# feiyeha/EGM-Unet

Measured on AMD Instinct MI355X. Metric: train images/sec at 3x512x512 bs=8/GPU, higher is better.
Workload: dtype bf16; 1 GPU; EGM-UNet GRFBUNet(3,2,base_c=32) fwd+5-term-loss+bwd+SGD, 8x3x512x512 per GPU (BASELINE.json configs[1]); global_batch=8, parallelism=dp1, launch=hipGraph replay, world_size=1

## Files before the change

egm_unet_amd/csrc/bn.hip:

```cpp
#include "common.h"
#include "bn_elem.h"
#include <stdlib.h>

namespace {


template <typename T, int MODE>
__device__ __forceinline__ void channel_partials_body(const T* __restrict__ a, int lda, const T* __restrict__ y, int ldy,
                                                      const float* __restrict__ scale, const float* __restrict__ shift,
                                                      const float* __restrict__ mean, const float* __restrict__ rstd,
                                                      int act, long long npix, int C, float* __restrict__ out, int bid, int nb) {
    __shared__ float red[2 * 256 * 8];
    const int ncv = C >> 3, rows = 256 / ncv;
    const int tid = threadIdx.x, cv = tid % ncv, row = tid / ncv;
    float s[8], q[8];
    zero8(s); zero8(q);
    if (MODE == 1) {
        for (int c = tid; c < C; c += 256) { red[c] = scale[c]; red[C + c] = shift[c]; red[2 * C + c] = mean[c]; red[3 * C + c] = rstd[c]; }
        __syncthreads();
    }
    float sc[8], sh[8], mu[8], rs[8];
    if (MODE == 1) {
#pragma unroll
        for (int j = 0; j < 8; ++j) { sc[j] = red[cv * 8 + j]; sh[j] = red[C + cv * 8 + j]; mu[j] = red[2 * C + cv * 8 + j]; rs[j] = red[3 * C + cv * 8 + j]; }
        __syncthreads();
    }
    if (row < rows) {
        for (long long p = (long long)bid * rows + row; p < npix; p += (long long)nb * rows) {
            float v[8];
            load8(a + p * lda + cv * 8, v);
            if (MODE == 0) {
#pragma unroll
                for (int j = 0; j < 8; ++j) { s[j] += v[j]; q[j] += v[j] * v[j]; }
            } else {
                float yv[8];
                load8(y + p * ldy + cv * 8, yv);
#pragma unroll
                for (int j = 0; j < 8; ++j) {
                    const float g = v[j] * act_grad<sizeof(T) == 2>(fmaf(yv[j], sc[j], sh[j]), act);
                    s[j] += g; q[j] += g * (yv[j] - mu[j]) * rs[j];
                }
            }
        }
    }
#pragma unroll
    for (int j = 0; j < 8; ++j) { red[tid * 8 + j] = s[j]; red[(256 + tid) * 8 + j] = q[j]; }
    __syncthreads();
    for (int t = tid; t < 2 * C; t += 256) {
        const int which = t / C, c = t - which * C, ccv = c >> 3, j = c & 7;
        float v = 0.f;
        for (int r = 0; r < rows; ++r) v += red[(which * 256 + r * ncv + ccv) * 8 + j];
        out[((long long)bid * 2 + which) * C + c] = v;
    }
}
template <typename T, int MODE>
__global__ __launch_bounds__(256) void channel_partials_kernel(const T* __restrict__ a, int lda, const T* __restrict__ y, int ldy,
                                                               const float* __restrict__ scale, const float* __restrict__ shift,
                                                               const float* __restrict__ mean, const float* __restrict__ rstd,
                                                               int act, long long npix, int C, float* __restrict__ out) {
    channel_partials_body<T, MODE>(a, lda, y, ldy, scale, shift, mean, rstd, act, npix, C, out, blockIdx.x, gridDim.x);
}

__device__ __forceinline__ void tiles_reduce(const float* __restrict__ st, int ntiles, int C, int c0, double& s_out, double& q_out,
                                             double* red) {
    const int tid = threadIdx.x, j = tid & 7, tl = tid >> 3;
    const int c = c0 + j;
    double s = 0.0, q = 0.0;
    if (c < C) {
        for (int t = tl; t < ntiles; t += 128) {
            s += (double)st[((long long)t * 2 + 0) * C + c];
            q += (double)st[((long long)t * 2 + 1) * C + c];
        }
    }
    red[tid] = s; red[1024 + tid] = q;
    __syncthreads();
    for (int stride = 64; stride > 0; stride >>= 1) {
        if (tl < stride) { red[tid] += red[tid + stride * 8]; red[1024 + tid] += red[1024 + tid + stride * 8]; }
        __syncthreads();
    }
    s_out = red[j]; q_out = red[1024 + j];
}

__global__ __launch_bounds__(1024) void reduce_tiles_kernel(const float* __restrict__ st, int ntiles, int C, float* __restrict__ out) {
    __shared__ double red[2048];
    double s, q;
    st += (long long)blockIdx.y * ntiles * 2 * C;
    out += (long long)blockIdx.y * 2 * C;
    tiles_reduce(st, ntiles, C, blockIdx.x * 8, s, q, red);
    const int c = blockIdx.x * 8 + (threadIdx.x & 7);
    if (threadIdx.x < 8 && c < C) { out[c] = (float)s; out[C + c] = (float)q; }
}

__device__ __forceinline__ void bn_finalize_body(const float* __restrict__ st, int ntiles, double count,
                                                 const float* __restrict__ gamma, const float* __restrict__ beta, float eps,
                                                 float momentum, float* __restrict__ rmean, float* __restrict__ rvar,
                                                 float* __restrict__ scale, float* __restrict__ shift,
                                                 float* __restrict__ save_mean, float* __restrict__ save_rstd, int C,
                                                 int Creal, int bid) {
    __shared__ double red[2048];
    double s, q;
    tiles_reduce(st, ntiles, C, bid * 8, s, q, red);
    const int c = bid * 8 + (threadIdx.x & 7);
    if (threadIdx.x < 8 && c >= Creal && c < C) { scale[c] = 0.f; shift[c] = 0.f; save_mean[c] = 0.f; save_rstd[c] = 0.f; }
    if (threadIdx.x < 8 && c < Creal) {
        const double mean = s / count;
        double var = q / count - mean * mean;
        if (var < 0.0) var = 0.0;
// ... 437 lines not shown
```

egm_unet_amd/csrc/conv3x3_tile.hip:

```cpp
#include "common.h"
#include "group.h"
#include "bn_elem.h"
#include <stdlib.h>

typedef __attribute__((ext_vector_type(8))) __bf16 bf16x8_t;
typedef __attribute__((ext_vector_type(16))) float f32x16_t;

__device__ uint4 egm_zero_page[4];

#ifndef EGM_TILE_DMA_EVERY
#define EGM_TILE_DMA_EVERY 1
#endif

namespace {

constexpr int TW = 32, PW = TW + 2, KC = 16;

struct TileParams {
    const bf16_t* x; const bf16_t* w; const float* bias; bf16_t* y; float* stats;
    bf16_t* y2; int ldy2, csplit;
    int ldx, ldy, N, H, W, Cin, Cout, bias_n;
    int tiles_y, tiles_x, npt, nct, G;
    int dbg;
};

template <int R, int NT, int WR, int WC, int NBUF> struct TileGeom {
    static constexpr int TROWS = WR * R, PH = TROWS + 2, NC = WC * NT * 32;
    static constexpr int PSLOTS = PH * PW * 2, WSLOTS = 9 * NC * 2;
    static constexpr int NPI = (PSLOTS + 63) / 64, NWI = WSLOTS / 64;
    static constexpr int KT = (NPI + NWI + 7) / 8;
    static constexpr int STAGE_BYTES = KT * 8 * 1024;
    static constexpr int WOFF = NPI * 1024;
    static constexpr int OROW = NT * 64 + 16;
    static constexpr int OUT_BYTES = 8 * 32 * OROW;
    static constexpr int SMEM = NBUF * STAGE_BYTES + OUT_BYTES;
    static_assert(WSLOTS % 64 == 0, "weight image must be whole DMA instructions");
    static_assert(SMEM <= 160 * 1024, "LDS budget");
    static_assert(9 * NC * 32 + 64 * 32 < 65536, "ds_read immediate offsets");
};

typedef __attribute__((ext_vector_type(2))) float f32x2_t;
typedef __attribute__((ext_vector_type(2))) __bf16 bf16x2_t;
__device__ __forceinline__ uint32_t pack_bf16x2(float lo, float hi) {
    f32x2_t v; v.x = lo; v.y = hi;
    const bf16x2_t b = __builtin_convertvector(v, bf16x2_t);
    return *reinterpret_cast<const uint32_t*>(&b);
}

__device__ __forceinline__ void glds16(const void* gsrc, unsigned lds_byte_addr) {
    unsigned keep;
    asm volatile("s_mov_b32 %0, m0\n\ts_mov_b32 m0, %2\n\ts_nop 0\n\tglobal_load_lds_dwordx4 %1, off\n\ts_mov_b32 m0, %0"
                 : "=&s"(keep) : "v"(gsrc), "s"(lds_byte_addr));
}

template <int R, int NT, int WR, int WC, int NBUF>
__global__ __launch_bounds__(512, 2) void conv3x3_tile_kernel(TileParams p) {
    constexpr int ACT = EGM_ACT_NONE;
#include "conv3x3_tile_body.h"
}
template <int R, int NT, int WR, int WC, int NBUF, int ACT>
__global__ __launch_bounds__(512, 2) void conv3x3_tile_act_kernel(TileParams p) {
#include "conv3x3_tile_body.h"
}

template <int R, int NT, int WR, int WC, int NBUF, int ACT = EGM_ACT_NONE>
int launch_tile(const TileParams& p, hipStream_t st) {
    using Gm = TileGeom<R, NT, WR, WC, NBUF>;
    constexpr auto kern = [] {
        if constexpr (ACT == EGM_ACT_NONE) return &conv3x3_tile_kernel<R, NT, WR, WC, NBUF>;
        else return &conv3x3_tile_act_kernel<R, NT, WR, WC, NBUF, ACT>;
    }();
    static bool attr_done = false;
    if (!attr_done) {
        hipError_t e = hipFuncSetAttribute(reinterpret_cast<const void*>(kern),
                                           hipFuncAttributeMaxDynamicSharedMemorySize, 160 * 1024);
        if (e != hipSuccess) EGM_FAIL(EGM_ERR_LAUNCH, "conv3x3_tile: hipFuncSetAttribute: %s", hipGetErrorString(e));
        attr_done = true;
    }
    const int grid = ((p.G + 7) / 8) * 8 * p.nct;
    hipLaunchKernelGGL(kern, dim3(grid), dim3(512), Gm::SMEM, st, p);
    EGM_CHECK_LAUNCH("conv3x3_tile");
    return EGM_OK;
}

struct TileCfg { int id, rows, nc; };
constexpr TileCfg kCfgs[] = {
    {0, 16, 128},
    {1, 8, 128},
    {2, 32, 64},
    {3, 16, 64},
    {4, 32, 32},
    {5, 16, 32},
};
}

static int g_tile_mode = -1;
extern "C" int egm_conv_tile_mode(int mode) {
    if (g_tile_mode < 0) g_tile_mode = getenv("EGM_CONV_TILE") ? atoi(getenv("EGM_CONV_TILE")) : 5;
    const int old = g_tile_mode;
    if (mode >= 0) g_tile_mode = mode;
    return old;
}

static int g_tile_dbg = 0;
extern "C" int egm_conv_tile_debug(int dbg) { const int old = g_tile_dbg; if (dbg >= 0) g_tile_dbg = dbg; return old; }

int egm_conv_tile_plan(int dtype, int N, int H, int W, int Cin, int Cout, int KH, int KW, int dil, int* cfg_out, int* nct_out, int* G_out) {
    if (dtype != EGM_BF16 || KH != 3 || KW != 3 || dil != 1) return 0;
    if (!egm_w_chunk16(dtype, KH, KW, Cin, Cout)) return 0;
    if (Cout % 32 != 0) return 0;
    if (egm_group_recording()) return 0;
    if (!(egm_conv_tile_mode(-1) & 1)) return 0;
    static int min_cin = -1;
    if (min_cin < 0) min_cin = getenv("EGM_TILE_MIN_CIN") ? atoi(getenv("EGM_TILE_MIN_CIN")) : 16;
    if (Cin < min_cin) return 0;
    const int tx = egm_cdiv(W, TW);
    int best = -1, best_nct = 0, best_npt = 0;
    long long best_score = -1;
    for (const TileCfg& c : kCfgs) {
        if (Cout % c.nc != 0) continue;
        if (c.nc == 32 && !(egm_conv_tile_mode(-1) & 2)) continue;
        const int nct = Cout / c.nc;
        const int npt = N * egm_cdiv(H, c.rows) * tx;
        const long long wgs = (long long)npt * nct;
        if (wgs < 192) continue;
        const long long rounds = (wgs + 255) / 256;
        const long long eff = wgs * 1000 / (rounds * 256);
        const long long score = eff * 4 + (long long)c.rows * c.nc / 128;
        if (score > best_score) { best_score = score; best = c.id; best_nct = nct; best_npt = npt; }
    }
    if (best < 0) return 0;
    int g = (256 / best_nct) / 8 * 8;
    if (g < 8) g = 8;
    if (g > best_npt) g = best_npt;
    *cfg_out = best; *nct_out = best_nct; *G_out = g;
    return 1;
}

const char* egm_conv_tile_name(int cfg) {
    switch (cfg) {
        case 0: return "conv3x3_tile_kernel<4, 2, 4, 2, 2>";
        case 1: return "conv3x3_tile_kernel<2, 2, 4, 2, 2>";
        case 2: return "conv3x3_tile_kernel<4, 2, 8, 1, 2>";
        case 3: return "conv3x3_tile_kernel<2, 2, 8, 1, 2>";
        case 4: return "conv3x3_tile_kernel<4, 1, 8, 1, 2>";
        default: return "conv3x3_tile_kernel<2, 1, 8, 1, 2>";
    }
}

int egm_conv_tile_launch(const void* x, int ldx, const void* wf, const float* bias, int bias_n, void* y, int ldy, float* stats, int N, int H,
                         int W, int Cin, int Cout, int cfg, int nct, int G, egm_stream_t s, void* y2, int ldy2, int csplit, int act) {
    TileParams p;
    p.x = (const bf16_t*)x; p.w = (const bf16_t*)wf; p.bias = bias; p.y = (bf16_t*)y; p.stats = stats;
    p.y2 = (bf16_t*)y2; p.ldy2 = ldy2; p.csplit = y2 ? csplit : 0;
    p.ldx = ldx; p.ldy = ldy; p.N = N; p.H = H; p.W = W; p.Cin = Cin; p.Cout = Cout; p.bias_n = bias ? bias_n : 0;
    p.dbg = g_tile_dbg;
    const int rows = kCfgs[cfg].rows;
    p.tiles_y = egm_cdiv(H, rows); p.tiles_x = egm_cdiv(W, TW); p.npt = N * p.tiles_y * p.tiles_x; p.nct = nct; p.G = G;
    EGM_REQUIRE((long long)(rows + 2) * W * ldx < (1LL << 31), "conv3x3_tile: halo window offsets exceed 32 bits");
    hipStream_t st = (hipStream_t)s;
    if (act != EGM_ACT_NONE) {
        EGM_REQUIRE(cfg <= 3 && y2 == nullptr, "conv3x3_tile: no activation instantiation for tile configuration %d", cfg);
        switch (cfg * 4 + act) {
#define EGM_TILE_ACT(c, R_, NT_, WR_, WC_) \
            case c * 4 + EGM_ACT_RELU: return launch_tile<R_, NT_, WR_, WC_, 2, EGM_ACT_RELU>(p, st); \
            case c * 4 + EGM_ACT_SIGMOID: return launch_tile<R_, NT_, WR_, WC_, 2, EGM_ACT_SIGMOID>(p, st); \
            case c * 4 + EGM_ACT_SILU: return launch_tile<R_, NT_, WR_, WC_, 2, EGM_ACT_SILU>(p, st);
            EGM_TILE_ACT(0, 4, 2, 4, 2)
            EGM_TILE_ACT(1, 2, 2, 4, 2)
            EGM_TILE_ACT(2, 4, 2, 8, 1)
            EGM_TILE_ACT(3, 2, 2, 8, 1)
#undef EGM_TILE_ACT
            default: EGM_FAIL(EGM_ERR_ARG, "conv3x3_tile: unknown activation %d", act);
        }
    }
    switch (cfg) {
        case 0: return launch_tile<4, 2, 4, 2, 2>(p, st);
        case 1: return launch_tile<2, 2, 4, 2, 2>(p, st);
        case 2: return launch_tile<4, 2, 8, 1, 2>(p, st);
        case 3: return launch_tile<2, 2, 8, 1, 2>(p, st);
        case 4: return launch_tile<4, 1, 8, 1, 2>(p, st);
        default: return launch_tile<2, 1, 8, 1, 2>(p, st);
    }
}
```

egm_unet_amd/csrc/conv3x3_tile_body.h:

```cpp
    extern __shared__ __attribute__((aligned(16))) unsigned char smem[];
    using Gm = TileGeom<R, NT, WR, WC, NBUF>;
    constexpr int PH = Gm::PH, NC = Gm::NC, NPI = Gm::NPI, NWI = Gm::NWI, KT = Gm::KT, STAGE = Gm::STAGE_BYTES, WOFF = Gm::WOFF;
    constexpr int OROW = Gm::OROW, NV = NT * 4;
    typedef __attribute__((address_space(3))) unsigned char* lds_p;

    const int b = blockIdx.x, q = b >> 3;
    const int ct = q % p.nct;
    const int grp = (q / p.nct) * 8 + (b & 7);
    if (grp >= p.G) return;
    const int co0 = ct * NC;
    const int tid = threadIdx.x, lane = tid & 63, r31 = lane & 31, h = lane >> 5;
    const int wv = __builtin_amdgcn_readfirstlane(tid >> 6);
    const int wr = wv / WC, wc = wv % WC;
    const int nch = p.Cin / KC;
    const int tpi = p.tiles_y * p.tiles_x;
    const unsigned smem_lds = (unsigned)(unsigned long long)(lds_p)smem;

    int rel[KT];
    int pk[KT];
#pragma unroll
    for (int k = 0; k < KT; ++k) {
        const int j = wv + 8 * k;
        if (j < NPI) {
            const int slot = j * 64 + lane, pix = slot >> 1, prow = pix / PW, col = pix - prow * PW;
// ... 75 lines not shown
    f32x16_t acc[R][NT];
#define EGM_ACC(m, nt, i) acc[m][nt][i]
    float ssum[8], ssq[8];
    zero8(ssum); zero8(ssq);

    auto compute = [&](int bufi, bool with_dma, const Src& q) __attribute__((always_inline)) {
        const unsigned char* sb = smem + bufi * STAGE;
#pragma unroll
        for (int s = 0; s < 3; ++s) {
            bf16x8_t fa[3][NT];
#pragma unroll
            for (int r = 0; r < 3; ++r)
#pragma unroll
                for (int nt = 0; nt < NT; ++nt)
                    fa[r][nt] = *reinterpret_cast<const bf16x8_t*>(sb + wbo + ((r * 3 + s) * NC + nt * 32) * 32);
#pragma unroll
            for (int rho = 0; rho < R + 2; ++rho) {
                const bf16x8_t fb = *reinterpret_cast<const bf16x8_t*>(sb + pb[s] + rho * (PW * 32));
#pragma unroll
                for (int m = 0; m < R; ++m) {
                    const int r = rho - m;
                    if (r >= 0 && r < 3) {
#pragma unroll
                        for (int nt = 0; nt < NT; ++nt) {
#ifdef EGM_TILE_MFMA16_PROXY
                            f32x16_t& a = acc[m][nt];
                            if (((r * 3 + s) & 1) == 0) {
                                f32x4_t t0 = __builtin_shufflevector(a, a, 0, 1, 2, 3), t1 = __builtin_shufflevector(a, a, 4, 5, 6, 7);
                                t0 = __builtin_amdgcn_mfma_f32_16x16x32_bf16(fa[r][nt], fb, t0, 0, 0, 0);
                                t1 = __builtin_amdgcn_mfma_f32_16x16x32_bf16(fa[r][nt], fb, t1, 0, 0, 0);
                                a[0] = t0[0]; a[1] = t0[1]; a[2] = t0[2]; a[3] = t0[3]; a[4] = t1[0]; a[5] = t1[1]; a[6] = t1[2]; a[7] = t1[3];
                            } else {
                                f32x4_t t0 = __builtin_shufflevector(a, a, 8, 9, 10, 11), t1 = __builtin_shufflevector(a, a, 12, 13, 14, 15);
                                t0 = __builtin_amdgcn_mfma_f32_16x16x32_bf16(fa[r][nt], fb, t0, 0, 0, 0);
                                t1 = __builtin_amdgcn_mfma_f32_16x16x32_bf16(fa[r][nt], fb, t1, 0, 0, 0);
                                a[8] = t0[0]; a[9] = t0[1]; a[10] = t0[2]; a[11] = t0[3]; a[12] = t1[0]; a[13] = t1[1]; a[14] = t1[2]; a[15] = t1[3];
                            }
#else
                            acc[m][nt] = __builtin_amdgcn_mfma_f32_32x32x16_bf16(fa[r][nt], fb, acc[m][nt], 0, 0, 0);
#endif
                        }
                    }
                }
                const int gi = s * (R + 2) + rho;
                if (gi % EGM_TILE_DMA_EVERY == 0 && gi / EGM_TILE_DMA_EVERY < KT) {
                    if (with_dma) dma(q, gi / EGM_TILE_DMA_EVERY);
                }
            }
        }
    };
    static_assert(9 >= KT && (3 * (R + 2) + EGM_TILE_DMA_EVERY - 1) / EGM_TILE_DMA_EVERY >= KT, "not enough fragment groups to carry the stage's DMA instructions");

    unsigned char* ot = smem + NBUF * STAGE + wv * 32 * OROW;
    auto epilogue = [&](const Tile& t) __attribute__((always_inline)) {
        const int cv = lane % NV, slot = lane / NV;
#pragma unroll
        for (int m = 0; m < R; ++m) {
#pragma unroll
            for (int nt = 0; nt < NT; ++nt)
#pragma unroll
                for (int gq = 0; gq < 4; ++gq) {
                    if (p.bias != nullptr) {
#pragma unroll
                        for (int j = 0; j < 4; ++j) {
                            const int co = co0 + wc * NT * 32 + nt * 32 + gq * 8 + h * 4 + j;
                            EGM_ACC(m, nt, gq * 4 + j) += co < p.bias_n ? p.bias[co] : 0.f;
                        }
                    }
                    if constexpr (ACT != EGM_ACT_NONE) {
#pragma unroll
                        for (int j = 0; j < 4; ++j) EGM_ACC(m, nt, gq * 4 + j) = conv_epi_act<ACT, true>(EGM_ACC(m, nt, gq * 4 + j));
                    }
                    uint2 v;
                    v.x = pack_bf16x2(EGM_ACC(m, nt, gq * 4 + 0), EGM_ACC(m, nt, gq * 4 + 1));
                    v.y = pack_bf16x2(EGM_ACC(m, nt, gq * 4 + 2), EGM_ACC(m, nt, gq * 4 + 3));
                    *reinterpret_cast<uint2*>(ot + r31 * OROW + (nt * 32 + gq * 8 + h * 4) * 2) = v;
                }
            const int oy = t.oy0 + R * wr + m;
            uint4 raw[NV / 2];
#pragma unroll
            for (int it2 = 0; it2 < NV / 2; ++it2)
                raw[it2] = *reinterpret_cast<const uint4*>(ot + (it2 * (64 / NV) + slot) * OROW + cv * 16);
            if (oy < p.H) {
                const int cvec = co0 + wc * NT * 32 + cv * 8;
                const bool second = p.csplit > 0 && cvec >= p.csplit;
                const int ldo = second ? p.ldy2 : p.ldy;
                bf16_t* yrow = (second ? p.y2 + (cvec - p.csplit) : p.y + cvec) + ((long long)(t.n * p.H + oy) * p.W + t.ox0) * ldo;
#pragma unroll
                for (int it2 = 0; it2 < NV / 2; ++it2) {
                    const int pl = it2 * (64 / NV) + slot;
                    const bool ok = t.ox0 + pl < p.W;
                    uint4 rw = raw[it2];
                    if (!ok) rw = make_uint4(0, 0, 0, 0);
                    if (ok) egm_store16_conv(yrow + (long long)pl * ldo, rw);
                    float v[8];
                    v[0] = __uint_as_float(rw.x << 16); v[1] = __uint_as_float(rw.x & 0xffff0000u);
                    v[2] = __uint_as_float(rw.y << 16); v[3] = __uint_as_float(rw.y & 0xffff0000u);
                    v[4] = __uint_as_float(rw.z << 16); v[5] = __uint_as_float(rw.z & 0xffff0000u);
                    v[6] = __uint_as_float(rw.w << 16); v[7] = __uint_as_float(rw.w & 0xffff0000u);
#pragma unroll
                    for (int j = 0; j < 8; ++j) { ssum[j] += v[j]; ssq[j] = fmaf(v[j], v[j], ssq[j]); }
                }
            }
        }
    };

#ifdef EGM_TILE_TIMING
    long long tph[6] = {0, 0, 0, 0, 0, 0};
    __builtin_amdgcn_sched_barrier(0);
    long long tmark = __builtin_amdgcn_s_memtime();
    const long long treal0 = __builtin_amdgcn_s_memrealtime();
    __builtin_amdgcn_sched_barrier(0);
#define EGM_TICK(i) do { __builtin_amdgcn_sched_barrier(0); const long long t_ = __builtin_amdgcn_s_memtime(); \
                         __builtin_amdgcn_s_waitcnt(0xC07F); __builtin_amdgcn_sched_barrier(0); tph[i] += t_ - tmark; tmark = t_; } while (0)
#else
#define EGM_TICK(i) do { } while (0)
#endif
    int cu_ch = 0;
    bool pending = false;
    if (NBUF == 3 && S > 1) asm volatile("s_waitcnt vmcnt(%0)" :: "n"(KT) : "memory");
    else asm volatile("s_waitcnt vmcnt(0)" ::: "memory");
    __builtin_amdgcn_s_barrier();
    EGM_TICK(5);

    int bc = 0, bi = NBUF - 1;
    for (int t = 0; t < S; ++t) {
        const bool more = t + NBUF - 1 < S;
        Src q = make_src(it, it_ch, bi);
        const bool with_dma = more && !(p.dbg & 1);
        if (more) advance_issue();
        if (with_dma && (p.dbg & 2)) {
#pragma unroll
            for (int k = 0; k < KT; ++k) dma(q, k);
        }
        EGM_TICK(0);
        if (pending) { if (!(p.dbg & 4)) epilogue(done); pending = false; }
        EGM_TICK(1);
        if (cu_ch == 0) {
#pragma unroll
            for (int m = 0; m < R; ++m)
#pragma unroll
                for (int nt = 0; nt < NT; ++nt)
#pragma unroll
                    for (int i = 0; i < 16; ++i) EGM_ACC(m, nt, i) = 0.f;
        }
        if (!(p.dbg & 2)) compute(bc, with_dma, q);
        EGM_TICK(2);
        if (++cu_ch == nch) {
            cu_ch = 0; pending = true; done = cu;
            cu.pt += p.G; if (cu.pt < p.npt) decode(cu);
        }
        if (NBUF == 3 && more) asm volatile("s_waitcnt vmcnt(%0)" :: "n"(KT) : "memory");
        else asm volatile("s_waitcnt vmcnt(0)" ::: "memory");
        EGM_TICK(3);
// ... 39 lines not shown
```

egm_unet_amd/csrc/conv3x3_wreg.hip:

```cpp
#include "common.h"
#include "group.h"
#include "bn_elem.h"
#include <stdlib.h>

typedef __attribute__((ext_vector_type(8))) __bf16 bf16x8_t;
typedef __attribute__((ext_vector_type(16))) float f32x16_t;
typedef __attribute__((ext_vector_type(2))) float f32x2_t;
typedef __attribute__((ext_vector_type(2))) __bf16 bf16x2_t;

__device__ uint4 egm_dump_wreg[64];
__device__ uint4 egm_zero_page_wreg[4];

namespace {

constexpr int TW = 32, PW = TW + 2, R = 2, TROWS = 16, PH = TROWS + 2, NBUF = 3;
constexpr int PSLOTS = PH * PW * 4;
constexpr int NPI = (PSLOTS + 63) / 64;
constexpr int KT = (NPI + 7) / 8;
constexpr int STAGE = KT * 8 * 1024;
constexpr int OROW = 64 + 16;
constexpr int SMEM = NBUF * STAGE + 8 * R * 32 * OROW;
static_assert(SMEM <= 160 * 1024, "LDS budget");
static_assert(KT <= 6, "DMA slots of a stage");

struct WregParams {
    const bf16_t* x; const bf16_t* w; const float* bias; bf16_t* y; float* stats;
    int ldx, ldy, N, H, W, Cin, Cout, bias_n;
    int tiles_y, tiles_x, npt, G;
};

__device__ __forceinline__ uint32_t pack2(float lo, float hi) {
    f32x2_t v; v.x = lo; v.y = hi;
    const bf16x2_t b = __builtin_convertvector(v, bf16x2_t);
    return *reinterpret_cast<const uint32_t*>(&b);
}
__device__ __forceinline__ void glds16(const void* gsrc, unsigned lds_byte_addr) {
    unsigned keep;
    asm volatile("s_mov_b32 %0, m0\n\ts_mov_b32 m0, %2\n\ts_nop 0\n\tglobal_load_lds_dwordx4 %1, off\n\ts_mov_b32 m0, %0"
                 : "=&s"(keep) : "v"(gsrc), "s"(lds_byte_addr));
}

template <int CH>
__global__ __launch_bounds__(512, 2) void conv3x3_wreg_kernel(WregParams p) {
    constexpr int ACT = EGM_ACT_NONE;
#include "conv3x3_wreg_body.h"
}
template <int CH, int ACT>
__global__ __launch_bounds__(512, 2) void conv3x3_wreg_act_kernel(WregParams p) {
#include "conv3x3_wreg_body.h"
}

template <int CH, int ACT = EGM_ACT_NONE>
int launch_wreg(const WregParams& p, hipStream_t st) {
    constexpr auto kern = [] { if constexpr (ACT == EGM_ACT_NONE) return &conv3x3_wreg_kernel<CH>; else return &conv3x3_wreg_act_kernel<CH, ACT>; }();
    static bool attr_done = false;
    if (!attr_done) {
        hipError_t e = hipFuncSetAttribute(reinterpret_cast<const void*>(kern), hipFuncAttributeMaxDynamicSharedMemorySize, 160 * 1024);
        if (e != hipSuccess) EGM_FAIL(EGM_ERR_LAUNCH, "conv3x3_wreg: hipFuncSetAttribute: %s", hipGetErrorString(e));
        attr_done = true;
    }
    hipLaunchKernelGGL(kern, dim3(p.G), dim3(512), SMEM, st, p);
    EGM_CHECK_LAUNCH("conv3x3_wreg");
    return EGM_OK;
}
}

int egm_conv_tile_mode(int mode);

int egm_conv_wreg_plan(int dtype, int N, int H, int W, int Cin, int Cout, int KH, int KW, int dil, int* G_out) {
    if (dtype != EGM_BF16 || KH != 3 || KW != 3 || dil != 1 || Cout != 32 || Cin != 32) return 0;
    if (egm_group_recording()) return 0;
    if (!(egm_conv_tile_mode(-1) & 4)) return 0;
    const long long npt = (long long)N * egm_cdiv(H, TROWS) * egm_cdiv(W, TW);
    if (npt < 512) return 0;
    *G_out = 256;
    return 1;
}
const char* egm_conv_wreg_name(int Cin) { (void)Cin; return "conv3x3_wreg_kernel<1>"; }

int egm_conv_wreg_launch(const void* x, int ldx, const void* wf, const float* bias, int bias_n, void* y, int ldy, float* stats, int N, int H,
                         int W, int Cin, int Cout, int G, egm_stream_t s, int act) {
    WregParams p;
    p.x = (const bf16_t*)x; p.w = (const bf16_t*)wf; p.bias = bias; p.y = (bf16_t*)y; p.stats = stats;
    p.ldx = ldx; p.ldy = ldy; p.N = N; p.H = H; p.W = W; p.Cin = Cin; p.Cout = Cout; p.bias_n = bias ? bias_n : 0;
    p.tiles_y = egm_cdiv(H, TROWS); p.tiles_x = egm_cdiv(W, TW); p.npt = N * p.tiles_y * p.tiles_x; p.G = G;
    EGM_REQUIRE((long long)(PH + 1) * W * ldx < (1LL << 31), "conv3x3_wreg: halo window offsets exceed 32 bits");
    switch (act) {
        case EGM_ACT_RELU: return launch_wreg<1, EGM_ACT_RELU>(p, (hipStream_t)s);
        case EGM_ACT_SIGMOID: return launch_wreg<1, EGM_ACT_SIGMOID>(p, (hipStream_t)s);
        case EGM_ACT_SILU: return launch_wreg<1, EGM_ACT_SILU>(p, (hipStream_t)s);
        default: return launch_wreg<1>(p, (hipStream_t)s);
    }
}
```

egm_unet_amd/csrc/conv3x3_wreg_body.h:

```cpp
    static_assert(CH == 1, "one 32-channel stage per tile");
    extern __shared__ __attribute__((aligned(16))) unsigned char smem[];
    typedef __attribute__((address_space(3))) unsigned char* lds_p;
    const int grp = blockIdx.x;
    if (grp >= p.G) return;
    const int tid = threadIdx.x, lane = tid & 63, r31 = lane & 31, h = lane >> 5;
    const int wv = __builtin_amdgcn_readfirstlane(tid >> 6);
    const int tpi = p.tiles_y * p.tiles_x;
    const unsigned smem_lds = (unsigned)(unsigned long long)(lds_p)smem;
    const void* const zp = reinterpret_cast<const void*>(egm_zero_page_wreg);
    const bool late = wv >= 4;

    int rel[KT];
#pragma unroll
    for (int k = 0; k < KT; ++k) {
        const int j = wv + 8 * k;
        const int slot = j * 64 + lane, pix = slot >> 2, prow = pix / PW, col = pix - prow * PW;
        const int cg = (slot & 3) ^ ((col >> 2) & 3);
        rel[k] = (j < NPI && pix < PH * PW) ? (prow * p.W + col) * p.ldx + cg * 8 : -1;
    }
    struct Tile { int pt, n, ty, tx; };
    const int d_n = p.G / tpi, d_rem = p.G - d_n * tpi, d_y = d_rem / p.tiles_x, d_x = d_rem - d_y * p.tiles_x;
    auto first_tile = [&](Tile& t) {
        t.pt = grp; t.n = grp / tpi; const int trem = grp - t.n * tpi;
        t.ty = trem / p.tiles_x; t.tx = trem - t.ty * p.tiles_x;
// ... 51 lines not shown
        }

    float ssum[8], ssq[8];
    zero8(ssum); zero8(ssq);
    unsigned char* ot = smem + NBUF * STAGE + wv * (R * 32 * OROW);
    unsigned char* dump = reinterpret_cast<unsigned char*>(egm_dump_wreg) + lane * 16;
    f32x16_t acc[R];

    auto compute = [&](int bufi, bool with_dma, const Src& q) __attribute__((always_inline)) {
        const unsigned char* sb = smem + bufi * STAGE;
#pragma unroll
        for (int ks = 0; ks < 2; ++ks)
#pragma unroll
            for (int s = 0; s < 3; ++s) {
                bf16x8_t fb[R + 2];
#pragma unroll
                for (int rho = 0; rho < R + 2; ++rho) fb[rho] = *reinterpret_cast<const bf16x8_t*>(sb + pb[s][ks] + rho * (PW * 64));
#pragma unroll
                for (int rho = 0; rho < R + 2; ++rho) {
#pragma unroll
                    for (int m = 0; m < R; ++m) {
                        const int r = rho - m;
                        if (r >= 0 && r < 3) acc[m] = __builtin_amdgcn_mfma_f32_32x32x16_bf16(wr[r * 3 + s][ks], fb[rho], acc[m], 0, 0, 0);
                    }
                }
                const int gi = ks * 3 + s;
                if (gi < KT) {
                    if (with_dma) dma(q, gi);
                }
            }
    };
    auto park = [&]() __attribute__((always_inline)) {
#pragma unroll
        for (int m = 0; m < R; ++m)
#pragma unroll
            for (int gq = 0; gq < 4; ++gq) {
                if (p.bias != nullptr) {
#pragma unroll
                    for (int j = 0; j < 4; ++j) {
                        const int co = gq * 8 + h * 4 + j;
                        acc[m][gq * 4 + j] += co < p.bias_n ? p.bias[co] : 0.f;
                    }
                }
                if constexpr (ACT != EGM_ACT_NONE) {
#pragma unroll
                    for (int j = 0; j < 4; ++j) acc[m][gq * 4 + j] = conv_epi_act<ACT, true>(acc[m][gq * 4 + j]);
                }
                uint2 v;
                v.x = pack2(acc[m][gq * 4 + 0], acc[m][gq * 4 + 1]);
                v.y = pack2(acc[m][gq * 4 + 2], acc[m][gq * 4 + 3]);
                *reinterpret_cast<uint2*>(ot + (m * 32 + r31) * OROW + (gq * 8 + h * 4) * 2) = v;
            }
    };
    auto store_tile = [&](const Tile& t) __attribute__((always_inline)) {
        const int cv = lane & 3, slot = lane >> 2;
        const int oy0 = t.ty * TROWS, ox0 = t.tx * TW;
        uint4 raw[R][2];
#pragma unroll
        for (int m = 0; m < R; ++m)
#pragma unroll
            for (int i2 = 0; i2 < 2; ++i2) raw[m][i2] = *reinterpret_cast<const uint4*>(ot + (m * 32 + i2 * 16 + slot) * OROW + cv * 16);
#pragma unroll
        for (int m = 0; m < R; ++m) {
            const int oy = oy0 + R * wv + m;
            bf16_t* yrow = p.y + ((long long)(t.n * p.H + oy) * p.W + ox0) * p.ldy + cv * 8;
#pragma unroll
            for (int i2 = 0; i2 < 2; ++i2) {
                const int pl = i2 * 16 + slot;
                const bool ok = oy < p.H && ox0 + pl < p.W;
                uint4 rw = raw[m][i2];
                if (!ok) rw = make_uint4(0, 0, 0, 0);
                unsigned char* dst = ok ? reinterpret_cast<unsigned char*>(yrow + (long long)pl * p.ldy) : dump;
                egm_store16_conv(dst, rw);
                float v[8];
                v[0] = __uint_as_float(rw.x << 16); v[1] = __uint_as_float(rw.x & 0xffff0000u);
                v[2] = __uint_as_float(rw.y << 16); v[3] = __uint_as_float(rw.y & 0xffff0000u);
                v[4] = __uint_as_float(rw.z << 16); v[5] = __uint_as_float(rw.z & 0xffff0000u);
                v[6] = __uint_as_float(rw.w << 16); v[7] = __uint_as_float(rw.w & 0xffff0000u);
#pragma unroll
                for (int j = 0; j < 8; ++j) { ssum[j] += v[j]; ssq[j] = fmaf(v[j], v[j], ssq[j]); }
            }
        }
    };

#ifdef EGM_TILE_TIMING
    long long tph[6] = {0, 0, 0, 0, 0, 0};
    __builtin_amdgcn_sched_barrier(0);
    long long tmark = __builtin_amdgcn_s_memtime();
    const long long treal0 = __builtin_amdgcn_s_memrealtime();
    __builtin_amdgcn_sched_barrier(0);
#define EGM_TICK(i) do { __builtin_amdgcn_sched_barrier(0); const long long t_ = __builtin_amdgcn_s_memtime(); \
                         __builtin_amdgcn_s_waitcnt(0xC07F); __builtin_amdgcn_sched_barrier(0); tph[i] += t_ - tmark; tmark = t_; } while (0)
#else
#define EGM_TICK(i) do { } while (0)
#endif
    if (ntl > 1) asm volatile("s_waitcnt vmcnt(%0)" :: "n"(KT) : "memory");
    else asm volatile("s_waitcnt vmcnt(0)" ::: "memory");
    __builtin_amdgcn_s_barrier();
    EGM_TICK(5);
    int bc = 0, bi = NBUF - 1;
    Tile cu; first_tile(cu);
    Tile prev = cu;
    for (int t = 0; t < ntl; ++t) {
        const bool more = t + NBUF - 1 < ntl;
        const Src q = make_src(it, bi);
        if (more) next_tile(it);
        EGM_TICK(0);
        if (t > 0 && !late) store_tile(prev);
        EGM_TICK(1);
#pragma unroll
        for (int m = 0; m < R; ++m)
#pragma unroll
            for (int i = 0; i < 16; ++i) acc[m][i] = 0.f;
        compute(bc, more, q);
        EGM_TICK(2);
        if (t > 0 && late) store_tile(prev);
        park();
        EGM_TICK(1);
        if (!more) asm volatile("s_waitcnt vmcnt(0)" ::: "memory");
        else if (late && t > 0) asm volatile("s_waitcnt vmcnt(%0)" :: "n"(KT + R * 2) : "memory");
        else asm volatile("s_waitcnt vmcnt(%0)" :: "n"(KT) : "memory");
        EGM_TICK(3);
        __builtin_amdgcn_s_barrier();
        EGM_TICK(4);
        prev = cu; next_tile(cu);
        bc = (bc + 1 == NBUF) ? 0 : bc + 1;
        bi = (bi + 1 == NBUF) ? 0 : bi + 1;
    }
    store_tile(prev);
    EGM_TICK(1);
#ifdef EGM_TILE_TIMING
    if (p.stats != nullptr) {
        const long long treal = __builtin_amdgcn_s_memrealtime() - treal0;
// ... 28 lines not shown
```

egm_unet_amd/csrc/conv_igemm.hip:

```cpp
#include "common.h"
#include "group.h"
#include "bn_elem.h"
#include <string.h>
#include <stdio.h>

typedef __attribute__((ext_vector_type(8))) __bf16 bf16x8_t;
typedef __attribute__((ext_vector_type(16))) float f32x16_t;
typedef __attribute__((ext_vector_type(2))) unsigned short u16x2_t;

int egm_conv_direct_plan(int dtype, int N, int H, int W, int Cin, int Cout, int KH, int KW, int dil, int* NT_out, int* nct_out, int* G_out,
                         size_t* smem_out);
int egm_conv_direct_launch(const void* x, int ldx, const void* wf, const float* bias, int bias_n, void* y, int ldy,
                           float* stats, int N, int H, int W, int Cin, int Cout, int KH, int KW, int dil, int NT, int nct, int G, size_t smem,
                           egm_stream_t s, int act = EGM_ACT_NONE);

int egm_conv_tile_plan(int dtype, int N, int H, int W, int Cin, int Cout, int KH, int KW, int dil, int* cfg_out, int* nct_out, int* G_out);
const char* egm_conv_tile_name(int cfg);
int egm_conv_wreg_plan(int dtype, int N, int H, int W, int Cin, int Cout, int KH, int KW, int dil, int* G_out);
const char* egm_conv_wreg_name(int Cin);
int egm_conv_wreg_launch(const void* x, int ldx, const void* wf, const float* bias, int bias_n, void* y, int ldy, float* stats, int N, int H,
                         int W, int Cin, int Cout, int G, egm_stream_t s, int act = EGM_ACT_NONE);
int egm_conv_tile_launch(const void* x, int ldx, const void* wf, const float* bias, int bias_n, void* y, int ldy, float* stats, int N, int H,
                         int W, int Cin, int Cout, int cfg, int nct, int G, egm_stream_t s, void* y2 = nullptr, int ldy2 = 0, int csplit = 0,
                         int act = EGM_ACT_NONE);
int egm_conv_c7_plan(int dtype, int N, int H, int W, int Cin, int Cout, int KH, int KW, int dil);
int egm_conv_c7_launch(const void* x, int ldx, const void* wf, const float* bias, int bias_n, void* y, int ldy, int N, int H, int W,
                       egm_stream_t s, int act = EGM_ACT_NONE);
int egm_conv_c16d_plan(int dtype, int N, int H, int W, int Cin, int Cout, int KH, int KW, int dil);
int egm_conv_c16d_launch(const void* x, int ldx, const void* wf, const float* bias, int bias_n, void* y, int ldy, float* stats, int N, int H,
                         int W, int dil, egm_stream_t s, int act = EGM_ACT_NONE);

namespace {

constexpr int TH = 8, TW = 32, KC = 32;

template <typename T> struct Mma;
template <> struct Mma<bf16_t> {
    static constexpr int kStep = 16;
    static constexpr int kPixStride = KC * 2 + 16;
    using Frag = bf16x8_t;
    static __device__ __forceinline__ Frag load(const unsigned char* row, int ks, int h) {
        return *reinterpret_cast<const Frag*>(row + ks * 32 + h * 16);
    }
    static __device__ __forceinline__ f32x16_t mma(Frag a, Frag b, f32x16_t c) {
        return __builtin_amdgcn_mfma_f32_32x32x16_bf16(a, b, c, 0, 0, 0);
    }
    static __device__ __forceinline__ void stage16(unsigned char* dst, const bf16_t* src, bool ok) {
        uint4 v = make_uint4(0, 0, 0, 0);
        if (ok) v = *reinterpret_cast<const uint4*>(src);
        *reinterpret_cast<uint4*>(dst) = v;
    }
    static __device__ __forceinline__ void stage_val(unsigned char* dst, uint4 v) { *reinterpret_cast<uint4*>(dst) = v; }
};
template <> struct Mma<float> {
    static constexpr int kStep = 2;
    static constexpr int kPixStride = KC * 4 + 4;
    using Frag = float;
    static __device__ __forceinline__ Frag load(const unsigned char* row, int ks, int h) {
        return *reinterpret_cast<const float*>(row + (ks * 2 + h) * 4);
    }
    static __device__ __forceinline__ f32x16_t mma(Frag a, Frag b, f32x16_t c) {
        return __builtin_amdgcn_mfma_f32_32x32x2f32(a, b, c, 0, 0, 0);
    }
    static __device__ __forceinline__ void stage16(unsigned char* dst, const float* src, bool ok) {
        float4 v = make_float4(0.f, 0.f, 0.f, 0.f);
        if (ok) v = *reinterpret_cast<const float4*>(src);
        float* d = reinterpret_cast<float*>(dst);
        d[0] = v.x; d[1] = v.y; d[2] = v.z; d[3] = v.w;
    }
    static __device__ __forceinline__ void stage_val(unsigned char* dst, uint4 v) {
        uint32_t* d = reinterpret_cast<uint32_t*>(dst);
        d[0] = v.x; d[1] = v.y; d[2] = v.z; d[3] = v.w;
    }
};

struct ConvParams {
    const void* x; const void* w; const float* bias; void* y; float* stats;
// ... 565 lines not shown
    const ConvPlan c = conv_plan(dtype, N, H, W, Cin, Cout, KH, KW, dil);
    char tmp[96];
    if (c.c16d) snprintf(tmp, sizeof(tmp), "conv3x3d_c16_kernel");
    else if (c.c7) snprintf(tmp, sizeof(tmp), "conv7x7_c16_kernel");
    else if (c.wreg) snprintf(tmp, sizeof(tmp), "%s", egm_conv_wreg_name(Cin));
    else if (c.tile) snprintf(tmp, sizeof(tmp), "%s", egm_conv_tile_name(c.tile_cfg));
    else if (c.direct) snprintf(tmp, sizeof(tmp), "conv_direct_kernel<%d, %s>", c.NT, KH == 1 ? "true" : "false");
    else if (c.pipe) snprintf(tmp, sizeof(tmp), "conv_igemm_pipe_kernel<%d, %d, %d, %d>", c.NT, (KH == 3 && dil == 1) ? 3 : 1,
                              (KH == 3 && dil == 1) ? 3 : (KH == 7 ? 7 : 1), c.R);
    else snprintf(tmp, sizeof(tmp), "conv_igemm_kernel<%s, %d>", dtype == EGM_BF16 ? "bf16_t" : "float", c.NT);
    const int n = (int)strlen(tmp);
    if (buf != nullptr && buflen > 0) { strncpy(buf, tmp, (size_t)buflen - 1); buf[buflen - 1] = 0; }
    return n;
}
extern "C" int egm_conv_stats_tiles(int dtype, int N, int H, int W, int Cin, int Cout, int KH, int KW, int dil) {
    return conv_plan(dtype, N, H, W, Cin, Cout, KH, KW, dil).G;
}

extern "C" int egm_conv_pack(int dtype, const void* w, void* wf, void* wd, int Cout, int Cin, int KH, int KW, int groups,
                             egm_stream_t s) {
    EGM_REQUIRE(w != nullptr && (wf != nullptr || wd != nullptr), "conv_pack: null pointer");
    EGM_REQUIRE(Cout > 0 && Cin > 0 && groups > 0 && Cout % groups == 0 && Cin % groups == 0, "conv_pack: bad channels/groups");
    EGM_REQUIRE(KH > 0 && KW > 0 && (KH & 1) && (KW & 1), "conv_pack: kernel must be odd");
    const int CoutP = (Cout + 7) / 8 * 8, CinP = (Cin + 7) / 8 * 8;
    const long long total = (long long)KH * KW * CoutP * CinP;
    const int grid = (int)((total + 255) / 256 > 4096 ? 4096 : (total + 255) / 256);
    EGM_DISPATCH_DTYPE(dtype, hipLaunchKernelGGL((conv_pack_kernel<T>), dim3(grid), dim3(256), 0, (hipStream_t)s,
                                                 (const float*)w, (T*)wf, (T*)wd, Cout, Cin, CoutP, CinP, KH, KW, groups));
    EGM_CHECK_LAUNCH("conv_pack");
    return EGM_OK;
}

extern "C" int egm_conv_pack_chunk(void) { return kPackChunk; }
extern "C" int egm_conv_pack_multi(int dtype, const void* table_dev, int n, long long total_chunks, egm_stream_t s) {
    EGM_REQUIRE(table_dev && n > 0 && total_chunks > 0 && total_chunks < (1LL << 30), "conv_pack_multi: bad args");
    EGM_DISPATCH_DTYPE(dtype, hipLaunchKernelGGL((conv_pack_multi_kernel<T>), dim3((unsigned)total_chunks), dim3(256), 0, (hipStream_t)s,
                                                 (const PackEntry*)table_dev, n));
    EGM_CHECK_LAUNCH("conv_pack_multi");
    return EGM_OK;
}

extern "C" int egm_conv_split_ok(int dtype, int N, int H, int W, int Cin, int Cout, int KH, int KW, int dil, int csplit) {
    if (csplit <= 0 || csplit >= Cout || csplit % 8 || N <= 0 || H <= 0 || W <= 0 || Cin <= 0 || Cin % 8 || Cout % 8) return 0;
    const ConvPlan c = conv_plan(dtype, N, H, W, Cin, Cout, KH, KW, dil);
    return (!c.c7 && !c.wreg && c.tile) ? 1 : 0;
}
extern "C" int egm_conv_fwd_split(int dtype, const void* x, int ldx, const void* wf, void* y, int ldy, void* y2, int ldy2, int csplit, int N,
                                  int H, int W, int Cin, int Cout, int KH, int KW, int dil, egm_stream_t s) {
    EGM_REQUIRE(x && wf && y && y2 && egm_aligned16(x) && egm_aligned16(wf) && egm_aligned16(y) && egm_aligned16(y2), "conv_fwd_split: bad pointers");
    EGM_REQUIRE(egm_conv_split_ok(dtype, N, H, W, Cin, Cout, KH, KW, dil, csplit), "conv_fwd_split: shape not supported (egm_conv_split_ok)");
    EGM_REQUIRE(ldx >= Cin && ldx % 8 == 0 && ldy >= csplit && ldy % 8 == 0 && ldy2 >= Cout - csplit && ldy2 % 8 == 0, "conv_fwd_split: bad ld");
    const ConvPlan c = conv_plan(dtype, N, H, W, Cin, Cout, KH, KW, dil);
    return egm_conv_tile_launch(x, ldx, wf, nullptr, 0, y, ldy, nullptr, N, H, W, Cin, Cout, c.tile_cfg, c.nct, c.G, s, y2, ldy2, csplit);
}

static int conv_fwd_impl(int dtype, const void* x, int ldx, const void* wf, const void* bias, int bias_n, void* y, int ldy, float* stats,
                         int N, int H, int W, int Cin, int Cout, int KH, int KW, int dil, int act, egm_stream_t s) {
    EGM_REQUIRE(x && wf && y, "conv_fwd: null pointer");
    EGM_REQUIRE(!bias || (bias_n > 0 && bias_n <= Cout), "conv_fwd: bad bias_n %d", bias_n);
    EGM_REQUIRE(N > 0 && H > 0 && W > 0, "conv_fwd: bad shape N=%d H=%d W=%d", N, H, W);
    EGM_REQUIRE(Cin > 0 && Cout > 0 && Cin % 8 == 0 && Cout % 8 == 0, "conv_fwd: Cin=%d/Cout=%d must be multiples of 8", Cin, Cout);
    EGM_REQUIRE(ldx >= Cin && ldy >= Cout && ldx % 8 == 0 && ldy % 8 == 0, "conv_fwd: bad ld (ldx=%d ldy=%d)", ldx, ldy);
    EGM_REQUIRE((KH & 1) && (KW & 1) && KH <= 7 && KW <= 7 && dil >= 1, "conv_fwd: unsupported kernel %dx%d dil %d", KH, KW, dil);
    EGM_REQUIRE(egm_aligned16(x) && egm_aligned16(wf) && egm_aligned16(y), "conv_fwd: pointers must be 16-byte aligned");
    EGM_REQUIRE((long long)N * H * W * (long long)(ldx > ldy ? ldx : ldy) < (1LL << 40), "conv_fwd: tensor too large");
    if (KH == 1 && KW == 1) dil = 1;

    ConvParams p;
    p.x = x; p.w = wf; p.bias = (const float*)bias; p.y = y; p.stats = stats;
    p.ldx = ldx; p.ldy = ldy; p.N = N; p.H = H; p.W = W; p.Cin = Cin; p.Cout = Cout; p.KH = KH; p.KW = KW; p.dil = dil; p.bias_n = bias ? bias_n : 0;
    p.wl = egm_w_layout(dtype, KH, KW, Cin, Cout);
    const ConvPlan c = conv_plan(dtype, N, H, W, Cin, Cout, KH, KW, dil);
    if (c.c16d) return egm_conv_c16d_launch(x, ldx, wf, (const float*)bias, bias_n, y, ldy, stats, N, H, W, dil, s, act);
    if (c.c7 && stats == nullptr) return egm_conv_c7_launch(x, ldx, wf, (const float*)bias, bias_n, y, ldy, N, H, W, s, act);
    if (c.wreg) return egm_conv_wreg_launch(x, ldx, wf, (const float*)bias, bias_n, y, ldy, stats, N, H, W, Cin, Cout, c.G, s, act);
    if (c.tile)
        return egm_conv_tile_launch(x, ldx, wf, (const float*)bias, bias_n, y, ldy, stats, N, H, W, Cin, Cout, c.tile_cfg, c.nct, c.G, s,
                                    nullptr, 0, 0, act);
    if (c.direct)
        return egm_conv_direct_launch(x, ldx, wf, (const float*)bias, bias_n, y, ldy, stats, N, H, W, Cin, Cout, KH, KW, dil, c.NT,
                                      c.nct, c.G, c.smem, s, act);
    p.tiles_y = c.tiles_y; p.tiles_x = c.tiles_x; p.npt = c.npt; p.nct = c.nct;
    const int NT = c.NT;
    if (c.pipe) {
        hipStream_t st = (hipStream_t)s;
        if (KH == 3 && dil == 1) {
            if (c.R == 4) return launch_pipe_act<1, 3, 3, 4>(p, c.G, st, act);
            if (c.R == 1) return launch_pipe_act<1, 3, 3, 1>(p, c.G, st, act);
            return NT == 2 ? launch_pipe_act<2, 3, 3, 2>(p, c.G, st, act) : launch_pipe_act<1, 3, 3, 2>(p, c.G, st, act);
        }
        if (KH == 7) return NT == 2 ? launch_pipe_act<2, 1, 7, 2>(p, c.G, st, act) : launch_pipe_act<1, 1, 7, 2>(p, c.G, st, act);
        return NT == 2 ? launch_pipe_act<2, 1, 1, 2>(p, c.G, st, act) : launch_pipe_act<1, 1, 1, 2>(p, c.G, st, act);
    }
    const int ps = (dtype == EGM_BF16) ? Mma<bf16_t>::kPixStride : Mma<float>::kPixStride;
    const bool halo = (dil == 1);
    const int wh = halo ? KH : 1, ww = halo ? KW : 1;
    int patch = (TH + wh - 1) * (TW + ww - 1) * ps;
    patch = (patch + 15) / 16 * 16;
    p.patch_bytes = patch;
    const int row_bytes = ww * NT * 32 * ps;
    p.wrows_per_stage = (wh * row_bytes <= 48 * 1024) ? wh : 1;
    size_t smem = (size_t)patch + (size_t)p.wrows_per_stage * row_bytes;
    const size_t red_bytes = 4 * 2 * NT * 32 * sizeof(float);
    if (smem < red_bytes) smem = red_bytes;
    EGM_REQUIRE(smem <= 160 * 1024, "conv_fwd: LDS budget exceeded (%zu)", smem);
    hipStream_t st = (hipStream_t)s;
// ... 16 lines not shown
```

egm_unet_amd/csrc/pool_up.hip:

```cpp
#include "common.h"

namespace {

inline int stream_grid(long long total_threads) {
    long long b = (total_threads + 255) / 256;
    if (b > 256 * 16) b = 256 * 16;
    if (b < 1) b = 1;
    return (int)b;
}

template <typename T>
__global__ void nchw_to_nhwc_kernel(const float* __restrict__ src, T* __restrict__ dst, int ld, int N, int C, long long HW) {
    const long long total = (long long)N * HW;
    for (long long i = blockIdx.x * 256LL + threadIdx.x; i < total; i += (long long)gridDim.x * 256) {
        const long long n = i / HW, p = i - n * HW;
        for (int c0 = 0; c0 < ld; c0 += 8) {
            float v[8];
#pragma unroll
            for (int j = 0; j < 8; ++j) v[j] = (c0 + j < C) ? src[(n * C + c0 + j) * HW + p] : 0.f;
            store8(dst + i * ld + c0, v);
        }
    }
}
template <typename T>
__global__ void nhwc_to_nchw_kernel(const T* __restrict__ src, int ld, float* __restrict__ dst, int N, int C, long long HW) {
    const long long total = (long long)N * HW;
    for (long long i = blockIdx.x * 256LL + threadIdx.x; i < total; i += (long long)gridDim.x * 256) {
        const long long n = i / HW, p = i - n * HW;
        for (int c0 = 0; c0 < C; c0 += 8) {
            float v[8];
            load8(src + i * ld + c0, v);
#pragma unroll
            for (int j = 0; j < 8; ++j) if (c0 + j < C) dst[(n * C + c0 + j) * HW + p] = v[j];
        }
    }
}

template <typename T>
__global__ void maxpool2_fwd_kernel(const T* __restrict__ x, int ldx, T* __restrict__ y, int ldy, int N, int H, int W, int C) {
    const int ncv = C >> 3, Ho = H >> 1, Wo = W >> 1;
    const long long total = (long long)N * Ho * Wo * ncv;
    for (long long i = blockIdx.x * 256LL + threadIdx.x; i < total; i += (long long)gridDim.x * 256) {
        long long p; int cv; egm_divmod(i, ncv, p, cv);
        int n, oy, ox; egm_pix_nyx(p, Ho, Wo, n, oy, ox);
        const T* b = x + (((long long)n * H + 2 * oy) * W + 2 * ox) * ldx + cv * 8;
        float a[8], v[8];
        load8(b, a);
        load8(b + ldx, v);
#pragma unroll
        for (int j = 0; j < 8; ++j) a[j] = fmaxf(a[j], v[j]);
        load8(b + (long long)W * ldx, v);
#pragma unroll
        for (int j = 0; j < 8; ++j) a[j] = fmaxf(a[j], v[j]);
// ... 387 lines not shown
        load8(a + p * lda + cv * 8, v);
        load8(b + p * ldb + cv * 8, u);
#pragma unroll
        for (int j = 0; j < 8; ++j) v[j] += u[j];
        load8(c + p * ldc + cv * 8, u);
#pragma unroll
        for (int j = 0; j < 8; ++j) v[j] += u[j];
        if (d != nullptr) {
            load8(d + p * ldd + cv * 8, u);
#pragma unroll
            for (int j = 0; j < 8; ++j) v[j] += u[j];
        }
        store8(out + p * ldo + cv * 8, v);
    }
}
template <typename T>
__global__ void sum4_hp_kernel(const T* __restrict__ a, int lda, const T* __restrict__ b, int ldb, const T* __restrict__ c, int ldc,
                               const T* __restrict__ d, int ldd, T* __restrict__ out, int ldo, int N, int H, int W, int C) {
    const int ncv = C >> 3;
    const long long total = (long long)N * H * W * ncv;
    for (long long i = xcd_contiguous_item(blockIdx.x, gridDim.x) * 256LL + threadIdx.x; i < total; i += (long long)gridDim.x * 256) {
        long long p; int cv; egm_divmod(i, ncv, p, cv);
        int xx, yy; egm_pix_yx(p, H, W, yy, xx);
        float v[8], u[8], s8[8];
        zero8(s8);
        load8(a + p * lda + cv * 8, v);
#pragma unroll
        for (int r = -1; r <= 1; ++r)
#pragma unroll
            for (int q = -1; q <= 1; ++q) {
                if (yy + r < 0 || yy + r >= H || xx + q < 0 || xx + q >= W) continue;
                load8(a + (p + (long long)r * W + q) * lda + cv * 8, u);
#pragma unroll
                for (int j = 0; j < 8; ++j) s8[j] += u[j];
            }
#pragma unroll
        for (int j = 0; j < 8; ++j) v[j] = to_f32(from_f32<T>(v[j] - s8[j] * (1.f / 9.f)));
        load8(b + p * ldb + cv * 8, u);
#pragma unroll
        for (int j = 0; j < 8; ++j) v[j] += u[j];
        if (c != nullptr) {
            load8(c + p * ldc + cv * 8, u);
#pragma unroll
            for (int j = 0; j < 8; ++j) v[j] += u[j];
        }
        if (d != nullptr) {
            load8(d + p * ldd + cv * 8, u);
#pragma unroll
            for (int j = 0; j < 8; ++j) v[j] += u[j];
        }
        store8(out + p * ldo + cv * 8, v);
    }
}
__global__ void vec_add_f32_kernel(float* __restrict__ y, const float* __restrict__ x, long long n) {
    for (long long i = blockIdx.x * 256LL + threadIdx.x; i < n; i += (long long)gridDim.x * 256) y[i] += x[i];
}
__global__ void fill_f32_kernel(float* __restrict__ y, float v, long long n) {
    for (long long i = blockIdx.x * 256LL + threadIdx.x; i < n; i += (long long)gridDim.x * 256) y[i] = v;
}

}

#define EGM_REQ_VEC(name, ptr, ld, C)                                                                      \
    EGM_REQUIRE((ptr) != nullptr && egm_aligned16(ptr) && (C) > 0 && (C) % 8 == 0 && (ld) >= (C) && (ld) % 8 == 0, \
                name ": bad tensor (ptr/alignment/C=%d/ld=%d)", (int)(C), (int)(ld))

extern "C" int egm_nchw_to_nhwc(int dtype, const void* src, void* dst, int ld, int N, int C, int H, int W, egm_stream_t s) {
    EGM_REQUIRE(src && dst && egm_aligned16(dst) && N > 0 && C > 0 && H > 0 && W > 0 && ld >= C && ld % 8 == 0, "nchw_to_nhwc: bad args");
    const long long HW = (long long)H * W;
    EGM_DISPATCH_DTYPE(dtype, hipLaunchKernelGGL((nchw_to_nhwc_kernel<T>), dim3(stream_grid(N * HW)), dim3(256), 0, (hipStream_t)s,
                                                 (const float*)src, (T*)dst, ld, N, C, HW));
    EGM_CHECK_LAUNCH("nchw_to_nhwc");
    return EGM_OK;
}
extern "C" int egm_nhwc_to_nchw(int dtype, const void* src, int ld, void* dst, int N, int C, int H, int W, egm_stream_t s) {
    EGM_REQUIRE(src && dst && egm_aligned16(src) && N > 0 && C > 0 && H > 0 && W > 0 && ld >= C && ld % 8 == 0, "nhwc_to_nchw: bad args");
    const long long HW = (long long)H * W;
    EGM_DISPATCH_DTYPE(dtype, hipLaunchKernelGGL((nhwc_to_nchw_kernel<T>), dim3(stream_grid(N * HW)), dim3(256), 0, (hipStream_t)s,
                                                 (const T*)src, ld, (float*)dst, N, C, HW));
    EGM_CHECK_LAUNCH("nhwc_to_nchw");
    return EGM_OK;
}

extern "C" int egm_maxpool2_fwd(int dtype, const void* x, int ldx, void* y, int ldy, int N, int H, int W, int C, egm_stream_t s) {
    EGM_REQ_VEC("maxpool2_fwd", x, ldx, C);
    EGM_REQ_VEC("maxpool2_fwd", y, ldy, C);
    EGM_REQUIRE(N > 0 && H >= 2 && W >= 2, "maxpool2_fwd: bad shape");
    const long long total = (long long)N * (H / 2) * (W / 2) * (C / 8);
    EGM_DISPATCH_DTYPE(dtype, hipLaunchKernelGGL((maxpool2_fwd_kernel<T>), dim3(stream_grid(total)), dim3(256), 0, (hipStream_t)s,
                                                 (const T*)x, ldx, (T*)y, ldy, N, H, W, C));
    EGM_CHECK_LAUNCH("maxpool2_fwd");
    return EGM_OK;
}
extern "C" int egm_maxpool2_bwd(int dtype, const void* x, int ldx, const void* dy, int lddy, void* dx, int lddx, int N, int H, int W,
                                int C, egm_stream_t s) {
    EGM_REQ_VEC("maxpool2_bwd", x, ldx, C);
    EGM_REQ_VEC("maxpool2_bwd", dy, lddy, C);
    EGM_REQ_VEC("maxpool2_bwd", dx, lddx, C);
    EGM_REQUIRE(N > 0 && H >= 2 && W >= 2, "maxpool2_bwd: bad shape");
    const long long total = (long long)N * (H / 2) * (W / 2) * (C / 8);
    EGM_DISPATCH_DTYPE(dtype, {
        hipLaunchKernelGGL((maxpool2_bwd_kernel<T>), dim3(stream_grid(total)), dim3(256), 0, (hipStream_t)s, (const T*)x, ldx,
                           (const T*)dy, lddy, (const T*)nullptr, 0, (T*)dx, lddx, N, H, W, C);
        if ((H & 1) || (W & 1))
            hipLaunchKernelGGL((zero_tail_kernel<T>), dim3(stream_grid((long long)N * H * W * (C / 8))), dim3(256), 0, (hipStream_t)s,
                               (T*)dx, lddx, N, H, W, C);
    });
    EGM_CHECK_LAUNCH("maxpool2_bwd");
    return EGM_OK;
}

extern "C" int egm_maxpool2_bwd_add(int dtype, const void* x, int ldx, const void* dy, int lddy, const void* add, int ldadd, void* dx, int lddx,
                                    int N, int H, int W, int C, egm_stream_t s) {
    EGM_REQ_VEC("maxpool2_bwd_add", x, ldx, C); EGM_REQ_VEC("maxpool2_bwd_add", dy, lddy, C); EGM_REQ_VEC("maxpool2_bwd_add", add, ldadd, C);
    EGM_REQ_VEC("maxpool2_bwd_add", dx, lddx, C);
    EGM_REQUIRE(N > 0 && H >= 2 && W >= 2 && !(H & 1) && !(W & 1), "maxpool2_bwd_add: H and W must be even (got %d x %d)", H, W);
    const long long total = (long long)N * (H / 2) * (W / 2) * (C / 8);
    EGM_DISPATCH_DTYPE(dtype, hipLaunchKernelGGL((maxpool2_bwd_kernel<T>), dim3(stream_grid(total)), dim3(256), 0, (hipStream_t)s, (const T*)x, ldx,
                                                 (const T*)dy, lddy, (const T*)add, ldadd, (T*)dx, lddx, N, H, W, C));
    EGM_CHECK_LAUNCH("maxpool2_bwd_add");
    return EGM_OK;
}

extern "C" int egm_sum4_hp(int dtype, const void* a, int lda, const void* b, int ldb, const void* c, int ldc, const void* d, int ldd, void* out,
                           int ldo, int N, int H, int W, int C, egm_stream_t s) {
    EGM_REQ_VEC("sum4_hp", a, lda, C); EGM_REQ_VEC("sum4_hp", b, ldb, C); EGM_REQ_VEC("sum4_hp", out, ldo, C);
    if (c != nullptr) EGM_REQ_VEC("sum4_hp", c, ldc, C);
    if (d != nullptr) EGM_REQ_VEC("sum4_hp", d, ldd, C);
    EGM_REQUIRE(N > 0 && H > 0 && W > 0, "sum4_hp: bad shape");
    EGM_DISPATCH_DTYPE(dtype, hipLaunchKernelGGL((sum4_hp_kernel<T>), dim3(stream_grid((long long)N * H * W * (C / 8))), dim3(256), 0, (hipStream_t)s,
                                                 (const T*)a, lda, (const T*)b, ldb, (const T*)c, ldc, (const T*)d, ldd, (T*)out, ldo, N, H, W, C));
    EGM_CHECK_LAUNCH("sum4_hp");
    return EGM_OK;
}
extern "C" int egm_upcat_fwd(int dtype, const void* skip, int lds, const void* low, int ldl, void* out, int ldo, int N, int Hs, int Ws,
                             int Cs, int Hl, int Wl, int Cl, egm_stream_t s) {
    if (skip != nullptr) EGM_REQ_VEC("upcat_fwd", skip, lds, Cs);
    EGM_REQUIRE(Cs > 0 && Cs % 8 == 0, "upcat_fwd: bad Cs %d", Cs);
    EGM_REQ_VEC("upcat_fwd", low, ldl, Cl);
    EGM_REQ_VEC("upcat_fwd", out, ldo, Cs + Cl);
    EGM_REQUIRE(N > 0 && Hl > 0 && Wl > 0 && Hs >= 2 * Hl && Ws >= 2 * Wl, "upcat_fwd: skip must be at least 2x the low-res size");
    const long long total = (long long)N * Hs * Ws * ((skip ? Cs + Cl : Cl) / 8);
    EGM_DISPATCH_DTYPE(dtype, hipLaunchKernelGGL((upcat_fwd_kernel<T>), dim3(stream_grid(total)), dim3(256), 0, (hipStream_t)s,
                                                 (const T*)skip, lds, (const T*)low, ldl, (T*)out, ldo, N, Hs, Ws, Cs, Hl, Wl, Cl));
    EGM_CHECK_LAUNCH("upcat_fwd");
    return EGM_OK;
}
extern "C" int egm_upcat_bwd_low(int dtype, const void* dout, int ldo, void* dlow, int ldl, int N, int Hs, int Ws, int Cs, int Hl,
                                 int Wl, int Cl, egm_stream_t s) {
    EGM_REQ_VEC("upcat_bwd_low", dout, ldo, Cs + Cl);
    EGM_REQ_VEC("upcat_bwd_low", dlow, ldl, Cl);
    EGM_REQUIRE(N > 0 && Hl > 0 && Wl > 0 && Hs >= 2 * Hl && Ws >= 2 * Wl && Cs % 8 == 0, "upcat_bwd_low: bad shape");
    const long long total = (long long)N * Hl * Wl * (Cl / 8);
    if (dtype == EGM_BF16 && Hl >= UB_TY && Wl >= UB_TX) {
        const int tiles_y = egm_cdiv(Hl, UB_TY), tiles_x = egm_cdiv(Wl, UB_TX), nchunk = egm_cdiv(Cl, UB_CB);
        hipLaunchKernelGGL((upcat_bwd_low_tiled_kernel<bf16_t>), dim3((unsigned)((long long)N * tiles_y * tiles_x * nchunk)), dim3(256), 0, (hipStream_t)s,
                           (const bf16_t*)dout, ldo, (bf16_t*)dlow, ldl, N, Hs, Ws, Cs, Hl, Wl, Cl, tiles_x, tiles_y, nchunk);
        EGM_CHECK_LAUNCH("upcat_bwd_low");
        return EGM_OK;
    }
    EGM_DISPATCH_DTYPE(dtype, hipLaunchKernelGGL((upcat_bwd_low_kernel<T>), dim3(stream_grid(total)), dim3(256), 0, (hipStream_t)s,
                                                 (const T*)dout, ldo, (T*)dlow, ldl, N, Hs, Ws, Cs, Hl, Wl, Cl));
    EGM_CHECK_LAUNCH("upcat_bwd_low");
    return EGM_OK;
}

extern "C" int egm_dwconv3_fwd(int dtype, const void* x, int ldx, const float* w, const float* b, const float* scale, void* y, int ldy,
                               int N, int H, int W, int C, egm_stream_t s) {
    EGM_REQ_VEC("dwconv3_fwd", x, ldx, C);
    EGM_REQ_VEC("dwconv3_fwd", y, ldy, C);
    EGM_REQUIRE(w && N > 0 && H > 0 && W > 0, "dwconv3_fwd: bad args");
    const long long total = (long long)N * H * W * (C / 8);
    EGM_DISPATCH_DTYPE(dtype, hipLaunchKernelGGL((dwconv3_fwd_kernel<T>), dim3(stream_grid(total)), dim3(256), (size_t)C * 10 * sizeof(float), (hipStream_t)s,
                                                 (const T*)x, ldx, w, b, scale, (T*)y, ldy, N, H, W, C));
    EGM_CHECK_LAUNCH("dwconv3_fwd");
    return EGM_OK;
}
static int dw_blocks(long long npix, int C) {
    const int rows = 256 / (C >> 3);
    long long b = (npix + rows - 1) / rows;
    if (b > 256) b = 256;
    return (int)(b < 1 ? 1 : b);
}
extern "C" long long egm_dwconv3_bwd_workspace(int N, int H, int W, int C) {
    if (C <= 0 || C % 8 || C > 2048) return -1;
// ... 150 lines not shown
```

egm_unet_amd/egm_unet.py:

```python
import math
from typing import Dict

import torch
import torch.nn as nn

from . import ops
from ._lib import ACT_NONE, ACT_RELU, ACT_SIGMOID
from .unet import DoubleConv, OutConv, Up, _SegNetBase


class StdPool(nn.Module):
    """Holder only (src/EGM-UNet.py:827-834); the statistics come from egm_mca_reduce."""


class MCAGate(nn.Module):
    def __init__(self, k_size, pool_types=("avg", "std")):
        super().__init__()
        self.pools = nn.ModuleList([nn.AdaptiveAvgPool2d(1) if p == "avg" else StdPool() for p in pool_types])
        self.conv = nn.Conv2d(1, 1, kernel_size=(1, k_size), stride=1, padding=(0, (k_size - 1) // 2), bias=False)
        self.sigmoid = nn.Sigmoid()
        self.weight = nn.Parameter(torch.rand(2))
        self.conv._egm_no_prepack = True


# ... 334 lines not shown
        self.proj_out = nn.Conv2d(self.split_sizes[-1], dim, 1)
        self.scale = nn.Parameter(torch.tensor(1.0))
        self.dwconv._egm_no_prepack = True
        print(f"[RGA] order={order}, split_sizes={self.split_sizes}")

    def _gate(self, i, g):
        seq = self.gate_convs[i]
        h = ops.gelu(ops.conv2d(g, seq[0].weight, seq[0].bias))
        return ops.conv2d(h, seq[2].weight, seq[2].bias)

    def forward(self, x):
        s0 = self.split_sizes[0]
        fused = ops.conv2d(x, self.proj_in.weight, self.proj_in.bias)
        base, gates = ops.split_channels(fused, s0)
        gates = ops.dwconv3(gates, self.dwconv.weight, self.dwconv.bias, self.scale)
        pieces, rest = [], gates
        for i in range(self.order - 1):
            piece, rest = ops.split_channels(rest, self.split_sizes[i])
            pieces.append(piece)
        pieces.append(rest)
        out = base
        for i in range(self.order):
            out = ops.bcast_gate(out, self._gate(i, pieces[i]))
            if i < self.order - 1:
                out = ops.conv2d(out, self.transform_convs[i].weight, self.transform_convs[i].bias)
        return ops.conv2d(out, self.proj_out.weight, self.proj_out.bias)


class DoubleConv1(nn.Sequential):

    def __init__(self, in_channels, out_channels, mid_channels=None, use_mca=True):
        if mid_channels is None:
            mid_channels = out_channels
        layers = [nn.Conv2d(in_channels, mid_channels, kernel_size=3, padding=1, bias=False), nn.BatchNorm2d(mid_channels), nn.ReLU(inplace=True)]
        if use_mca:
            layers.append(MCALayer(mid_channels))
        layers += [nn.Conv2d(mid_channels, out_channels, kernel_size=3, padding=1, bias=False), nn.BatchNorm2d(out_channels),
                   nn.ReLU(inplace=True), EdgeEnhancedGRFB(mid_channels, out_channels, stride=1, scale=0.1, visual=12)]
        super().__init__(*layers)
        self._mca = use_mca

    def forward(self, x, out=None, pool=False):
        o = 1 if self._mca else 0
        if self._mca:
            if ops.fuse_mca_bn():
                x = self[3](ops.conv_bn_lazy(x, self[0], self[1], ACT_RELU), exclusive=True)
            else:
                x = self[3](ops.conv_bn_act(x, self[0], self[1], ACT_RELU))
        else:
            x = ops.conv_bn_act(x, self[0], self[1], ACT_RELU)
        grfb = self[6 + o]
        N, H, W = x.shape[0], x.shape[1], x.shape[2]
        cat = grfb.cat_buffer(N, H, W, x.dtype, x.device) if self[3 + o].out_channels == grfb.shortcut.conv.in_channels else None
        x = ops.conv_bn_act(x, self[3 + o], self[4 + o], ACT_RELU, out=None if cat is None else cat[1][0])
        return grfb(x, out, cat, pool=pool)


class Down(nn.Sequential):
    def __init__(self, in_channels, out_channels, use_mca=True):
        super().__init__(nn.MaxPool2d(2, stride=2), DoubleConv1(in_channels, out_channels, use_mca=use_mca))

    def forward(self, x, out=None, pooled=None, pool=False):
        return self[1](ops.maxpool2(x) if pooled is None else pooled, out, pool=pool)


class GRFBUNet(_SegNetBase):
    def __init__(self, in_channels: int = 1, num_classes: int = 2, bilinear: bool = True, base_c: int = 64,
                 use_attention: bool = False, use_mca: bool = True):
        super().__init__()
        self.in_channels = in_channels
        self.num_classes = num_classes
        self.bilinear = bilinear
        self.in_conv = DoubleConv(in_channels, base_c)
        self.down1 = Down(base_c, base_c * 2, use_mca)
        self.down2 = Down(base_c * 2, base_c * 4, use_mca)
        self.down3 = Down(base_c * 4, base_c * 8, use_mca)
        factor = 2 if bilinear else 1
        self.down4 = Down(base_c * 8, base_c * 16 // factor, use_mca)
        self.attn1 = RecursiveGatedAttention(base_c * 16 // factor)
        self.up1 = Up(base_c * 16, base_c * 8 // factor, bilinear)
        self.up2 = Up(base_c * 8, base_c * 4 // factor, bilinear)
        self.up3 = Up(base_c * 4, base_c * 2 // factor, bilinear)
        self.up4 = Up(base_c * 2, base_c, bilinear)
        self.out_conv = OutConv(base_c, num_classes)

    def forward(self, x: torch.Tensor) -> Dict[str, torch.Tensor]:
        x = self._enter(x)
        bufs, slots = [None] * 4, [None] * 4
        if self.bilinear:
            N, H, W, _ = x.shape
            for k, up in enumerate((self.up4, self.up3, self.up2, self.up1)):
                cin = up.conv[0].in_channels
                cs = cin // 2
                h, w = H >> k, W >> k
                if cs % 8 == 0 and cin % 8 == 0 and (h << k) == H and (w << k) == W:
                    bufs[k], (slots[k], _) = ops.cat_slots(N, h, w, [cs, cin - cs], x.dtype, x.device)
        x1s, p1 = self.in_conv(x, slots[0], pool=True)
        x2s, p2 = self.down1(None, slots[1], pooled=p1, pool=True)
        x3s, p3 = self.down2(None, slots[2], pooled=p2, pool=True)
        x4s, p4 = self.down3(None, slots[3], pooled=p3, pool=True)
        d4 = self.down4(None, pooled=p4)
        if self.ddp_boundary is not None:
            self.ddp_boundary.extend([x1s, x2s, x3s, x4s, d4])
        x5 = self.attn1(d4)
        y = self.up1(x5, x4s, bufs[3])
        y = self.up2(y, x3s, bufs[2])
        y = self.up3(y, x2s, bufs[1])
# ... 3 lines not shown
```

egm_unet_amd/ops.py:

```python
import ctypes
import os
import struct
import threading
import weakref
from collections import namedtuple

import torch
from torch.autograd import Function, Variable

from ._lib import ACT_NONE, ACT_RELU, ACT_SIGMOID, dtype_code, lib, ptr, stream


def pad8(c: int) -> int:
    return (c + 7) // 8 * 8


def _nhwc(t: torch.Tensor):
    assert t.dim() == 4, t.shape
    N, H, W, C = t.shape
    s = t.stride()
    ok = (s[3] == 1 and s[2] % 8 == 0 and s[2] >= C and s[1] == W * s[2] and s[0] == H * W * s[2]
          and t.data_ptr() % 16 == 0 and C % 8 == 0)
    if not ok:
        if C % 8:
# ... 232 lines not shown
    blob, chunks = bytearray(), 0
    for m, (wf, wd) in zip(convs, bufs):
        Cout, Cin_g, KH, KW = m.weight.shape
        Cin = Cin_g * m.groups
        blob += struct.pack("<QQQiiiiiiii", m.weight.data_ptr(), wf.data_ptr(), wd.data_ptr(), Cout, Cin, pad8(Cout), pad8(Cin), KH, KW,
                            m.groups, chunks)
        chunks += (KH * KW * pad8(Cout) * pad8(Cin) + chunk - 1) // chunk
    dev = convs[0].weight.device
    table = st["table"].get(bytes(blob), dev)
    L.call("egm_conv_pack_multi", dtype_code(dtype), ptr(table), len(convs), chunks, stream())
    for m, (wf, wd) in zip(convs, bufs):
        w = m.weight
        key = (w.data_ptr(), w._version, _weight_generation[0], dtype, m.groups, tuple(w.shape))
        _pack_cache[id(w)] = (key, wf, wd, weakref.ref(w))
    st["stamp"] = stamp


_conv_uses = {}


def _note_conv_use(weight):
    ent = _conv_uses.get(id(weight))
    if ent is None or ent[0]() is not weight or ent[1] != _weight_generation[0]:
        ent = _conv_uses[id(weight)] = [weakref.ref(weight), _weight_generation[0], 0, 0]
        if len(_conv_uses) > 4096:
            for k in [k for k, v in _conv_uses.items() if v[0]() is None]:
                del _conv_uses[k]
    ent[2] += 1
    ent[3] = max(ent[3], ent[2])


def _sole_conv_use(weight):
    ent = _conv_uses.get(id(weight))
    if ent is None or ent[0]() is not weight:
        return False
    sole = ent[3] == 1
    ent[2] -= 1
    if ent[2] <= 0:
        del _conv_uses[id(weight)]
    return sole


_DEFER_WGRAD = os.environ.get("EGM_DEFER_WGRAD", "1") != "0"
merge_wgrads = _Switch("EGM_MERGE_WGRAD", "1",
                       """Get / set whether the slab kernels of deferred weight gradients are launched together when backward ends (merged
                       launches).""")
defer_bgrads = _Switch("EGM_DEFER_BGRAD", "1",
                       """Get / set whether conv bias gradients are left to the one multi-tensor pass at the end of backward.""")
fuse_dz = _Switch("EGM_FUSE_DZ", "1",
                  """Get / set whether BatchNorm backward computes dz on the fly from the classifier / MCALayer behind it (tests compare both
                  ways).""")


def _wgrad_deferrable(weight):
    return (_DEFER_WGRAD and _sole_conv_use(weight) and weight.is_leaf and weight.grad is None
            and not weight._backward_hooks and not torch.is_grad_enabled())


_wgrad_table, _wgrad_table_partial, _bgrad_table, _bgrad_table_partial = DeviceTable(), DeviceTable(), DeviceTable(), DeviceTable()
_BSUM_ENTRY = struct.Struct("<3Qq6i")
_WGRAD_DESC = struct.Struct("<3Q14i")
_wgrad_names = {}


def _wgrad_kernel_of(dt, N, H, W, CinP, CoutP, KH, KW, dil):
    key = (dt, N, H, W, CinP, CoutP, KH, KW, dil)
    name = _wgrad_names.get(key)
    if name is None:
        buf = ctypes.create_string_buffer(96)
        lib().cdll.egm_conv_wgrad_kernel_name(dt, N, H, W, CinP, CoutP, KH, KW, dil, ctypes.cast(buf, ctypes.c_void_p), 96)
        name = _wgrad_names[key] = buf.value
    return name


_Slab = namedtuple("_Slab", "dt x ldx gy ldg ws N H W CinP CoutP Cin Cout KH KW dil groups")
_Wgrad = namedtuple("_Wgrad", "ws param nslab taps CoutP CinP Cout Cin groups gref gptr")
_Bgrad = namedtuple("_Bgrad", "gy ldg npix C Cout param gref gptr")


def _handed_over(queue, ready_only, name):
    todo, later = [], []
    for ent in queue:
        grad = ent.param.grad
        if ent.gref() is not None or (grad is not None and grad.data_ptr() == ent.gptr):
            todo.append(ent)
        elif ready_only:
            later.append(ent)
        elif grad is not None:
            raise RuntimeError(f"deferred conv {name} gradient lost its destination: {name}.grad exists but is not the buffer backward() "
                               f"returned (tensor hook / gradient copy); set EGM_DEFER_{name[0].upper()}GRAD=0 for this model")
    queue[:] = later
    return todo


_runs = {}


class _BackwardRun:
    __slots__ = ("id", "slabs", "wgrads", "bgrads", "dz", "__weakref__")

    def __init__(self, run_id):
        self.id, self.slabs, self.wgrads, self.bgrads, self.dz = run_id, [], [], [], {}

    def finish(self):
        _runs.pop(self.id, None)
        if self.dz:
            kinds = [v[1][0] for v in self.dz.values()]
            self.dz.clear()
            raise RuntimeError(f"egm_unet_amd: deferred BatchNorm gradients {kinds} were never consumed (the tensor between the producer and "
                               "its BatchNorm had another consumer); call ops.fuse_dz(False)")
        self.flush()

    def flush(self, ready_only=False):
        self.flush_bgrads(ready_only)
        self.launch_slabs()
        self.reduce_wgrads(ready_only)

    def flush_bgrads(self, ready_only=False):
        todo = _handed_over(self.bgrads, ready_only, "bias") if self.bgrads else None
        if not todo:
            return
        L = lib()
        by_dtype = {}
        for e in todo:
            by_dtype.setdefault(e.gy.dtype, []).append(e)
        for dtype, ents in by_dtype.items():
            dev = ents[0].gy.device
            nblks = [L.query("egm_channel_partials_blocks", e.npix, e.C) for e in ents]
            ws = torch.empty(sum(nb * 2 * e.C for nb, e in zip(nblks, ents)), dtype=torch.float32, device=dev)
            blob1, blob2, b1, b2, off = bytearray(), bytearray(), 0, 0, 0
            for nb, e in zip(nblks, ents):
                part = ws.data_ptr() + 4 * off
                blob1 += _BSUM_ENTRY.pack(e.gy.data_ptr(), part, e.gptr, e.npix, e.ldg, e.C, e.Cout, nb, b1, 0)
                blob2 += _BSUM_ENTRY.pack(e.gy.data_ptr(), part, e.gptr, e.npix, e.ldg, e.C, e.Cout, nb, b2, 0)
                b1 += nb; b2 += e.C // 8; off += nb * 2 * e.C
            _bgrad_table.reserve(dev); _bgrad_table_partial.reserve(dev)
            table = (_bgrad_table_partial if ready_only else _bgrad_table).get(bytes(blob1 + blob2), dev)
            L.call("egm_bias_grad_multi", dtype_code(dtype), ptr(table), len(ents), b1, b2, stream())

    def launch_slabs(self):
        if not self.slabs:
            return
        L, st = lib(), stream()
        todo, self.slabs = self.slabs, []
        buckets = {}
        for e in todo:
            buckets.setdefault((e.dt, _wgrad_kernel_of(e.dt, e.N, e.H, e.W, e.CinP, e.CoutP, e.KH, e.KW, e.dil)), []).append(e)
        per = 4
        for (dt, _name), ents in buckets.items():
            for i in range(0, len(ents), per):
                blob = b"".join(_WGRAD_DESC.pack(e.x.data_ptr(), e.gy.data_ptr(), e.ws.data_ptr(), e.ldx, e.ldg, e.N, e.H, e.W, e.CinP, e.CoutP,
                                                 e.Cin, e.Cout, e.KH, e.KW, e.dil, e.groups, 0) for e in ents[i:i + per])
                L.call("egm_conv_wgrad_multi", dt, blob, len(ents[i:i + per]), st)

    def reduce_wgrads(self, ready_only=False):
        todo = _handed_over(self.wgrads, ready_only, "weight") if self.wgrads else None
        if not todo:
            return
# ... 19 lines not shown
    return run


def flush_ready_wgrads():
    run = _run(create=False)
    if run is not None:
        run.flush(ready_only=True)


def _queue_wgrad(ws, weight, nslab, taps, CoutP, CinP, Cout, Cin, groups, gw):
    _run().wgrads.append(_Wgrad(ws, weight, nslab, taps, CoutP, CinP, Cout, Cin, groups, weakref.ref(gw), gw.data_ptr()))


def _defer_dz(standin, payload):
    _run().dz[standin.data_ptr()] = (standin, payload)


def _take_dz(g):
    run = _run(create=False)
    return run.dz.pop(g.data_ptr(), None) if run is not None and run.dz else None


def _bias_grad(gy, Cout, bias=None, defer=False):
    if (defer and defer_bgrads.on and bias is not None and bias.is_leaf and bias.grad is None and not bias._backward_hooks
            and not torch.is_grad_enabled()):
        gy, ldg = _nhwc(gy)
        gb = torch.empty(Cout, dtype=torch.float32, device=gy.device)
        _run().bgrads.append(_Bgrad(gy, ldg, _npix(gy), gy.shape[3], Cout, bias, weakref.ref(gb), gb.data_ptr()))
        return gb
    return _channel_sum(gy)[0, :Cout]


def _channel_sum(t):
    t, ld = _nhwc(t)
    C, npix = t.shape[3], _npix(t)
    nb = lib().query("egm_channel_partials_blocks", npix, C)
    part = _f32(nb * 2 * C, t.device)
    out = _f32((2, C), t.device)
    lib().call("egm_channel_sums", dtype_code(t.dtype), ptr(t), ld, npix, C, ptr(part), stream())
    lib().call("egm_reduce_tiles", ptr(part), nb, C, ptr(out), stream())
    return out


class Lazy:
    __slots__ = ("y", "coef", "act")

    def __init__(self, y, coef, act):
        self.y, self.coef, self.act = y, coef, act

    shape = property(lambda self: self.y.shape)
    dtype = property(lambda self: self.y.dtype)
    device = property(lambda self: self.y.device)

    def materialize(self, out=None):
        return _Materialize.apply(self.y, self.coef, self.act, None if out is None else [out])


def materialize(x, out=None):
    if isinstance(x, Lazy):
        return x.materialize(out)
    if out is not None and not (x.data_ptr() == out.data_ptr() and x.stride() == out.stride()):
        return _axpby(x, 1.0, None, 0.0, out)
    return x


class _Materialize(Function):

    @staticmethod
    def forward(ctx, y, coef, act, out_slot):
        y, ldy = _nhwc(y)
        N, H, W, CP = y.shape
        z, ldz = _slot_or_new(out_slot, (N, H, W, CP), y.dtype, y.device)
        lib().call("egm_bn_act_fwd", dtype_code(y.dtype), ptr(y), ldy, ptr(coef[0]), ptr(coef[1]), act, ptr(z), ldz, _npix(y), CP, stream())
        return z

    @staticmethod
    def backward(ctx, g):
        return g, None, None, None


def _unlazy(x):
    if isinstance(x, Lazy):
        return x.y, x.coef, x.act
    return x, None, ACT_NONE


group_convs = _Switch("EGM_GROUP_CONVS", "1",
                      """Get / set whether conv_group() merges launches (tests compare both ways).""")


class conv_group:

    depth = 0
    serial = 0

    def __enter__(self):
        self.on = group_convs.on
        conv_group.depth += 1
        if conv_group.depth == 1:
            conv_group.serial += 1
        if self.on:
            lib().call("egm_group_begin")
        return self

    def __exit__(self, et, ev, tb):
        conv_group.depth -= 1
        if self.on:
            if et is None:
# ... 11 lines not shown
        raise RuntimeError(f"conv2d: input has {CinP} channels, weight expects {Cin} (padded {pad8(Cin)})")
    CoutP = pad8(Cout)
    L, dt = lib(), dtype_code(x.dtype)
    wf, wd = _packed_weights(weight, groups, x.dtype)
    y = torch.empty((N, H, W, CoutP), dtype=x.dtype, device=x.device)
    stats = None
    if want_stats:
        ntiles = L.query("egm_conv_stats_tiles", dt, N, H, W, CinP, CoutP, KH, KW, dil)
        stats = _f32((ntiles, 2, CoutP), x.device)
    b = bias.detach() if bias is not None else None
    L.call("egm_conv_fwd", dt, ptr(x), ldx, ptr(wf), ptr(b), Cout if b is not None else 0, ptr(y), CoutP, ptr(stats), N, H, W, CinP, CoutP,
           KH, KW, dil, stream())
    return y, stats, wd


_C1_DESC = struct.Struct("<5Qq6i")
_C1_MAXC = int(os.environ.get("EGM_CONV1X1_BWD_MAXC", "64"))


fuse_c1 = _Switch("EGM_CONV1X1_BWD", "1",
                  """Get / set whether the backward of a 1x1 conv runs as one fused launch (dx + weight-gradient slabs) where that applies.""")


def _c1_shape_ok(x, gy, weight, dil, groups):
    return (fuse_c1.on and weight.shape[2] == 1 and weight.shape[3] == 1 and groups == 1 and x.shape[3] <= _C1_MAXC and gy.shape[3] <= _C1_MAXC
            and bool(lib().cdll.egm_conv1x1_bwd_supported(dtype_code(x.dtype), x.shape[3], gy.shape[3])))


def _conv1x1_bwd(items):
    L, st = lib(), stream()
    descs, res, now = [], [], []
    dt = dtype_code(items[0][0].dtype)
    for x, ldx, dy, lddy, weight, wd, need_gx, defer in items:
        N, H, W, CinP = x.shape
        CoutP, npix = dy.shape[3], _npix(x)
        Cout, Cin = weight.shape[0], weight.shape[1]
        nslab = L.query("egm_conv1x1_bwd_slabs", npix)
        ws = torch.empty(nslab * CoutP * CinP + 4, dtype=torch.float32, device=x.device)
        gx = torch.empty((N, H, W, CinP), dtype=x.dtype, device=x.device) if need_gx else None
        gw = torch.empty_like(weight)
        descs.append(_C1_DESC.pack(x.data_ptr(), dy.data_ptr(), wd.data_ptr(), 0 if gx is None else gx.data_ptr(), ws.data_ptr(), npix, ldx, lddy,
                                   CinP, CinP, CoutP, 0))
        if defer:
            _queue_wgrad(ws, weight, nslab, 1, CoutP, CinP, Cout, Cin, 1, gw)
        else:
            now.append((ws, gw, nslab, CoutP, CinP, Cout, Cin))
        res.append((gx, gw))
    L.call("egm_conv1x1_bwd", dt, b"".join(descs), len(descs), st)
    for ws, gw, nslab, CoutP, CinP, Cout, Cin in now:
        L.call("egm_wgrad_reduce", ptr(ws), ptr(gw), nslab, 1, CoutP, CinP, Cout, Cin, 1, 0, st)
    return res


def _conv_grads(x, ldx, dy, weight, wd, dil, groups, Cin, Cout, need_gx, need_gw, x_split=0, c1=True):
    N, H, W, CinP = x.shape
    CoutP = dy.shape[3]
    if c1 and need_gw and not x_split and _c1_shape_ok(x, dy, weight, dil, groups):
        return _conv1x1_bwd([(x, ldx, dy, CoutP, weight, wd, need_gx, _wgrad_deferrable(weight))])[0]
    gx = gw = None
    if need_gw:
        gw = _conv_wgrad(x, ldx, dy, CoutP, weight, dil, groups, Cin, Cout)
    if need_gx:
        gx = _conv_dgrad(dy, wd, N, H, W, CoutP, CinP, weight.shape[2], weight.shape[3], dil, x_split)
    return gx, gw


def _conv_wgrad(x, ldx, gy, ldg, weight, dil, groups, Cin, Cout, defer=None):
    N, H, W, CinP = x.shape
    CoutP = gy.shape[3]
    KH, KW = weight.shape[2], weight.shape[3]
    L, dt, st = lib(), dtype_code(x.dtype), stream()
    gw = torch.empty_like(weight)
    nbytes = L.query("egm_conv_wgrad_workspace", N, H, W, CinP, CoutP, KH, KW)
    ws = torch.empty(nbytes // 4 + 4, dtype=torch.float32, device=x.device)
    if defer is None:
        defer = _wgrad_deferrable(weight)
    if defer and merge_wgrads.on:
        _run().slabs.append(_Slab(dt, x, ldx, gy, ldg, ws, N, H, W, CinP, CoutP, Cin, Cout, KH, KW, dil, groups))
    else:
        L.call("egm_conv_wgrad", dt, ptr(x), ldx, ptr(gy), ldg, None if defer else ptr(gw), ptr(ws), N, H, W, CinP, CoutP, Cin, Cout, KH, KW,
               dil, groups, 0, st)
    if defer:
        nslab = L.query("egm_conv_wgrad_slabs", dt, N, H, W, CinP, CoutP, KH, KW, dil)
        _queue_wgrad(ws, weight, nslab, KH * KW, CoutP, CinP, Cout, Cin, groups, gw)
    return gw


def _dz_fusable(C):
    return fuse_dz.on and C % 8 == 0 and C <= 1024 and 256 % (C // 8) == 0


class _Conv2d(Function):

    @staticmethod
    def forward(ctx, x, weight, bias, dil, groups, want_stats, bias_grad_zero=False, defer_dgrad=False):
        x, ldx = _nhwc(x)
        Cout, Cin_g = weight.shape[0], weight.shape[1]
        y, stats, wd = _conv_forward(x, ldx, weight, bias, dil, groups, want_stats)
        if ctx.needs_input_grad[1]:
            _note_conv_use(weight)
        ctx.save_for_backward(x, weight, wd)
        ctx.meta = (dil, groups, bias is not None, Cin_g * groups, Cout)
        ctx.bias_grad_zero = bias_grad_zero
        ctx.bias = bias
        ctx.defer_dgrad = bool(defer_dgrad and weight.shape[2] == 1 and weight.shape[3] == 1 and groups == 1
                               and Cout <= 8 and weight.is_contiguous() and _dz_fusable(x.shape[3]))
        ctx.set_materialize_grads(False)
        if want_stats:
            ctx.mark_non_differentiable(stats)
            return y, stats
        return y

    @staticmethod
    def backward(ctx, gy, *_):
        if gy is None:
            return (None,) * 8
        x, weight, wd = ctx.saved_tensors
        dil, groups, has_bias, Cin, Cout = ctx.meta
        gy, ldg = _nhwc(gy)
        x, ldx = _nhwc(x)
        N, H, W, CinP = x.shape
        CoutP = gy.shape[3]
        KH, KW = weight.shape[2], weight.shape[3]
        L, dt, st = lib(), dtype_code(x.dtype), stream()
        gx = gw = gb = None
        need_gx, need_gw = ctx.needs_input_grad[0], ctx.needs_input_grad[1]
        defer = _wgrad_deferrable(weight) if need_gw else False
        if has_bias and ctx.needs_input_grad[2]:
            gb = _zero_grad_vec(Cout, x.device) if ctx.bias_grad_zero else _bias_grad(gy, Cout, ctx.bias, defer)
        if need_gw and not (need_gx and ctx.defer_dgrad and fuse_dz.on) and _c1_shape_ok(x, gy, weight, dil, groups):
            gx, gw = _conv1x1_bwd([(x, ldx, gy, ldg, weight, wd, need_gx, defer)])[0]
            return gx, gw, gb, None, None, None, None, None
        if need_gx:
            gx = torch.empty((N, H, W, CinP), dtype=x.dtype, device=x.device)
            if ctx.defer_dgrad and fuse_dz.on:
                _defer_dz(gx, ("cls", gy, ldg, weight.detach(), Cout, Cin))
            else:
                L.call("egm_conv_fwd", dt, ptr(gy), ldg, ptr(wd), None, 0, ptr(gx), CinP, None, N, H, W, CoutP, CinP, KH, KW, dil, st)
        if need_gw and gw is None:
            gw = _conv_wgrad(x, ldx, gy, ldg, weight, dil, groups, Cin, Cout, defer=defer)
        return gx, gw, gb, None, None, None, None, None


def conv2d(x, weight, bias=None, dil=1, groups=1, want_stats=False, bias_grad_zero=False, defer_dgrad=False):
    return _Conv2d.apply(materialize(x), weight, bias, dil, groups, want_stats, bias_grad_zero, defer_dgrad)


def _conv_dgrad(dy, wd, N, H, W, CoutP, CinP, KH, KW, dil, x_split):
    L, dt, st = lib(), dtype_code(dy.dtype), stream()
    gx = torch.empty((N, H, W, CinP), dtype=dy.dtype, device=dy.device)
    if x_split and fuse_dz.on and L.cdll.egm_conv_split_ok(dt, N, H, W, CoutP, CinP, KH, KW, dil, x_split):
        ga = torch.empty((N, H, W, x_split), dtype=dy.dtype, device=dy.device)
        gb = torch.empty((N, H, W, CinP - x_split), dtype=dy.dtype, device=dy.device)
        L.call("egm_conv_fwd_split", dt, ptr(dy), CoutP, ptr(wd), ptr(ga), x_split, ptr(gb), CinP - x_split, x_split, N, H, W, CoutP, CinP,
               KH, KW, dil, st)
        _defer_dz(gx, ("split", ga, gb))
    else:
        L.call("egm_conv_fwd", dt, ptr(dy), CoutP, ptr(wd), None, 0, ptr(gx), CinP, None, N, H, W, CoutP, CinP, KH, KW, dil, st)
    return gx


fuse_cls = _Switch("EGM_FUSE_CLS", "1",
                   """Get / set whether the 1x1 classifier runs inside the BatchNorm apply pass of the layer in front (tests compare both ways).""")


class _BnActCls(Function):

    @staticmethod
    def forward(ctx, y, coef, act, weight, bias):
        y, ldy = _nhwc(y)
        N, H, W, C = y.shape
        nc, Cin = weight.shape[0], weight.shape[1]
        L, dt, st, dev = lib(), dtype_code(y.dtype), stream(), y.device
        z = torch.empty((N, H, W, C), dtype=y.dtype, device=dev)
        logits = torch.empty((N, nc, H, W), dtype=torch.float32, device=dev)
        L.call("egm_bn_act_cls_fwd", dt, ptr(y), ldy, ptr(coef[0]), ptr(coef[1]), act, ptr(z), C, ptr(weight.detach()), nc, Cin,
               ptr(bias.detach()) if bias is not None else None, ptr(logits), N, H, W, C, st)
        if ctx.needs_input_grad[3]:
            _note_conv_use(weight)
        ctx.save_for_backward(z, weight)
        ctx.meta = (nc, Cin, bias is not None)
        ctx.bias = bias
        return logits

    @staticmethod
    def backward(ctx, g):
        z, weight = ctx.saved_tensors
        nc, Cin, has_bias = ctx.meta
        N, H, W, C = z.shape
        L, dt, st, dev = lib(), dtype_code(z.dtype), stream(), z.device
        g = g.contiguous().float()
        dl = torch.empty((N, H, W, 8), dtype=z.dtype, device=dev)
        L.call("egm_nchw_to_nhwc", dt, ptr(g), ptr(dl), 8, N, nc, H, W, st)
        gy = gw = gb = None
        defer = _wgrad_deferrable(weight) if ctx.needs_input_grad[3] else False
        if ctx.needs_input_grad[3]:
            gw = _conv_wgrad(z, C, dl, 8, weight, 1, 1, Cin, nc, defer=defer)
        if has_bias and ctx.needs_input_grad[4]:
            gb = _bias_grad(dl, nc, ctx.bias, defer)
        if ctx.needs_input_grad[0]:
            gy = torch.empty((N, H, W, C), dtype=z.dtype, device=dev)
            if fuse_dz.on and _dz_fusable(C):
                _defer_dz(gy, ("cls", dl, 8, weight.detach(), nc, Cin))
            else:
                _, wd = _packed_weights(weight, 1, z.dtype)
                L.call("egm_conv_fwd", dt, ptr(dl), 8, ptr(wd), None, 0, ptr(gy), C, None, N, H, W, 8, C, 1, 1, 1, st)
        return gy, None, None, gw, gb


def bn_act_cls_ok(x, weight):
    C = x.shape[3] if isinstance(x, Lazy) else 0
    return (fuse_cls.on and isinstance(x, Lazy) and weight.dim() == 4 and weight.shape[2] == 1 and weight.shape[3] == 1 and weight.shape[0] <= 8
            and pad8(weight.shape[1]) == C and C % 8 == 0 and C // 8 <= 64 and (C // 8) & (C // 8 - 1) == 0 and weight.is_contiguous())


def bn_act_cls(x, weight, bias):
    return _BnActCls.apply(x.y, x.coef, x.act, weight, bias)


def _bn_step(bn):
    if bn.training and bn.num_batches_tracked is not None and not getattr(bn, "_egm_counter_managed", False):
        bn.num_batches_tracked.add_(1)
    return bn.training or bn.running_mean is None, 0.1 if bn.momentum is None else bn.momentum


def _rows(coef):
    return ptr(coef[0]), ptr(coef[1]), ptr(coef[2]), ptr(coef[3])


def _bn_coef(stats, npix, gamma, beta, running_mean, running_var, eps, momentum, training, CP, C, dev):
    L, coef = lib(), _f32((4, CP), dev)
    if training:
        L.call("egm_bn_finalize", ptr(stats), stats.shape[0], npix, ptr(gamma.detach()), ptr(beta.detach()), eps, momentum,
               ptr(running_mean), ptr(running_var), *_rows(coef), CP, C, stream())
    else:
        L.call("egm_bn_eval_coeffs", ptr(gamma.detach()), ptr(beta.detach()), ptr(running_mean), ptr(running_var), eps, *_rows(coef), CP, C,
               stream())
    return coef


def _bn_bwd_buffers(y, nb=None):
    CP, dev = y.shape[3], y.device
    if nb is None:
        nb = lib().query("egm_channel_partials_blocks", _npix(y), CP)
    return nb, _f32(nb * 2 * CP, dev), _f32((2, CP), dev), _f32((4, CP), dev), torch.empty(tuple(y.shape), dtype=y.dtype, device=dev)


def _bn_backward(family, lead, geo, y, coef, act, training, nb=None):
    L, st = lib(), stream()
    y, ldy = _nhwc(y)
    CP, npix = y.shape[3], _npix(y)
    nb, part, sums, cf4, dy = _bn_bwd_buffers(y, nb)
    rows, train = _rows(coef), 1 if training else 0
    L.call(family + "_bwd_reduce", *lead, ptr(y), ldy, *rows, act, ptr(part), *geo, st)
    L.call("egm_bn_bwd_coefs", ptr(part), nb, npix, *rows, train, ptr(sums), ptr(cf4), CP, st)
    L.call(family + "_bwd_apply", *lead, ptr(y), ldy, *rows, act, train, ptr(sums), ptr(dy), CP, *geo, st)
    return dy, sums


def _conv_bn_grads(need, x, ldx, dy, weight, wd, sums, dil, groups, has_bias, Cin, Cout, training, x_split=0, c1=True, conv_grads=None):
    if conv_grads is None:
        conv_grads = _conv_grads(x, ldx, dy, weight, wd, dil, groups, Cin, Cout, need[0], need[1], x_split, c1)
    gx, gw = conv_grads
    gb = _bn_conv_bias_grad(Cout, dy, training, dy.device) if (has_bias and need[2]) else None
    return gx, gw, gb, sums[1, :Cout] if need[3] else None, sums[0, :Cout] if need[4] else None


class _ConvBN(Function):

    @staticmethod
    def forward(ctx, x, weight, bias, gamma, beta, running_mean, running_var, eps, momentum, act, training, dil, groups, x_split=0):
        x, ldx = _nhwc(x)
        ctx.x_split = int(x_split) if (x_split and 0 < x_split < x.shape[3] and x_split % 8 == 0) else 0
        Cout, Cin_g = weight.shape[0], weight.shape[1]
        y, stats, wd = _conv_forward(x, ldx, weight, bias, dil, groups, training)
        coef = _bn_coef(stats, _npix(y), gamma, beta, running_mean, running_var, eps, momentum, training, y.shape[3], Cout, y.device)
        if ctx.needs_input_grad[1]:
            _note_conv_use(weight)
        ctx.save_for_backward(x, weight, wd, y, coef)
        ctx.meta = (dil, groups, bias is not None, Cin_g * groups, Cout, act, training)
        ctx.mark_non_differentiable(coef)
        ctx.set_materialize_grads(False)
        return y, coef

    @staticmethod
    def backward(ctx, gz, _):
        if gz is None:
            return (None,) * 14
        x, weight, wd, y, coef = ctx.saved_tensors
        dil, groups, has_bias, Cin, Cout, act, training = ctx.meta
        pend = _take_dz(gz)
        gz, ldg = _nhwc(gz)
        x, ldx = _nhwc(x)
        CoutP, npix, dt = y.shape[3], _npix(y), dtype_code(x.dtype)
        if pend is None:
            family = ("egm_bn_act", (dt, ptr(gz), ldg), (npix, CoutP))
        elif pend[1][0] == "cls":
            _, dl, lddl, wcls, nc, ldw = pend[1]
            family = ("egm_bn_cls", (dt, ptr(dl), lddl, ptr(wcls), nc, ldw), (npix, CoutP))
        else:
            _, dxo, ldd, gates, mcoef, ns, geo = pend[1]
            family = ("egm_bn_mca", (dt, ptr(dxo), ldd, ptr(gates), ptr(mcoef), ns), geo + (CoutP,))
        dy, sums = _bn_backward(*family, y, coef, act, training)
        return _conv_bn_grads(ctx.needs_input_grad, x, ldx, dy, weight, wd, sums, dil, groups, has_bias, Cin, Cout, training,
                              ctx.x_split) + (None,) * 9


fuse_mca_bwd = _Switch("EGM_FUSE_MCA_BWD", "1",
                       """Get / set whether the MCALayer backward computes du and dxo in one tiled launch (bf16; egm_mca_bwd_dudxo).""")


fuse_mca_bn = _Switch("EGM_FUSE_MCA_BN", "1",
                      """Get / set whether the BatchNorm+ReLU in front of an MCALayer is applied by the layer's statistics pass
                      (egm_mca_reduce_bn).""")


fuse_pool = _Switch("EGM_FUSE_POOL", "1",
                    """Get / set whether the skip-connection max pool is fused into the kernels on either side of it (tests compare both
                    ways).""")


class _ConvBNPool(Function):

    @staticmethod
    def forward(ctx, x, weight, bias, gamma, beta, running_mean, running_var, eps, momentum, act, training, dil, groups, out_slot):
        x, ldx = _nhwc(x)
        Cout, Cin_g = weight.shape[0], weight.shape[1]
        y, stats, wd = _conv_forward(x, ldx, weight, bias, dil, groups, training)
        N, H, W, CoutP = y.shape
        L, dt, st, dev = lib(), dtype_code(y.dtype), stream(), y.device
        coef = _bn_coef(stats, _npix(y), gamma, beta, running_mean, running_var, eps, momentum, training, CoutP, Cout, dev)
        z, ldz = _slot_or_new(out_slot, (N, H, W, CoutP), y.dtype, dev)
        pooled = torch.empty((N, H // 2, W // 2, CoutP), dtype=y.dtype, device=dev)
        L.call("egm_bn_act_fwd_pool", dt, ptr(y), CoutP, ptr(coef[0]), ptr(coef[1]), act, ptr(z), ldz, ptr(pooled), CoutP, N, H, W, CoutP, st)
        if ctx.needs_input_grad[1]:
            _note_conv_use(weight)
        ctx.save_for_backward(x, weight, wd, y, coef, z)
        ctx.meta = (dil, groups, bias is not None, Cin_g * groups, Cout, act, training)
        ctx.set_materialize_grads(False)
        return z, pooled

    @staticmethod
    def backward(ctx, gz, gpool):
        if gz is None and gpool is None:
            return (None,) * 14
        x, weight, wd, y, coef, z = ctx.saved_tensors
        dil, groups, has_bias, Cin, Cout, act, training = ctx.meta
        x, ldx = _nhwc(x)
        N, H, W, CoutP = y.shape
        L, dt = lib(), dtype_code(x.dtype)
        if gz is not None and gpool is not None:
            gz, ldg = _nhwc(gz)
            gpool, ldp = _nhwc(gpool)
            family = ("egm_bn_pool", (dt, ptr(gz), ldg, ptr(gpool), ldp), (N, H, W, CoutP))
            nb = L.query("egm_bn_pool_bwd_blocks", N, H, W, CoutP)
        else:
            if gz is None:
                zk, ldzk = _nhwc(z)
                gpool, ldp = _nhwc(gpool)
                gz = torch.empty((N, H, W, CoutP), dtype=x.dtype, device=y.device)
                L.call("egm_maxpool2_bwd", dt, ptr(zk), ldzk, ptr(gpool), ldp, ptr(gz), CoutP, N, H, W, CoutP, stream())
            gz, ldg = _nhwc(gz)
            family, nb = ("egm_bn_act", (dt, ptr(gz), ldg), (_npix(y), CoutP)), None
        dy, sums = _bn_backward(*family, y, coef, act, training, nb)
        return _conv_bn_grads(ctx.needs_input_grad, x, ldx, dy, weight, wd, sums, dil, groups, has_bias, Cin, Cout, training,
                              c1=False) + (None,) * 9


def conv_bn_lazy(x, conv, bn, act, dil=1, groups=1):
    if _fold_packs() is not None:
        return _fold_conv(x, conv, act, dil)
    training, momentum = _bn_step(bn)
    y, coef = _ConvBN.apply(materialize(x), conv.weight, conv.bias, bn.weight, bn.bias, bn.running_mean, bn.running_var, bn.eps, momentum, act,
                            training, dil, groups)
    return Lazy(y, coef, act)


def conv_bn_act_pool(x, conv, bn, act, dil=1, groups=1, out=None):
    if _fold_packs() is not None:
        z = _fold_conv(x, conv, act, dil, out)
        return z, maxpool2(z)
    training, momentum = _bn_step(bn)
    x = materialize(x)
    return _ConvBNPool.apply(x, conv.weight, conv.bias, bn.weight, bn.bias, bn.running_mean, bn.running_var, bn.eps, momentum, act,
                             training, dil, groups, None if out is None else [out])


def pool_fusable(x):
    return fuse_pool.on and x.shape[1] % 2 == 0 and x.shape[2] % 2 == 0 and x.shape[1] >= 2 and x.shape[2] >= 2 and x.shape[3] <= 1024


class _BnAct(Function):
    @staticmethod
    def forward(ctx, y, stats, gamma, beta, running_mean, running_var, eps, momentum, act, training, out_slot=None):
        y, ldy = _nhwc(y)
        N, H, W, CP = y.shape
        C, npix, dev = gamma.shape[0], _npix(y), y.device
        L, dt, st = lib(), dtype_code(y.dtype), stream()
        if training and stats is None:
            nb = L.query("egm_channel_partials_blocks", npix, CP)
            stats = _f32((nb, 2, CP), dev)
            L.call("egm_channel_sums", dt, ptr(y), ldy, npix, CP, ptr(stats), st)
        coef = _bn_coef(stats, npix, gamma, beta, running_mean, running_var, eps, momentum, training, CP, C, dev)
        z, ldz = _slot_or_new(out_slot, (N, H, W, CP), y.dtype, dev)
        L.call("egm_bn_act_fwd", dt, ptr(y), ldy, ptr(coef[0]), ptr(coef[1]), act, ptr(z), ldz, npix, CP, st)
        ctx.save_for_backward(y, coef)
        ctx.meta = (act, training, C)
        return z

    @staticmethod
    def backward(ctx, gz):
        y, coef = ctx.saved_tensors
        act, training, C = ctx.meta
        gz, ldg = _nhwc(gz)
        y, ldy = _nhwc(y)
        N, H, W, CP = y.shape
        npix, dev = _npix(y), y.device
        L, dt, st = lib(), dtype_code(y.dtype), stream()
        rows = _rows(coef)
# ... 315 lines not shown
                    dbias = _zero_grad_vec(Cout, dev) if training else _f32(CoutP, dev)
                descs.append(_pw_head(x=x, w=wf, wd=wd, coef=coef, g=g, q=q, dp=dp, sums=sums, cf4=cf4, dw=dw, dbias=None if training else dbias,
                                      cov=cov, mu=mu, bwd=bwd, dx=dx, npix=npix, ldx=ldx, lddx=CinP, Cin=CinP, Cin_real=Cin, Cout=Cout, CoutP=CoutP,
                                      act=act, mode=mode, ldg=ldg, ldq=ldq, lddp=CoutP, train=1 if training else 0, alpha=alpha))
                keep += [g, q, sums, cf4, bwd]
                grads[wpos] = dw
                grads[wpos + 1] = dbias if (dbias is None or training) else dbias[:Cout]
                grads[wpos + 2] = sums[1, :Cout] if ctx.needs_input_grad[1 + wpos + 2] else None
                grads[wpos + 3] = sums[0, :Cout] if ctx.needs_input_grad[1 + wpos + 3] else None
                grads[wpos + 4] = dp
        blob = b"".join(descs)
        L.call("egm_pw_bwd_reduce", dt, blob, len(descs), st)
        L.call("egm_pw_bwd_coefs", dt, blob, len(descs), st)
        L.call("egm_pw_bwd_apply", dt, blob, len(descs), st)
        return (None,) + tuple(grads)


def pw_conv_bn(problems):
    meta, flat = [], []
    for x, heads in problems:
        flat.append(materialize(x))
        hm = []
        for conv, bn, act, mode, p, alpha, out in heads:
            training, momentum = _bn_step(bn)
            hm.append((bn.running_mean, bn.running_var, bn.eps, momentum, act, 0 if mode is None else mode + 1, alpha, training,
                       None if out is None else [out]))
            flat += [conv.weight, conv.bias, bn.weight, bn.bias, None if mode is None else materialize(p)]
        meta.append(hm)
    return list(_PwConvBN.apply(meta, *flat))


_pw_sites = _Switch("EGM_PW_SITES", "ew,heads,tails", parse=lambda v: set(t for t in v.split(",") if t))


def pw_sites(sites=None):
    return _pw_sites(sites)


def pw_applicable(x, convs, site="ew"):
    if not fuse_pw.on or site not in _pw_sites.on or _fold_packs() is not None:
        return False
    for c in convs:
        if tuple(c.weight.shape[2:]) != (1, 1) or c.groups != 1 or pad8(c.weight.shape[1]) != x.shape[3]:
            return False
    return _pw_ok(x.dtype, x.shape[3], [pad8(c.weight.shape[0]) for c in convs])


def bn_act(y, bn, act, stats=None, out=None):
    training, momentum = _bn_step(bn)
    return _BnAct.apply(y, stats, bn.weight, bn.bias, bn.running_mean, bn.running_var, bn.eps, momentum, act, training,
                        None if out is None else [out])


def conv_bn_act(x, conv, bn, act, dil=1, groups=1, out=None, lazy=False):
    if _fold_packs() is not None:
        z = _fold_conv(x, conv, act, dil, out)
        return Lazy(z, _fold_identity(z.shape[3]), ACT_NONE) if out is None and lazy == "force" else z
    training, momentum = _bn_step(bn)
    x = materialize(x)
    y, coef = _ConvBN.apply(x, conv.weight, conv.bias, bn.weight, bn.bias, bn.running_mean, bn.running_var, bn.eps, momentum, act,
                            training, dil, groups, getattr(x, "_egm_split", 0))
    z = Lazy(y, coef, act)
    if out is None and lazy == "force":
        return z
    return z.materialize(out)


_fold_state = threading.local()


class folded_inference:

    def __init__(self, packs):
        self.packs, self.prev = packs, None

    def __enter__(self):
        self.prev = getattr(_fold_state, "packs", None)
        _fold_state.packs = self.packs
        return self

    def __exit__(self, *a):
        _fold_state.packs = self.prev
        return False


def _fold_packs():
    return getattr(_fold_state, "packs", None)


def _fold_identity(C):
    ident = _fold_state.packs["identity"]
    if ident.shape[1] < C:
        raise RuntimeError(f"folded_inference: identity coefficients cover {ident.shape[1]} channels, {C} needed")
    return ident[:, :C]


def _fold_conv(x, conv, act, dil=1, out=None):
    hit = _fold_state.packs.get(conv)
    if hit is None:
        raise RuntimeError("folded_inference: no folded pack for this convolution (not followed by a BatchNorm in the model)")
    wf, bias = hit
    x, ldx = _nhwc(materialize(x))
    N, H, W, CinP = x.shape
    Cout, Cin_g, KH, KW = conv.weight.shape
    if pad8(Cin_g * conv.groups) != CinP:
        raise RuntimeError(f"conv_bn: input has {CinP} channels, weight expects {Cin_g * conv.groups}")
    CoutP = pad8(Cout)
    z, ldz = _slot_or_new(None if out is None else [out], (N, H, W, CoutP), x.dtype, x.device)
    lib().call("egm_conv_fwd_act", dtype_code(x.dtype), ptr(x), ldx, ptr(wf), ptr(bias), CoutP, ptr(z), ldz, N, H, W, CinP, CoutP, KH, KW,
               1 if KH == 1 and KW == 1 else dil, act, stream())
    return z


def _fold_conv_ew(x, conv, act, p, mode, alpha, out):
    y = _fold_conv(x, conv, ACT_NONE)
    p, ldp = _nhwc(materialize(p))
    if tuple(p.shape) != tuple(y.shape):
        raise RuntimeError(f"conv_bn_ew: element-wise operand {tuple(p.shape)} does not match the conv output {tuple(y.shape)}")
# ... 228 lines not shown
        cs = [x.shape[3] for x in xs]
        buf = buf_slot[0] if buf_slot is not None else None
        if buf is not None and not (buf.is_contiguous() and tuple(buf.shape) == (N, H, W, sum(cs)) and buf.dtype == xs[0].dtype):
            raise RuntimeError("cat_channels: destination buffer does not match the inputs")
        out = buf if buf is not None else torch.empty((N, H, W, sum(cs)), dtype=xs[0].dtype, device=xs[0].device)
        off = 0
        for x, c in zip(xs, cs):
            dst = out[..., off:off + c]
            if not (x.data_ptr() == dst.data_ptr() and x.stride() == dst.stride()):
                _axpby(x, 1.0, None, 0.0, dst)
            off += c
        ctx.cs = cs
        return out

    @staticmethod
    def backward(ctx, g):
        outs, off = [None], 0
        for c in ctx.cs:
            outs.append(g[..., off:off + c])
            off += c
        return tuple(outs)


def cat_channels(xs, buf=None):
    return _CatC.apply(None if buf is None else [buf], *xs)


def _hp(x):
    x, ldx = _nhwc(x)
    N, H, W, C = x.shape
    out = torch.empty((N, H, W, C), dtype=x.dtype, device=x.device)
    lib().call("egm_highpass3", dtype_code(x.dtype), ptr(x), ldx, ptr(out), C, N, H, W, C, stream())
    return out


class _Highpass3(Function):
    @staticmethod
    def forward(ctx, x):
        return _hp(x)

    @staticmethod
    def backward(ctx, g):
        return _hp(g)


def highpass3(x):
    return _Highpass3.apply(x)


class _ForkHighpass(Function):

    @staticmethod
    def forward(ctx, x, n):
        return (_hp(x),) + tuple(x.view_as(x) for _ in range(n))

    @staticmethod
    def backward(ctx, ghp, *gs):
        gs = [g for g in gs if g is not None]
        if ghp is None:
            return (_Fork.backward(ctx, *gs)[0] if gs else None), None
        if not gs:
            return _hp(ghp), None
        while len(gs) > 3:
            gs = gs[:2] + [_Fork.backward(ctx, *gs[2:])[0]]
        a, lda = _nhwc(ghp)
        N, H, W, C = a.shape
        ts = [_nhwc(t) for t in gs] + [(None, 0)] * (3 - len(gs))
        out = torch.empty(a.shape, dtype=a.dtype, device=a.device)
        lib().call("egm_sum4_hp", dtype_code(a.dtype), ptr(a), lda, ptr(ts[0][0]), ts[0][1], ptr(ts[1][0]), ts[1][1], ptr(ts[2][0]), ts[2][1],
                   ptr(out), C, N, H, W, C, stream())
        return out, None


def fork_highpass3(x, n):
    return _ForkHighpass.apply(x, n)


class _GateMul(Function):
    @staticmethod
    def forward(ctx, x, w):
        x, ldx = _nhwc(x)
        w, ldw = _nhwc(w)
        out = torch.empty(x.shape, dtype=x.dtype, device=x.device)
        lib().call("egm_gate_mul_fwd", dtype_code(x.dtype), ptr(x), ldx, ptr(w), ldw, ptr(out), x.shape[3], _npix(x), x.shape[3], stream())
        ctx.save_for_backward(x, w)
        return out

    @staticmethod
    def backward(ctx, g):
        x, w = ctx.saved_tensors
        x, ldx = _nhwc(x); w, ldw = _nhwc(w); g, ldg = _nhwc(g)
        C = x.shape[3]
        dx = torch.empty(x.shape, dtype=x.dtype, device=x.device)
        dw = torch.empty(x.shape, dtype=x.dtype, device=x.device)
        lib().call("egm_gate_mul_bwd", dtype_code(x.dtype), ptr(g), ldg, ptr(x), ldx, ptr(w), ldw, ptr(dx), C, ptr(dw), C, _npix(x), C, stream())
        return dx, dw


def gate_mul(x, w):
    return _GateMul.apply(x, w)


class _ScaleAddRelu(Function):
    @staticmethod
    def forward(ctx, a, alpha, b):
        a, lda = _nhwc(a); b, ldb = _nhwc(b)
        C = a.shape[3]
        out = torch.empty(a.shape, dtype=a.dtype, device=a.device)
        lib().call("egm_scale_add_relu_fwd", dtype_code(a.dtype), ptr(a), lda, float(alpha), ptr(b), ldb, ptr(out), C, _npix(a), C, stream())
        ctx.save_for_backward(out)
        ctx.alpha = float(alpha)
        return out

    @staticmethod
    def backward(ctx, g):
        (out,) = ctx.saved_tensors
        out, ldo = _nhwc(out); g, ldg = _nhwc(g)
        C = out.shape[3]
        da = torch.empty(out.shape, dtype=out.dtype, device=out.device)
        db = torch.empty(out.shape, dtype=out.dtype, device=out.device)
        lib().call("egm_scale_add_relu_bwd", dtype_code(out.dtype), ptr(g), ldg, ptr(out), ldo, ctx.alpha, ptr(da), C, ptr(db), C, _npix(out), C,
                   stream())
        return da, None, db
# ... 688 lines not shown
```

egm_unet_amd/unet.py:

```python
from typing import Dict

import torch
import torch.nn as nn

from . import ops
from ._lib import ACT_RELU, require_gpu


class DoubleConv(nn.Sequential):

    def __init__(self, in_channels, out_channels, mid_channels=None, use_attention=False):
        if mid_channels is None:
            mid_channels = out_channels
        super().__init__(
            nn.Conv2d(in_channels, mid_channels, kernel_size=3, padding=1, bias=False),
            nn.BatchNorm2d(mid_channels),
            nn.ReLU(inplace=True),
            nn.Conv2d(mid_channels, out_channels, kernel_size=3, padding=1, bias=False),
            nn.BatchNorm2d(out_channels),
            nn.ReLU(inplace=True),
        )

    def forward(self, x, out=None, lazy=False, pool=False):
        x = ops.conv_bn_act(x, self[0], self[1], ACT_RELU)
        if pool:
            if ops.pool_fusable(x):
                return ops.conv_bn_act_pool(x, self[3], self[4], ACT_RELU, out=out)
            return ops.fork_maxpool2(ops.conv_bn_act(x, self[3], self[4], ACT_RELU, out=out))
        return ops.conv_bn_act(x, self[3], self[4], ACT_RELU, out=out, lazy=lazy)


class Down(nn.Sequential):

    def __init__(self, in_channels, out_channels):
        super().__init__(nn.MaxPool2d(2, stride=2), DoubleConv(in_channels, out_channels))

    def forward(self, x, pooled=None, pool=False):
        return self[1](ops.maxpool2(x) if pooled is None else pooled, pool=pool)


class Up(nn.Module):

    def __init__(self, in_channels, out_channels, bilinear=True, use_attention=False):
        super().__init__()
        self.bilinear = bilinear
        if bilinear:
            self.up = nn.Upsample(scale_factor=2, mode="bilinear", align_corners=True)
            self.conv = DoubleConv(in_channels, out_channels, in_channels // 2)
        else:
            self.up = nn.ConvTranspose2d(in_channels, in_channels // 2, kernel_size=2, stride=2)
            self.conv = DoubleConv(in_channels, out_channels)

    def forward(self, x1, x2, catbuf=None, lazy=False):
        if self.bilinear:
            return self.conv(ops.upcat(x2, x1, catbuf), lazy=lazy)
        x1 = ops.conv_transpose2x2(x1, self.up, (x2.shape[1], x2.shape[2]))
        return self.conv(ops.cat_channels([x2, x1]), lazy=lazy)


class OutConv(nn.Sequential):

    def __init__(self, in_channels, num_classes):
        super().__init__(nn.Conv2d(in_channels, num_classes, kernel_size=1))

    def forward(self, x, sole_consumer=False):
        if sole_consumer and ops.bn_act_cls_ok(x, self[0].weight):
            out = ops.bn_act_cls(x, self[0].weight, self[0].bias)
            out._egm_nchw_logits = True
            return out
        was_lazy = isinstance(x, ops.Lazy)
        return ops.conv2d(ops.materialize(x), self[0].weight, self[0].bias, defer_dgrad=sole_consumer and not was_lazy)


class _SegNetBase(nn.Module):

    compute_dtype = torch.float32
    ddp_boundary = None
# ... 68 lines not shown
```

include/egm_hip.h:

```cpp
#ifndef EGM_HIP_H
#define EGM_HIP_H

#ifdef __cplusplus
extern "C" {
#endif

typedef void* egm_stream_t;

enum egm_status { EGM_OK = 0, EGM_ERR_ARG = -1, EGM_ERR_LAUNCH = -2, EGM_ERR_UNSUPPORTED = -3 };
enum egm_dtype { EGM_F32 = 0, EGM_BF16 = 1 };
enum egm_act { EGM_ACT_NONE = 0, EGM_ACT_RELU = 1, EGM_ACT_SIGMOID = 2, EGM_ACT_SILU = 3  };

int egm_version(void);
const char* egm_last_error(void);
int egm_device_ok(void);

int egm_nchw_to_nhwc(int dtype, const void* src_f32, void* dst, int ld, int N, int C, int H, int W, egm_stream_t s);
int egm_nhwc_to_nchw(int dtype, const void* src, int ld, void* dst_f32, int N, int C, int H, int W, egm_stream_t s);

int egm_conv_pack(int dtype, const void* w_oihw_f32, void* wf, void* wd, int Cout, int Cin, int KH, int KW, int groups,
                  egm_stream_t s);
int egm_conv_pack_chunk(void);
int egm_conv_pack_multi(int dtype, const void* table_dev, int n, long long total_chunks, egm_stream_t s);
int egm_group_begin(void);
int egm_group_end(egm_stream_t s);
int egm_group_abort(void);
int egm_conv_tile_mode(int mode);
int egm_conv_tile_debug(int dbg);
int egm_conv_c7_mode(int mode);
int egm_conv_split_ok(int dtype, int N, int H, int W, int Cin, int Cout, int KH, int KW, int dil, int csplit);
int egm_conv_fwd_split(int dtype, const void* x, int ldx, const void* wf, void* y, int ldy, void* y2, int ldy2, int csplit, int N,
                       int H, int W, int Cin, int Cout, int KH, int KW, int dil, egm_stream_t s);
int egm_conv_kernel_name(int dtype, int N, int H, int W, int Cin, int Cout, int KH, int KW, int dil, char* buf, int buflen);
int egm_conv_fwd(int dtype, const void* x, int ldx, const void* wf, const void* bias_f32, int bias_n, void* y, int ldy,
                 float* stats, int N, int H, int W, int Cin, int Cout, int KH, int KW, int dil, egm_stream_t s);
int egm_conv_stats_tiles(int dtype, int N, int H, int W, int Cin, int Cout, int KH, int KW, int dil);
int egm_conv_fwd_act(int dtype, const void* x, int ldx, const void* wf, const void* bias_f32, int bias_n, void* y, int ldy, int N, int H,
                     int W, int Cin, int Cout, int KH, int KW, int dil, int act, egm_stream_t s);
int egm_conv_fold_chunk(void);
int egm_conv_fold_pack_multi(int dtype, const void* table_dev, int n, long long total_chunks, egm_stream_t s);
int egm_argmax_u8(const float* logits, const unsigned char* lut, unsigned char* out, int N, int C, int H, int W, egm_stream_t s);
long long egm_conv_wgrad_workspace(int N, int H, int W, int Cin, int Cout, int KH, int KW);
int egm_conv_wgrad(int dtype, const void* x, int ldx, const void* dy, int lddy, float* dw_oihw_f32, void* workspace,
                   int N, int H, int W, int Cin, int Cout, int CinR, int CoutR, int KH, int KW, int dil, int groups,
                   int accumulate, egm_stream_t s);
int egm_conv_wgrad_kernel_name(int dtype, int N, int H, int W, int Cin, int Cout, int KH, int KW, int dil, char* buf, int buflen);
#define EGM_WGRAD_MULTI_MAX 4
typedef struct egm_conv_wgrad_desc {
    const void* x; const void* dy; void* slabs;
    int ldx, lddy, N, H, W, Cin, Cout, Cin_real, Cout_real, KH, KW, dil, groups, pad_;
} egm_conv_wgrad_desc;
int egm_conv_wgrad_multi(int dtype, const egm_conv_wgrad_desc* descs, int n, egm_stream_t stream);
int egm_conv_wgrad_slabs(int dtype, int N, int H, int W, int Cin, int Cout, int KH, int KW, int dil);
int egm_wgrad_reduce(const float* slabs, float* dw_oihw_f32, int nslab, int taps, int CoutP, int CinP, int CoutR, int CinR, int groups,
                     int accumulate, egm_stream_t s);
int egm_wgrad_reduce_chunk(void);
int egm_wgrad_reduce_multi(const void* table_dev, int n, long long total_chunks, egm_stream_t s);
int egm_dwconv3_fwd(int dtype, const void* x, int ldx, const float* w, const float* b, const float* scale, void* y, int ldy,
                    int N, int H, int W, int C, egm_stream_t s);
long long egm_dwconv3_bwd_workspace(int N, int H, int W, int C);
int egm_dwconv3_bwd(int dtype, const void* x, int ldx, const void* dy, int lddy, const float* w, const float* b,
                    const float* scale, void* dx, int lddx, float* dw, float* db, float* dscale, void* workspace,
                    int N, int H, int W, int C, egm_stream_t s);

int egm_channel_partials_blocks(long long npix, int C);
int egm_channel_sums(int dtype, const void* x, int ld, long long npix, int C, float* partials, egm_stream_t s);
int egm_reduce_tiles(const float* tiles, int ntiles, int C, float* out_2xC, egm_stream_t s);
int egm_reduce_tiles_batched(const float* tiles, int batch, int ntiles, int C, float* out, egm_stream_t s);
typedef struct { const void* x; float* part; float* out; long long npix; int ld, C, Cout, nblk, chunk0, pad; } egm_bsum_entry;
int egm_bias_grad_multi(int dtype, const void* table_dev, int n, long long blocks1, long long blocks2, egm_stream_t s);

int egm_bn_finalize(const float* stats, int ntiles, long long count, const float* gamma, const float* beta, float eps,
                    float momentum, float* running_mean, float* running_var, float* scale, float* shift,
                    float* save_mean, float* save_rstd, int C, int C_real, egm_stream_t s);
int egm_bn_eval_coeffs(const float* gamma, const float* beta, const float* running_mean, const float* running_var,
                       float eps, float* scale, float* shift, float* save_mean, float* save_rstd, int C, int C_real,
                       egm_stream_t s);
int egm_bn_act_fwd(int dtype, const void* y, int ldy, const float* scale, const float* shift, int act, void* z, int ldz,
                   long long npix, int C, egm_stream_t s);
int egm_bn_act_bwd_reduce(int dtype, const void* dz, int lddz, const void* y, int ldy, const float* scale,
                          const float* shift, const float* save_mean, const float* save_rstd, int act, float* partials,
                          long long npix, int C, egm_stream_t s);
int egm_bn_act_bwd_apply(int dtype, const void* dz, int lddz, const void* y, int ldy, const float* scale,
                         const float* shift, const float* save_mean, const float* save_rstd, int act, int train,
                         const float* sums, void* dy, int lddy, long long npix, int C, egm_stream_t s);
// ... 54 lines not shown
    int ldx, lddx, Cin, Cin_real, Cout, CoutP, act, mode, ldp, ldo, ldg, ldq, lddp, train;
    float alpha, eps, momentum;
} egm_pw_head;
int egm_pw_supported(int dtype, int Cin, int CoutTot, int heads_on_input);
int egm_pw_moments_parts(long long npix);
long long egm_pw_moments_floats(long long npix, int Cin);
int egm_pw_bwd_parts(int dtype, long long npix, int Cin, int CoutTot);
long long egm_pw_bwd_floats(int dtype, long long npix, int Cin, int CoutTot);
int egm_pw_moments(int dtype, const egm_pw_head* heads, int n, egm_stream_t s);
int egm_pw_fwd_coefs(int dtype, const egm_pw_head* heads, int n, egm_stream_t s);
int egm_pw_fwd(int dtype, const egm_pw_head* heads, int n, egm_stream_t s);
int egm_pw_bwd_reduce(int dtype, const egm_pw_head* heads, int n, egm_stream_t s);
int egm_pw_bwd_coefs(int dtype, const egm_pw_head* heads, int n, egm_stream_t s);
int egm_pw_bwd_apply(int dtype, const egm_pw_head* heads, int n, egm_stream_t s);

typedef struct egm_conv1x1_bwd_desc {
    const void* x;  const void* dy;  const void* wd;  void* dx;  float* slabs;
    long long npix;
    int ldx, lddy, lddx, Cin, Cout, pad_;
} egm_conv1x1_bwd_desc;
int egm_conv1x1_bwd_supported(int dtype, int Cin, int Cout);
int egm_conv1x1_bwd_slabs(long long npix);
int egm_conv1x1_bwd(int dtype, const egm_conv1x1_bwd_desc* descs, int n, egm_stream_t s);

int egm_maxpool2_fwd(int dtype, const void* x, int ldx, void* y, int ldy, int N, int H, int W, int C, egm_stream_t s);
int egm_maxpool2_bwd(int dtype, const void* x, int ldx, const void* dy, int lddy, void* dx, int lddx, int N, int H, int W,
                     int C, egm_stream_t s);
int egm_maxpool2_bwd_add(int dtype, const void* x, int ldx, const void* dy, int lddy, const void* add, int ldadd, void* dx, int lddx,
                         int N, int H, int W, int C, egm_stream_t s);
int egm_bn_act_fwd_pool(int dtype, const void* y, int ldy, const float* scale, const float* shift, int act, void* z, int ldz,
                        void* pooled, int ldp, int N, int H, int W, int C, egm_stream_t s);
int egm_bn_pool_bwd_blocks(int N, int H, int W, int C);
int egm_bn_pool_bwd_reduce(int dtype, const void* gskip, int ldgs, const void* gpool, int ldgp, const void* y, int ldy,
                           const float* scale, const float* shift, const float* save_mean, const float* save_rstd, int act,
                           float* partials, int N, int H, int W, int C, egm_stream_t s);
int egm_bn_pool_bwd_apply(int dtype, const void* gskip, int ldgs, const void* gpool, int ldgp, const void* y, int ldy,
                          const float* scale, const float* shift, const float* save_mean, const float* save_rstd, int act, int train,
                          const float* sums, void* dy, int lddy, int N, int H, int W, int C, egm_stream_t s);
int egm_gate3_fwd_pool(int dtype, const void* x, int ldx, const void* t, int ldt, void* out, int ldo, void* pooled, int ldp, int N,
                       int H, int W, int C, egm_stream_t s);
int egm_gate3_pool_bwd(int dtype, const void* gskip, int ldgs, const void* gpool, int ldgp, const void* x, int ldx, const void* t,
                       int ldt, void* dx, int lddx, void* dt, int lddt, int N, int H, int W, int C, egm_stream_t s);
int egm_upcat_fwd(int dtype, const void* skip, int lds, const void* low, int ldl, void* out, int ldo, int N, int Hs, int Ws,
                  int Cs, int Hl, int Wl, int Cl, egm_stream_t s);
int egm_upcat_bwd_low(int dtype, const void* dout, int ldo, void* dlow, int ldl, int N, int Hs, int Ws, int Cs, int Hl,
                      int Wl, int Cl, egm_stream_t s);

int egm_axpby(int dtype, const void* a, int lda, float alpha, const void* b, int ldb, float beta, void* out, int ldo,
              long long npix, int C, egm_stream_t s);
int egm_sum4(int dtype, const void* a, int lda, const void* b, int ldb, const void* c, int ldc, const void* d, int ldd, void* out,
             int ldo, long long npix, int C, egm_stream_t s);
int egm_sum4_hp(int dtype, const void* a, int lda, const void* b, int ldb, const void* c, int ldc, const void* d, int ldd, void* out,
                int ldo, int N, int H, int W, int C, egm_stream_t s);
int egm_vec_add_f32(float* y, const float* x, long long n, egm_stream_t s);
int egm_fill_f32(float* y, float v, long long n, egm_stream_t s);
int egm_copy_cols_f32(const float* src, int ld_src, int col0_src, float* dst, int ld_dst, int col0_dst, int rows, int ncols,
                      egm_stream_t s);

int egm_highpass3(int dtype, const void* x, int ldx, void* out, int ldo, int N, int H, int W, int C, egm_stream_t s);
int egm_gate_mul_fwd(int dtype, const void* x, int ldx, const void* w, int ldw, void* out, int ldo, long long npix, int C,
                     egm_stream_t s);
int egm_gate_mul_bwd(int dtype, const void* g, int ldg, const void* x, int ldx, const void* w, int ldw, void* dx, int lddx,
                     void* dw, int lddw, long long npix, int C, egm_stream_t s);

int egm_scale_add_relu_fwd(int dtype, const void* a, int lda, float alpha, const void* b, int ldb, void* out, int ldo,
                           long long npix, int C, egm_stream_t s);
int egm_scale_add_relu_bwd(int dtype, const void* g, int ldg, const void* out, int ldo, float alpha, void* da, int ldda,
                           void* db, int lddb, long long npix, int C, egm_stream_t s);
int egm_gate3_fwd(int dtype, const void* x, int ldx, const void* t, int ldt, void* out, int ldo, long long npix, int C,
                  egm_stream_t s);
int egm_gate3_bwd(int dtype, const void* g, int ldg, const void* x, int ldx, const void* t, int ldt, void* dx, int lddx,
                  void* dt, int lddt, long long npix, int C, egm_stream_t s);

int egm_bcast_gate_fwd(int dtype, const void* a, int lda, const void* gl, int ldgl, void* out, int ldo, long long npix, int C,
                       egm_stream_t s);
int egm_bcast_gate_bwd(int dtype, const void* g, int ldg, const void* a, int lda, const void* gl, int ldgl, void* da, int ldda,
                       void* dgl, int lddgl, long long npix, int C, egm_stream_t s);
int egm_gelu_fwd(int dtype, const void* x, int ldx, void* out, int ldo, long long npix, int C, egm_stream_t s);
int egm_gelu_bwd(int dtype, const void* g, int ldg, const void* x, int ldx, void* dx, int lddx, long long npix, int C,
                 egm_stream_t s);

int egm_chan_meanmax_fwd(int dtype, const void* x, int ldx, void* out, int ldo, long long npix, int C, int C_real,
                         egm_stream_t s);
int egm_chan_meanmax_bwd(int dtype, const void* g, int ldg, const void* x, int ldx, void* dx, int lddx, long long npix, int C,
                         int C_real, egm_stream_t s);
int egm_sa_conv7_fwd(int dtype, const void* x, int ldx, const float* w, void* y, int ldy, int N, int H, int W, egm_stream_t s);
long long egm_sa_conv7_bwd_workspace(int N, int H, int W);
int egm_sa_conv7_bwd(int dtype, const void* x, int ldx, const void* dy, int lddy, const float* w, void* dx, int lddx, float* dw,
                     void* workspace, int N, int H, int W, egm_stream_t s);
long long egm_global_pool_workspace(int N, long long HW, int C);
int egm_global_avgmax_fwd(int dtype, const void* x, int ldx, void* out, int* argidx, void* workspace, int N, long long HW,
                          int C, egm_stream_t s);
int egm_global_avgmax_bwd(int dtype, const void* gout, const int* argidx, void* dx, int lddx, int N, long long HW, int C,
                          egm_stream_t s);
int egm_rows_dup(int dtype, const float* red, void* dst, int ldd, int N, int C, egm_stream_t s);
int egm_ca_mlp_fwd(int dtype, const void* pooled, int ldp, const float* w0, const float* w2, float* h, void* logits, int ldo, int R,
                   int C, int Cr, egm_stream_t s);
int egm_ca_mlp_bwd(int dtype, const void* dlogits, int ldd, const void* pooled, int ldp, const float* h, const float* w0,
                   const float* w2, float* dw0, float* dw2, void* dpooled, int lddp, int R, int C, int Cr, egm_stream_t s);
int egm_fusion_combine_fwd(int dtype, const void* f, int ldf, const void* sv, int lds, const void* sa, int ldsa, const void* ca,
                           void* out, int ldo, int N, long long HW, int C, egm_stream_t s);
int egm_fusion_combine_blocks(long long HW, int C);
int egm_fusion_combine_bwd(int dtype, const void* g, int ldg, const void* sv, int lds, const void* sa, int ldsa, const void* ca,
                           void* ds, int ldds, void* dsa, int lddsa, float* partials, int N, long long HW, int C, egm_stream_t s);
int egm_fold2_fwd(const float* w, float* out, int rows, int K, egm_stream_t s);
int egm_fold2_bwd(const float* g, float* dw, int rows, int K, egm_stream_t s);
// ... 214 lines not shown
```

Measured before the change: 677.0 images/s.

## Fuse downstream BN-backward channel reductions into dgrad conv and sum4_hp epilogues

Adds bwdstats variants of the 3x3 tile/wreg conv kernels and the sum4_hp kernel whose epilogues compute the per-channel partial sums that the next BN backward needs (activation gradient times the input, plus its correlation with normalized y). The Python autograd layer tracks the BN producer below each conv/stream op and passes these partials forward, so the standalone bwd_reduce pass is skipped. This removes a full extra read of the gradient and activation tensors per BN backward. In exchange the epilogue gains extra loads and LDS, and the new paths only apply to single-use producers and supported tile configurations.

```diff
diff --git a/egm_unet_amd/csrc/bn.hip b/egm_unet_amd/csrc/bn.hip
--- a/egm_unet_amd/csrc/bn.hip
+++ b/egm_unet_amd/csrc/bn.hip
@@ -1,58 +1,11 @@
 #include "common.h"
 #include "bn_elem.h"
+#include "bn_partials.h"
 #include <stdlib.h>
 
 namespace {
 
 
-template <typename T, int MODE>
-__device__ __forceinline__ void channel_partials_body(const T* __restrict__ a, int lda, const T* __restrict__ y, int ldy,
-                                                      const float* __restrict__ scale, const float* __restrict__ shift,
-                                                      const float* __restrict__ mean, const float* __restrict__ rstd,
-                                                      int act, long long npix, int C, float* __restrict__ out, int bid, int nb) {
-    __shared__ float red[2 * 256 * 8];
-    const int ncv = C >> 3, rows = 256 / ncv;
-    const int tid = threadIdx.x, cv = tid % ncv, row = tid / ncv;
-    float s[8], q[8];
-    zero8(s); zero8(q);
-    if (MODE == 1) {
-        for (int c = tid; c < C; c += 256) { red[c] = scale[c]; red[C + c] = shift[c]; red[2 * C + c] = mean[c]; red[3 * C + c] = rstd[c]; }
-        __syncthreads();
-    }
-    float sc[8], sh[8], mu[8], rs[8];
-    if (MODE == 1) {
-#pragma unroll
-        for (int j = 0; j < 8; ++j) { sc[j] = red[cv * 8 + j]; sh[j] = red[C + cv * 8 + j]; mu[j] = red[2 * C + cv * 8 + j]; rs[j] = red[3 * C + cv * 8 + j]; }
-        __syncthreads();
-    }
-    if (row < rows) {
-        for (long long p = (long long)bid * rows + row; p < npix; p += (long long)nb * rows) {
-            float v[8];
-            load8(a + p * lda + cv * 8, v);
-            if (MODE == 0) {
-#pragma unroll
-                for (int j = 0; j < 8; ++j) { s[j] += v[j]; q[j] += v[j] * v[j]; }
-            } else {
-                float yv[8];
-                load8(y + p * ldy + cv * 8, yv);
-#pragma unroll
-                for (int j = 0; j < 8; ++j) {
-                    const float g = v[j] * act_grad<sizeof(T) == 2>(fmaf(yv[j], sc[j], sh[j]), act);
-                    s[j] += g; q[j] += g * (yv[j] - mu[j]) * rs[j];
-                }
-            }
-        }
-    }
-#pragma unroll
-    for (int j = 0; j < 8; ++j) { red[tid * 8 + j] = s[j]; red[(256 + tid) * 8 + j] = q[j]; }
-    __syncthreads();
-    for (int t = tid; t < 2 * C; t += 256) {
-        const int which = t / C, c = t - which * C, ccv = c >> 3, j = c & 7;
-        float v = 0.f;
-        for (int r = 0; r < rows; ++r) v += red[(which * 256 + r * ncv + ccv) * 8 + j];
-        out[((long long)bid * 2 + which) * C + c] = v;
-    }
-}
 template <typename T, int MODE>
 __global__ __launch_bounds__(256) void channel_partials_kernel(const T* __restrict__ a, int lda, const T* __restrict__ y, int ldy,
                                                                const float* __restrict__ scale, const float* __restrict__ shift,
diff --git a/egm_unet_amd/csrc/bn_partials.h b/egm_unet_amd/csrc/bn_partials.h
--- /dev/null
+++ b/egm_unet_amd/csrc/bn_partials.h
@@ -0,0 +1,60 @@
+#pragma once
+#include "common.h"
+#include "bn_elem.h"
+
+template <typename T, int MODE, typename Src>
+__device__ __forceinline__ void channel_partials_from(Src src, const T* __restrict__ y, int ldy,
+                                                      const float* __restrict__ scale, const float* __restrict__ shift,
+                                                      const float* __restrict__ mean, const float* __restrict__ rstd,
+                                                      int act, long long npix, int C, float* __restrict__ out, int bid, int nb) {
+    __shared__ float red[2 * 256 * 8];
+    const int ncv = C >> 3, rows = 256 / ncv;
+    const int tid = threadIdx.x, cv = tid % ncv, row = tid / ncv;
+    float s[8], q[8];
+    zero8(s); zero8(q);
+    if (MODE == 1) {
+        for (int c = tid; c < C; c += 256) { red[c] = scale[c]; red[C + c] = shift[c]; red[2 * C + c] = mean[c]; red[3 * C + c] = rstd[c]; }
+        __syncthreads();
+    }
+    float sc[8], sh[8], mu[8], rs[8];
+    if (MODE == 1) {
+#pragma unroll
+        for (int j = 0; j < 8; ++j) { sc[j] = red[cv * 8 + j]; sh[j] = red[C + cv * 8 + j]; mu[j] = red[2 * C + cv * 8 + j]; rs[j] = red[3 * C + cv * 8 + j]; }
+        __syncthreads();
+    }
+    if (row < rows) {
+        for (long long p = (long long)bid * rows + row; p < npix; p += (long long)nb * rows) {
+            float v[8];
+            src(p, cv, v);
+            if (MODE == 0) {
+#pragma unroll
+                for (int j = 0; j < 8; ++j) { s[j] += v[j]; q[j] += v[j] * v[j]; }
+            } else {
+                float yv[8];
+                load8(y + p * ldy + cv * 8, yv);
+#pragma unroll
+                for (int j = 0; j < 8; ++j) {
+                    const float g = v[j] * act_grad<sizeof(T) == 2>(fmaf(yv[j], sc[j], sh[j]), act);
+                    s[j] += g; q[j] += g * (yv[j] - mu[j]) * rs[j];
+                }
+            }
+        }
+    }
+#pragma unroll
+    for (int j = 0; j < 8; ++j) { red[tid * 8 + j] = s[j]; red[(256 + tid) * 8 + j] = q[j]; }
+    __syncthreads();
+    for (int t = tid; t < 2 * C; t += 256) {
+        const int which = t / C, c = t - which * C, ccv = c >> 3, j = c & 7;
+        float v = 0.f;
+        for (int r = 0; r < rows; ++r) v += red[(which * 256 + r * ncv + ccv) * 8 + j];
+        out[((long long)bid * 2 + which) * C + c] = v;
+    }
+}
+template <typename T, int MODE>
+__device__ __forceinline__ void channel_partials_body(const T* __restrict__ a, int lda, const T* __restrict__ y, int ldy,
+                                                      const float* __restrict__ scale, const float* __restrict__ shift,
+                                                      const float* __restrict__ mean, const float* __restrict__ rstd,
+                                                      int act, long long npix, int C, float* __restrict__ out, int bid, int nb) {
+    channel_partials_from<T, MODE>([&](long long p, int cv, float (&v)[8]) __attribute__((always_inline)) { load8(a + p * lda + cv * 8, v); },
+                                   y, ldy, scale, shift, mean, rstd, act, npix, C, out, bid, nb);
+}
diff --git a/egm_unet_amd/csrc/conv3x3_tile.hip b/egm_unet_amd/csrc/conv3x3_tile.hip
--- a/egm_unet_amd/csrc/conv3x3_tile.hip
+++ b/egm_unet_amd/csrc/conv3x3_tile.hip
@@ -23,6 +23,7 @@
     int tiles_y, tiles_x, npt, nct, G;
     int dbg;
 };
+struct TileBwdStats { const bf16_t* yb; const float* scale; const float* shift; const float* mean; const float* rstd; int ldyb, act; };
 
 template <int R, int NT, int WR, int WC, int NBUF> struct TileGeom {
     static constexpr int TROWS = WR * R, PH = TROWS + 2, NC = WC * NT * 32;
@@ -56,10 +57,20 @@
 template <int R, int NT, int WR, int WC, int NBUF>
 __global__ __launch_bounds__(512, 2) void conv3x3_tile_kernel(TileParams p) {
     constexpr int ACT = EGM_ACT_NONE;
+    constexpr bool BWDSTATS = false;
+    const TileBwdStats bs = {};
+#include "conv3x3_tile_body.h"
+}
+template <int R, int NT, int WR, int WC, int NBUF>
+__global__ __launch_bounds__(512, 2) void conv3x3_tile_bwdstats_kernel(TileParams p, TileBwdStats bs) {
+    constexpr int ACT = EGM_ACT_NONE;
+    constexpr bool BWDSTATS = true;
 #include "conv3x3_tile_body.h"
 }
 template <int R, int NT, int WR, int WC, int NBUF, int ACT>
 __global__ __launch_bounds__(512, 2) void conv3x3_tile_act_kernel(TileParams p) {
+    constexpr bool BWDSTATS = false;
+    const TileBwdStats bs = {};
 #include "conv3x3_tile_body.h"
 }
 
@@ -80,6 +91,24 @@
     const int grid = ((p.G + 7) / 8) * 8 * p.nct;
     hipLaunchKernelGGL(kern, dim3(grid), dim3(512), Gm::SMEM, st, p);
     EGM_CHECK_LAUNCH("conv3x3_tile");
+    return EGM_OK;
+}
+
+template <int R, int NT, int WR, int WC, int NBUF>
+int launch_tile_bwdstats(const TileParams& p, const TileBwdStats& bs, hipStream_t st) {
+    using Gm = TileGeom<R, NT, WR, WC, NBUF>;
+    constexpr int SMEM_BS = Gm::SMEM + 4 * Gm::NC * (int)sizeof(float);
+    static_assert(SMEM_BS <= 160 * 1024, "LDS budget");
+    constexpr auto kern = &conv3x3_tile_bwdstats_kernel<R, NT, WR, WC, NBUF>;
+    static bool attr_done = false;
+    if (!attr_done) {
+        hipError_t e = hipFuncSetAttribute(reinterpret_cast<const void*>(kern), hipFuncAttributeMaxDynamicSharedMemorySize, 160 * 1024);
+        if (e != hipSuccess) EGM_FAIL(EGM_ERR_LAUNCH, "conv3x3_tile: hipFuncSetAttribute: %s", hipGetErrorString(e));
+        attr_done = true;
+    }
+    const int grid = ((p.G + 7) / 8) * 8 * p.nct;
+    hipLaunchKernelGGL(kern, dim3(grid), dim3(512), SMEM_BS, st, p, bs);
+    EGM_CHECK_LAUNCH("conv3x3_tile (bwdstats)");
     return EGM_OK;
 }
 
@@ -148,9 +177,8 @@
     }
 }
 
-int egm_conv_tile_launch(const void* x, int ldx, const void* wf, const float* bias, int bias_n, void* y, int ldy, float* stats, int N, int H,
-                         int W, int Cin, int Cout, int cfg, int nct, int G, egm_stream_t s, void* y2, int ldy2, int csplit, int act) {
-    TileParams p;
+static int tile_params(TileParams& p, const void* x, int ldx, const void* wf, const float* bias, int bias_n, void* y, int ldy, float* stats, int N,
+                       int H, int W, int Cin, int Cout, int cfg, int nct, int G, void* y2, int ldy2, int csplit) {
     p.x = (const bf16_t*)x; p.w = (const bf16_t*)wf; p.bias = bias; p.y = (bf16_t*)y; p.stats = stats;
     p.y2 = (bf16_t*)y2; p.ldy2 = ldy2; p.csplit = y2 ? csplit : 0;
     p.ldx = ldx; p.ldy = ldy; p.N = N; p.H = H; p.W = W; p.Cin = Cin; p.Cout = Cout; p.bias_n = bias ? bias_n : 0;
@@ -158,6 +186,33 @@
     const int rows = kCfgs[cfg].rows;
     p.tiles_y = egm_cdiv(H, rows); p.tiles_x = egm_cdiv(W, TW); p.npt = N * p.tiles_y * p.tiles_x; p.nct = nct; p.G = G;
     EGM_REQUIRE((long long)(rows + 2) * W * ldx < (1LL << 31), "conv3x3_tile: halo window offsets exceed 32 bits");
+    return EGM_OK;
+}
+
+int egm_conv_tile_launch_bwdstats(const void* x, int ldx, const void* wf, void* y, int ldy, float* part, const void* yb, int ldyb,
+                                  const float* scale, const float* shift, const float* mean, const float* rstd, int act, int N, int H, int W,
+                                  int Cin, int Cout, int cfg, int nct, int G, egm_stream_t s) {
+    EGM_REQUIRE(cfg >= 0 && cfg <= 3, "conv3x3_tile: no bwdstats instantiation for tile configuration %d", cfg);
+    TileParams p;
+    const int rc = tile_params(p, x, ldx, wf, nullptr, 0, y, ldy, part, N, H, W, Cin, Cout, cfg, nct, G, nullptr, 0, 0);
+    if (rc != EGM_OK) return rc;
+    EGM_REQUIRE((long long)N * H * W * ldyb < (1LL << 40), "conv3x3_tile: yb too large");
+    TileBwdStats bs;
+    bs.yb = (const bf16_t*)yb; bs.scale = scale; bs.shift = shift; bs.mean = mean; bs.rstd = rstd; bs.ldyb = ldyb; bs.act = act;
+    hipStream_t st = (hipStream_t)s;
+    switch (cfg) {
+        case 0: return launch_tile_bwdstats<4, 2, 4, 2, 2>(p, bs, st);
+        case 1: return launch_tile_bwdstats<2, 2, 4, 2, 2>(p, bs, st);
+        case 2: return launch_tile_bwdstats<4, 2, 8, 1, 2>(p, bs, st);
+        default: return launch_tile_bwdstats<2, 2, 8, 1, 2>(p, bs, st);
+    }
+}
+
+int egm_conv_tile_launch(const void* x, int ldx, const void* wf, const float* bias, int bias_n, void* y, int ldy, float* stats, int N, int H,
+                         int W, int Cin, int Cout, int cfg, int nct, int G, egm_stream_t s, void* y2, int ldy2, int csplit, int act) {
+    TileParams p;
+    const int rc = tile_params(p, x, ldx, wf, bias, bias_n, y, ldy, stats, N, H, W, Cin, Cout, cfg, nct, G, y2, ldy2, csplit);
+    if (rc != EGM_OK) return rc;
     hipStream_t st = (hipStream_t)s;
     if (act != EGM_ACT_NONE) {
         EGM_REQUIRE(cfg <= 3 && y2 == nullptr, "conv3x3_tile: no activation instantiation for tile configuration %d", cfg);
diff --git a/egm_unet_amd/csrc/conv3x3_tile_body.h b/egm_unet_amd/csrc/conv3x3_tile_body.h
--- a/egm_unet_amd/csrc/conv3x3_tile_body.h
+++ b/egm_unet_amd/csrc/conv3x3_tile_body.h
@@ -151,10 +151,33 @@
     static_assert(9 >= KT && (3 * (R + 2) + EGM_TILE_DMA_EVERY - 1) / EGM_TILE_DMA_EVERY >= KT, "not enough fragment groups to carry the stage's DMA instructions");
 
     unsigned char* ot = smem + NBUF * STAGE + wv * 32 * OROW;
+    if constexpr (BWDSTATS) {
+        float* cf = reinterpret_cast<float*>(smem + Gm::SMEM);
+        for (int i = tid; i < NC; i += 512) {
+            cf[i] = bs.scale[co0 + i]; cf[NC + i] = bs.shift[co0 + i]; cf[2 * NC + i] = bs.mean[co0 + i]; cf[3 * NC + i] = bs.rstd[co0 + i];
+        }
+        asm volatile("s_waitcnt lgkmcnt(0)" ::: "memory");
+    }
     auto epilogue = [&](const Tile& t) __attribute__((always_inline)) {
         const int cv = lane % NV, slot = lane / NV;
+        [[maybe_unused]] const bool relu = bs.act == EGM_ACT_RELU;
+        [[maybe_unused]] const float* cf = reinterpret_cast<const float*>(smem + Gm::SMEM) + wc * NT * 32 + cv * 8;
 #pragma unroll
         for (int m = 0; m < R; ++m) {
+            [[maybe_unused]] uint4 ybr[NV / 2];
+            auto load_yb = [&]() __attribute__((always_inline)) {
+                const int oyb = t.oy0 + R * wr + m;
+                if (oyb < p.H) {
+                    const bf16_t* ybrow = bs.yb + co0 + wc * NT * 32 + ((long long)(t.n * p.H + oyb) * p.W + t.ox0) * bs.ldyb;
+#pragma unroll
+                    for (int it2 = 0; it2 < NV / 2; ++it2) {
+                        const int pl = it2 * (64 / NV) + slot;
+                        const int plc = t.ox0 + pl < p.W ? pl : 0;
+                        ybr[it2] = *reinterpret_cast<const uint4*>(ybrow + (plc * bs.ldyb + cv * 8));
+                    }
+                }
+            };
+            if constexpr (BWDSTATS && R < 4) load_yb();
 #pragma unroll
             for (int nt = 0; nt < NT; ++nt)
 #pragma unroll
@@ -175,6 +198,7 @@
                     v.y = pack_bf16x2(EGM_ACC(m, nt, gq * 4 + 2), EGM_ACC(m, nt, gq * 4 + 3));
                     *reinterpret_cast<uint2*>(ot + r31 * OROW + (nt * 32 + gq * 8 + h * 4) * 2) = v;
                 }
+            if constexpr (BWDSTATS && R >= 4) load_yb();
             const int oy = t.oy0 + R * wr + m;
             uint4 raw[NV / 2];
 #pragma unroll
@@ -197,8 +221,37 @@
                     v[2] = __uint_as_float(rw.y << 16); v[3] = __uint_as_float(rw.y & 0xffff0000u);
                     v[4] = __uint_as_float(rw.z << 16); v[5] = __uint_as_float(rw.z & 0xffff0000u);
                     v[6] = __uint_as_float(rw.w << 16); v[7] = __uint_as_float(rw.w & 0xffff0000u);
-#pragma unroll
-                    for (int j = 0; j < 8; ++j) { ssum[j] += v[j]; ssq[j] = fmaf(v[j], v[j], ssq[j]); }
+                    if constexpr (!BWDSTATS) {
+#pragma unroll
+                        for (int j = 0; j < 8; ++j) { ssum[j] += v[j]; ssq[j] = fmaf(v[j], v[j], ssq[j]); }
+                    }
+                }
+                if constexpr (BWDSTATS) {
+                    constexpr int CW = 4;
+                    typedef __attribute__((ext_vector_type(CW))) float cfv_t;
+#pragma unroll
+                    for (int c0 = 0; c0 < 8; c0 += CW) {
+                        const cfv_t csc = *reinterpret_cast<const volatile cfv_t*>(cf + c0), csh = *reinterpret_cast<const volatile cfv_t*>(cf + NC + c0);
+                        const cfv_t cmu = *reinterpret_cast<const volatile cfv_t*>(cf + 2 * NC + c0), crs = *reinterpret_cast<const volatile cfv_t*>(cf + 3 * NC + c0);
+#pragma unroll
+                        for (int it2 = 0; it2 < NV / 2; ++it2) {
+                            const bool ok = t.ox0 + it2 * (64 / NV) + slot < p.W;
+                            const unsigned rd[4] = {raw[it2].x, raw[it2].y, raw[it2].z, raw[it2].w};
+                            const unsigned yd[4] = {ybr[it2].x, ybr[it2].y, ybr[it2].z, ybr[it2].w};
+#pragma unroll
+                            for (int i = 0; i < CW; i += 2) {
+                                unsigned d = rd[(c0 + i) >> 1], y2 = yd[(c0 + i) >> 1];
+                                if (!ok) { d = 0; y2 = 0; }
+                                const float v[2] = {__uint_as_float(d << 16), __uint_as_float(d & 0xffff0000u)};
+                                const float yv[2] = {__uint_as_float(y2 << 16), __uint_as_float(y2 & 0xffff0000u)};
+#pragma unroll
+                                for (int k = 0; k < 2; ++k) {
+                                    const float g = v[k] * (relu ? act_grad<true>(fmaf(yv[k], csc[i + k], csh[i + k]), EGM_ACT_RELU) : 1.f);
+                                    ssum[c0 + i + k] += g; ssq[c0 + i + k] += g * (yv[k] - cmu[i + k]) * crs[i + k];
+                                }
+                            }
+                        }
+                    }
                 }
             }
         }
diff --git a/egm_unet_amd/csrc/conv3x3_wreg.hip b/egm_unet_amd/csrc/conv3x3_wreg.hip
--- a/egm_unet_amd/csrc/conv3x3_wreg.hip
+++ b/egm_unet_amd/csrc/conv3x3_wreg.hip
@@ -28,6 +28,7 @@
     int ldx, ldy, N, H, W, Cin, Cout, bias_n;
     int tiles_y, tiles_x, npt, G;
 };
+struct WregBwdStats { const bf16_t* yb; const float* scale; const float* shift; const float* mean; const float* rstd; int ldyb, act; };
 
 __device__ __forceinline__ uint32_t pack2(float lo, float hi) {
     f32x2_t v; v.x = lo; v.y = hi;
@@ -43,10 +44,20 @@
 template <int CH>
 __global__ __launch_bounds__(512, 2) void conv3x3_wreg_kernel(WregParams p) {
     constexpr int ACT = EGM_ACT_NONE;
+    constexpr bool BWDSTATS = false;
+    const WregBwdStats bs = {};
+#include "conv3x3_wreg_body.h"
+}
+template <int CH>
+__global__ __launch_bounds__(512, 2) void conv3x3_wreg_bwdstats_kernel(WregParams p, WregBwdStats bs) {
+    constexpr int ACT = EGM_ACT_NONE;
+    constexpr bool BWDSTATS = true;
 #include "conv3x3_wreg_body.h"
 }
 template <int CH, int ACT>
 __global__ __launch_bounds__(512, 2) void conv3x3_wreg_act_kernel(WregParams p) {
+    constexpr bool BWDSTATS = false;
+    const WregBwdStats bs = {};
 #include "conv3x3_wreg_body.h"
 }
 
@@ -78,13 +89,41 @@
 }
 const char* egm_conv_wreg_name(int Cin) { (void)Cin; return "conv3x3_wreg_kernel<1>"; }
 
-int egm_conv_wreg_launch(const void* x, int ldx, const void* wf, const float* bias, int bias_n, void* y, int ldy, float* stats, int N, int H,
-                         int W, int Cin, int Cout, int G, egm_stream_t s, int act) {
-    WregParams p;
+static int wreg_params(WregParams& p, const void* x, int ldx, const void* wf, const float* bias, int bias_n, void* y, int ldy, float* stats, int N,
+                       int H, int W, int Cin, int Cout, int G) {
     p.x = (const bf16_t*)x; p.w = (const bf16_t*)wf; p.bias = bias; p.y = (bf16_t*)y; p.stats = stats;
     p.ldx = ldx; p.ldy = ldy; p.N = N; p.H = H; p.W = W; p.Cin = Cin; p.Cout = Cout; p.bias_n = bias ? bias_n : 0;
     p.tiles_y = egm_cdiv(H, TROWS); p.tiles_x = egm_cdiv(W, TW); p.npt = N * p.tiles_y * p.tiles_x; p.G = G;
     EGM_REQUIRE((long long)(PH + 1) * W * ldx < (1LL << 31), "conv3x3_wreg: halo window offsets exceed 32 bits");
+    return EGM_OK;
+}
+
+int egm_conv_wreg_launch_bwdstats(const void* x, int ldx, const void* wf, void* y, int ldy, float* part, const void* yb, int ldyb,
+                                  const float* scale, const float* shift, const float* mean, const float* rstd, int act, int N, int H, int W,
+                                  int Cin, int Cout, int G, egm_stream_t s) {
+    WregParams p;
+    const int rc = wreg_params(p, x, ldx, wf, nullptr, 0, y, ldy, part, N, H, W, Cin, Cout, G);
+    if (rc != EGM_OK) return rc;
+    EGM_REQUIRE(Cout == 32 && (long long)N * H * W * ldyb < (1LL << 40), "conv3x3_wreg: bad yb");
+    WregBwdStats bs;
+    bs.yb = (const bf16_t*)yb; bs.scale = scale; bs.shift = shift; bs.mean = mean; bs.rstd = rstd; bs.ldyb = ldyb; bs.act = act;
+    constexpr auto kern = &conv3x3_wreg_bwdstats_kernel<1>;
+    static bool attr_done = false;
+    if (!attr_done) {
+        hipError_t e = hipFuncSetAttribute(reinterpret_cast<const void*>(kern), hipFuncAttributeMaxDynamicSharedMemorySize, 160 * 1024);
+        if (e != hipSuccess) EGM_FAIL(EGM_ERR_LAUNCH, "conv3x3_wreg: hipFuncSetAttribute: %s", hipGetErrorString(e));
+        attr_done = true;
+    }
+    hipLaunchKernelGGL(kern, dim3(p.G), dim3(512), SMEM, (hipStream_t)s, p, bs);
+    EGM_CHECK_LAUNCH("conv3x3_wreg (bwdstats)");
+    return EGM_OK;
+}
+
+int egm_conv_wreg_launch(const void* x, int ldx, const void* wf, const float* bias, int bias_n, void* y, int ldy, float* stats, int N, int H,
+                         int W, int Cin, int Cout, int G, egm_stream_t s, int act) {
+    WregParams p;
+    const int rc = wreg_params(p, x, ldx, wf, bias, bias_n, y, ldy, stats, N, H, W, Cin, Cout, G);
+    if (rc != EGM_OK) return rc;
     switch (act) {
         case EGM_ACT_RELU: return launch_wreg<1, EGM_ACT_RELU>(p, (hipStream_t)s);
         case EGM_ACT_SIGMOID: return launch_wreg<1, EGM_ACT_SIGMOID>(p, (hipStream_t)s);
diff --git a/egm_unet_amd/csrc/conv3x3_wreg_body.h b/egm_unet_amd/csrc/conv3x3_wreg_body.h
--- a/egm_unet_amd/csrc/conv3x3_wreg_body.h
+++ b/egm_unet_amd/csrc/conv3x3_wreg_body.h
@@ -127,9 +127,32 @@
                 *reinterpret_cast<uint2*>(ot + (m * 32 + r31) * OROW + (gq * 8 + h * 4) * 2) = v;
             }
     };
+    [[maybe_unused]] float sc[8], sh[8], mu[8], rs[8];
+    if constexpr (BWDSTATS) {
+#pragma unroll
+        for (int j = 0; j < 8; ++j) {
+            const int c = (lane & 3) * 8 + j;
+            sc[j] = bs.scale[c]; sh[j] = bs.shift[c]; mu[j] = bs.mean[c]; rs[j] = bs.rstd[c];
+        }
+    }
     auto store_tile = [&](const Tile& t) __attribute__((always_inline)) {
         const int cv = lane & 3, slot = lane >> 2;
         const int oy0 = t.ty * TROWS, ox0 = t.tx * TW;
+        [[maybe_unused]] const bool relu = bs.act == EGM_ACT_RELU;
+        [[maybe_unused]] uint4 ybr[R][2];
+        if constexpr (BWDSTATS) {
+#pragma unroll
+            for (int m = 0; m < R; ++m) {
+                const int oy = oy0 + R * wv + m;
+                const bf16_t* ybrow = bs.yb + ((long long)(t.n * p.H + oy) * p.W + ox0) * bs.ldyb + cv * 8;
+#pragma unroll
+                for (int i2 = 0; i2 < 2; ++i2) {
+                    const int pl = i2 * 16 + slot;
+                    ybr[m][i2] = make_uint4(0, 0, 0, 0);
+                    if (oy < p.H && ox0 + pl < p.W) ybr[m][i2] = *reinterpret_cast<const uint4*>(ybrow + (long long)pl * bs.ldyb);
+                }
+            }
+        }
         uint4 raw[R][2];
 #pragma unroll
         for (int m = 0; m < R; ++m)
@@ -152,8 +175,22 @@
                 v[2] = __uint_as_float(rw.y << 16); v[3] = __uint_as_float(rw.y & 0xffff0000u);
                 v[4] = __uint_as_float(rw.z << 16); v[5] = __uint_as_float(rw.z & 0xffff0000u);
                 v[6] = __uint_as_float(rw.w << 16); v[7] = __uint_as_float(rw.w & 0xffff0000u);
-#pragma unroll
-                for (int j = 0; j < 8; ++j) { ssum[j] += v[j]; ssq[j] = fmaf(v[j], v[j], ssq[j]); }
+                if constexpr (BWDSTATS) {
+                    const uint4 yr = ybr[m][i2];
+                    float yv[8];
+                    yv[0] = __uint_as_float(yr.x << 16); yv[1] = __uint_as_float(yr.x & 0xffff0000u);
+                    yv[2] = __uint_as_float(yr.y << 16); yv[3] = __uint_as_float(yr.y & 0xffff0000u);
+                    yv[4] = __uint_as_float(yr.z << 16); yv[5] = __uint_as_float(yr.z & 0xffff0000u);
+                    yv[6] = __uint_as_float(yr.w << 16); yv[7] = __uint_as_float(yr.w & 0xffff0000u);
+#pragma unroll
+                    for (int j = 0; j < 8; ++j) {
+                        const float g = v[j] * (relu ? act_grad<true>(fmaf(yv[j], sc[j], sh[j]), EGM_ACT_RELU) : 1.f);
+                        ssum[j] += g; ssq[j] += g * (yv[j] - mu[j]) * rs[j];
+                    }
+                } else {
+#pragma unroll
+                    for (int j = 0; j < 8; ++j) { ssum[j] += v[j]; ssq[j] = fmaf(v[j], v[j], ssq[j]); }
+                }
             }
         }
     };
diff --git a/egm_unet_amd/csrc/conv_igemm.hip b/egm_unet_amd/csrc/conv_igemm.hip
--- a/egm_unet_amd/csrc/conv_igemm.hip
+++ b/egm_unet_amd/csrc/conv_igemm.hip
@@ -23,6 +23,12 @@
 int egm_conv_tile_launch(const void* x, int ldx, const void* wf, const float* bias, int bias_n, void* y, int ldy, float* stats, int N, int H,
                          int W, int Cin, int Cout, int cfg, int nct, int G, egm_stream_t s, void* y2 = nullptr, int ldy2 = 0, int csplit = 0,
                          int act = EGM_ACT_NONE);
+int egm_conv_wreg_launch_bwdstats(const void* x, int ldx, const void* wf, void* y, int ldy, float* part, const void* yb, int ldyb,
+                                  const float* scale, const float* shift, const float* mean, const float* rstd, int act, int N, int H, int W,
+                                  int Cin, int Cout, int G, egm_stream_t s);
+int egm_conv_tile_launch_bwdstats(const void* x, int ldx, const void* wf, void* y, int ldy, float* part, const void* yb, int ldyb,
+                                  const float* scale, const float* shift, const float* mean, const float* rstd, int act, int N, int H, int W,
+                                  int Cin, int Cout, int cfg, int nct, int G, egm_stream_t s);
 int egm_conv_c7_plan(int dtype, int N, int H, int W, int Cin, int Cout, int KH, int KW, int dil);
 int egm_conv_c7_launch(const void* x, int ldx, const void* wf, const float* bias, int bias_n, void* y, int ldy, int N, int H, int W,
                        egm_stream_t s, int act = EGM_ACT_NONE);
@@ -694,6 +700,38 @@
     EGM_REQUIRE(ldx >= Cin && ldx % 8 == 0 && ldy >= csplit && ldy % 8 == 0 && ldy2 >= Cout - csplit && ldy2 % 8 == 0, "conv_fwd_split: bad ld");
     const ConvPlan c = conv_plan(dtype, N, H, W, Cin, Cout, KH, KW, dil);
     return egm_conv_tile_launch(x, ldx, wf, nullptr, 0, y, ldy, nullptr, N, H, W, Cin, Cout, c.tile_cfg, c.nct, c.G, s, y2, ldy2, csplit);
+}
+
+#ifndef EGM_WREG_BWDSTATS
+#define EGM_WREG_BWDSTATS 1
+#endif
+static int conv_bwdstats_kind(int dtype, int N, int H, int W, int Cin, int Cout, int KH, int KW, int dil) {
+    if (dtype != EGM_BF16 || N <= 0 || H <= 0 || W <= 0 || Cin <= 0 || Cin % 8 || Cout <= 0 || Cout % 8) return 0;
+    if (KH == 1 && KW == 1) dil = 1;
+    const ConvPlan c = conv_plan(dtype, N, H, W, Cin, Cout, KH, KW, dil);
+    if (c.c16d || c.c7) return 0;
+    if (c.wreg) return EGM_WREG_BWDSTATS ? 1 : 2;
+    if (!c.tile || c.tile_cfg > 3) return 0;
+    return (c.tile_cfg == 1 || c.tile_cfg == 3) ? 1 : 2;
+}
+extern "C" int egm_conv_bwdstats_ok(int dtype, int N, int H, int W, int Cin, int Cout, int KH, int KW, int dil) {
+    return conv_bwdstats_kind(dtype, N, H, W, Cin, Cout, KH, KW, dil) == 1;
+}
+extern "C" int egm_conv_fwd_bwdstats(int dtype, const void* x, int ldx, const void* wf, void* y, int ldy, float* part, const void* yb, int ldyb,
+                                     const float* scale, const float* shift, const float* mean, const float* rstd, int act, int N, int H,
+                                     int W, int Cin, int Cout, int KH, int KW, int dil, egm_stream_t s) {
+    EGM_REQUIRE(x && wf && y && part && yb && scale && shift && mean && rstd, "conv_fwd_bwdstats: null pointer");
+    EGM_REQUIRE(egm_aligned16(x) && egm_aligned16(wf) && egm_aligned16(y) && egm_aligned16(yb), "conv_fwd_bwdstats: pointers must be 16-byte aligned");
+    EGM_REQUIRE(conv_bwdstats_kind(dtype, N, H, W, Cin, Cout, KH, KW, dil) != 0, "conv_fwd_bwdstats: no instantiation for this shape");
+    EGM_REQUIRE(act == EGM_ACT_NONE || act == EGM_ACT_RELU, "conv_fwd_bwdstats: activation %d (NONE or RELU)", act);
+    EGM_REQUIRE(ldx >= Cin && ldx % 8 == 0 && ldy >= Cout && ldy % 8 == 0 && ldyb >= Cout && ldyb % 8 == 0, "conv_fwd_bwdstats: bad ld");
+    EGM_REQUIRE(act >= EGM_ACT_NONE && act <= EGM_ACT_SILU, "conv_fwd_bwdstats: unknown activation %d", act);
+    EGM_REQUIRE((long long)N * H * W * (long long)(ldx > ldy ? ldx : ldy) < (1LL << 40), "conv_fwd_bwdstats: tensor too large");
+    const ConvPlan c = conv_plan(dtype, N, H, W, Cin, Cout, KH, KW, dil);
+    if (c.wreg)
+        return egm_conv_wreg_launch_bwdstats(x, ldx, wf, y, ldy, part, yb, ldyb, scale, shift, mean, rstd, act, N, H, W, Cin, Cout, c.G, s);
+    return egm_conv_tile_launch_bwdstats(x, ldx, wf, y, ldy, part, yb, ldyb, scale, shift, mean, rstd, act, N, H, W, Cin, Cout, c.tile_cfg,
+                                         c.nct, c.G, s);
 }
 
 static int conv_fwd_impl(int dtype, const void* x, int ldx, const void* wf, const void* bias, int bias_n, void* y, int ldy, float* stats,
diff --git a/egm_unet_amd/csrc/pool_up.hip b/egm_unet_amd/csrc/pool_up.hip
--- a/egm_unet_amd/csrc/pool_up.hip
+++ b/egm_unet_amd/csrc/pool_up.hip
@@ -1,4 +1,5 @@
 #include "common.h"
+#include "bn_partials.h"
 
 namespace {
 
@@ -492,6 +493,48 @@
         store8(out + p * ldo + cv * 8, v);
     }
 }
+template <typename T>
+__global__ __launch_bounds__(256) void sum4_hp_part_kernel(const T* __restrict__ a, int lda, const T* __restrict__ b, int ldb, const T* __restrict__ c,
+                                                           int ldc, const T* __restrict__ d, int ldd, T* __restrict__ out, int ldo, int N, int H, int W,
+                                                           int C, const T* __restrict__ yb, int ldyb, const float* __restrict__ scale,
+                                                           const float* __restrict__ shift, const float* __restrict__ mean,
+                                                           const float* __restrict__ rstd, int act, float* __restrict__ part) {
+    auto produce = [&](long long p, int cv, float (&v)[8]) __attribute__((always_inline)) {
+        int xx, yy; egm_pix_yx(p, H, W, yy, xx);
+        float u[8], s8[8];
+        zero8(s8);
+        load8(a + p * lda + cv * 8, v);
+#pragma unroll
+        for (int r = -1; r <= 1; ++r)
+#pragma unroll
+            for (int q = -1; q <= 1; ++q) {
+                if (yy + r < 0 || yy + r >= H || xx + q < 0 || xx + q >= W) continue;
+                load8(a + (p + (long long)r * W + q) * lda + cv * 8, u);
+#pragma unroll
+                for (int j = 0; j < 8; ++j) s8[j] += u[j];
+            }
+#pragma unroll
+        for (int j = 0; j < 8; ++j) v[j] = to_f32(from_f32<T>(v[j] - s8[j] * (1.f / 9.f)));
+        load8(b + p * ldb + cv * 8, u);
+#pragma unroll
+        for (int j = 0; j < 8; ++j) v[j] += u[j];
+        if (c != nullptr) {
+            load8(c + p * ldc + cv * 8, u);
+#pragma unroll
+            for (int j = 0; j < 8; ++j) v[j] += u[j];
+        }
+        if (d != nullptr) {
+            load8(d + p * ldd + cv * 8, u);
+#pragma unroll
+            for (int j = 0; j < 8; ++j) v[j] += u[j];
+        }
+        store8(out + p * ldo + cv * 8, v);
+#pragma unroll
+        for (int j = 0; j < 8; ++j) v[j] = to_f32(from_f32<T>(v[j]));
+    };
+    channel_partials_from<T, 1>(produce, yb, ldyb, scale, shift, mean, rstd, act, (long long)N * H * W, C, part,
+                                xcd_contiguous_item(blockIdx.x, gridDim.x), gridDim.x);
+}
 __global__ void vec_add_f32_kernel(float* __restrict__ y, const float* __restrict__ x, long long n) {
     for (long long i = blockIdx.x * 256LL + threadIdx.x; i < n; i += (long long)gridDim.x * 256) y[i] += x[i];
 }
@@ -571,6 +614,25 @@
     EGM_DISPATCH_DTYPE(dtype, hipLaunchKernelGGL((sum4_hp_kernel<T>), dim3(stream_grid((long long)N * H * W * (C / 8))), dim3(256), 0, (hipStream_t)s,
                                                  (const T*)a, lda, (const T*)b, ldb, (const T*)c, ldc, (const T*)d, ldd, (T*)out, ldo, N, H, W, C));
     EGM_CHECK_LAUNCH("sum4_hp");
+    return EGM_OK;
+}
+extern "C" int egm_sum4_hp_bwdstats_ok(int dtype, long long npix, int C) {
+    return (dtype == EGM_BF16 || dtype == EGM_F32) && npix > 0 && C > 0 && C % 8 == 0 && C <= 1024 && 256 % (C / 8) == 0;
+}
+extern "C" int egm_sum4_hp_bwdstats(int dtype, const void* a, int lda, const void* b, int ldb, const void* c, int ldc, const void* d, int ldd,
+                                    void* out, int ldo, int N, int H, int W, int C, const void* yb, int ldyb, const float* scale,
+                                    const float* shift, const float* mean, const float* rstd, int act, float* part, egm_stream_t s) {
+    EGM_REQ_VEC("sum4_hp_bwdstats", a, lda, C); EGM_REQ_VEC("sum4_hp_bwdstats", b, ldb, C); EGM_REQ_VEC("sum4_hp_bwdstats", out, ldo, C);
+    EGM_REQ_VEC("sum4_hp_bwdstats", yb, ldyb, C);
+    if (c != nullptr) EGM_REQ_VEC("sum4_hp_bwdstats", c, ldc, C);
+    if (d != nullptr) EGM_REQ_VEC("sum4_hp_bwdstats", d, ldd, C);
+    EGM_REQUIRE(N > 0 && H > 0 && W > 0 && scale && shift && mean && rstd && part, "sum4_hp_bwdstats: bad args");
+    EGM_REQUIRE(egm_sum4_hp_bwdstats_ok(dtype, (long long)N * H * W, C), "sum4_hp_bwdstats: C=%d not offered (egm_sum4_hp_bwdstats_ok)", C);
+    const int nb = egm_partial_blocks((long long)N * H * W, C);
+    EGM_DISPATCH_DTYPE(dtype, hipLaunchKernelGGL((sum4_hp_part_kernel<T>), dim3(nb), dim3(256), 0, (hipStream_t)s, (const T*)a, lda, (const T*)b, ldb,
+                                                 (const T*)c, ldc, (const T*)d, ldd, (T*)out, ldo, N, H, W, C, (const T*)yb, ldyb, scale, shift, mean,
+                                                 rstd, act, part));
+    EGM_CHECK_LAUNCH("sum4_hp_bwdstats");
     return EGM_OK;
 }
 extern "C" int egm_upcat_fwd(int dtype, const void* skip, int lds, const void* low, int ldl, void* out, int ldo, int N, int Hs, int Ws,
diff --git a/egm_unet_amd/egm_unet.py b/egm_unet_amd/egm_unet.py
--- a/egm_unet_amd/egm_unet.py
+++ b/egm_unet_amd/egm_unet.py
@@ -410,7 +410,7 @@
         grfb = self[6 + o]
         N, H, W = x.shape[0], x.shape[1], x.shape[2]
         cat = grfb.cat_buffer(N, H, W, x.dtype, x.device) if self[3 + o].out_channels == grfb.shortcut.conv.in_channels else None
-        x = ops.conv_bn_act(x, self[3 + o], self[4 + o], ACT_RELU, out=None if cat is None else cat[1][0])
+        x = ops.conv_bn_act(x, self[3 + o], self[4 + o], ACT_RELU, out=None if cat is None else cat[1][0], sole=True)
         return grfb(x, out, cat, pool=pool)
 
 
diff --git a/egm_unet_amd/ops.py b/egm_unet_amd/ops.py
--- a/egm_unet_amd/ops.py
+++ b/egm_unet_amd/ops.py
@@ -308,6 +308,40 @@
                   ways).""")
 
 
+fuse_bn_bwd_stats = _Switch("EGM_FUSE_BN_BWD_STATS", "1", parse=int, doc=
+                           """Get / set where the kernel that WRITES the dz of a conv -> BatchNorm layer also emits that BatchNorm's backward
+                           partial sums, so that its reduce pass disappears: bit 1 = the 3x3 data-gradient convs (egm_conv_fwd_bwdstats), bit
+                           2 = the streaming producers (egm_sum4_hp_bwdstats; bit-identical partials).  0 = every BatchNorm backward runs its
+                           own reduce pass.  bf16 only.  Default 1: the streaming part measured slower in the step (on the reduce pass's
+                           1024-block decomposition egm_sum4_hp loses more than the pass costs; profiles/r04_ab_runs.md).""")
+_BWDSTATS_CONV, _BWDSTATS_STREAM = 1, 2
+
+
+class _BnBelow:
+    __slots__ = ("y", "coef", "act", "uses")
+
+    def __init__(self, y, coef, act):
+        self.y, self.coef, self.act, self.uses = y.detach(), coef, act, 0
+
+
+def _bn_below(x, bit):
+    link = getattr(x, "_egm_bn_below", None)
+    if link is None:
+        return None
+    link.uses += 1
+    return link if (fuse_bn_bwd_stats.on & bit) and x.dtype == torch.bfloat16 and link.act in (ACT_NONE, ACT_RELU) else None
+
+
+def _note_bwd_part(gx, part, ntiles):
+    _run().parts[gx.data_ptr()] = (gx, part, ntiles)
+
+
+def _take_bwd_part(g):
+    run = _run(create=False)
+    ent = run.parts.pop(g.data_ptr(), None) if run is not None and run.parts else None
+    return None if ent is None else (ent[1], ent[2])
+
+
 def _wgrad_deferrable(weight):
     return (_DEFER_WGRAD and _sole_conv_use(weight) and weight.is_leaf and weight.grad is None
             and not weight._backward_hooks and not torch.is_grad_enabled())
@@ -353,13 +387,14 @@
 
 
 class _BackwardRun:
-    __slots__ = ("id", "slabs", "wgrads", "bgrads", "dz", "__weakref__")
+    __slots__ = ("id", "slabs", "wgrads", "bgrads", "dz", "parts", "__weakref__")
 
     def __init__(self, run_id):
-        self.id, self.slabs, self.wgrads, self.bgrads, self.dz = run_id, [], [], [], {}
+        self.id, self.slabs, self.wgrads, self.bgrads, self.dz, self.parts = run_id, [], [], [], {}, {}
 
     def finish(self):
         _runs.pop(self.id, None)
+        self.parts.clear()
         if self.dz:
             kinds = [v[1][0] for v in self.dz.values()]
             self.dz.clear()
@@ -485,8 +520,11 @@
     dtype = property(lambda self: self.y.dtype)
     device = property(lambda self: self.y.device)
 
-    def materialize(self, out=None):
-        return _Materialize.apply(self.y, self.coef, self.act, None if out is None else [out])
+    def materialize(self, out=None, sole=False):
+        z = _Materialize.apply(self.y, self.coef, self.act, None if out is None else [out])
+        if sole and fuse_bn_bwd_stats.on and torch.is_grad_enabled() and self.y.requires_grad:
+            z._egm_bn_below = _BnBelow(self.y, self.coef, self.act)
+        return z
 
 
 def materialize(x, out=None):
@@ -604,7 +642,7 @@
     return res
 
 
-def _conv_grads(x, ldx, dy, weight, wd, dil, groups, Cin, Cout, need_gx, need_gw, x_split=0, c1=True):
+def _conv_grads(x, ldx, dy, weight, wd, dil, groups, Cin, Cout, need_gx, need_gw, x_split=0, c1=True, below=None):
     N, H, W, CinP = x.shape
     CoutP = dy.shape[3]
     if c1 and need_gw and not x_split and _c1_shape_ok(x, dy, weight, dil, groups):
@@ -613,7 +651,7 @@
     if need_gw:
         gw = _conv_wgrad(x, ldx, dy, CoutP, weight, dil, groups, Cin, Cout)
     if need_gx:
-        gx = _conv_dgrad(dy, wd, N, H, W, CoutP, CinP, weight.shape[2], weight.shape[3], dil, x_split)
+        gx = _conv_dgrad(dy, wd, N, H, W, CoutP, CinP, weight.shape[2], weight.shape[3], dil, x_split, below)
     return gx, gw
 
 
@@ -698,9 +736,18 @@
     return _Conv2d.apply(materialize(x), weight, bias, dil, groups, want_stats, bias_grad_zero, defer_dgrad)
 
 
-def _conv_dgrad(dy, wd, N, H, W, CoutP, CinP, KH, KW, dil, x_split):
+def _conv_dgrad(dy, wd, N, H, W, CoutP, CinP, KH, KW, dil, x_split, below=None):
     L, dt, st = lib(), dtype_code(dy.dtype), stream()
     gx = torch.empty((N, H, W, CinP), dtype=dy.dtype, device=dy.device)
+    if (below is not None and below.uses == 1 and not x_split and tuple(below.y.shape) == (N, H, W, CinP)
+            and L.cdll.egm_conv_bwdstats_ok(dt, N, H, W, CoutP, CinP, KH, KW, dil)):
+        yb, ldyb = _nhwc(below.y)
+        ntiles = L.query("egm_conv_stats_tiles", dt, N, H, W, CoutP, CinP, KH, KW, dil)
+        part = _f32(ntiles * 2 * CinP, dy.device)
+        L.call("egm_conv_fwd_bwdstats", dt, ptr(dy), CoutP, ptr(wd), ptr(gx), CinP, ptr(part), ptr(yb), ldyb, *_rows(below.coef), below.act,
+               N, H, W, CoutP, CinP, KH, KW, dil, st)
+        _note_bwd_part(gx, part, ntiles)
+        return gx
     if x_split and fuse_dz.on and L.cdll.egm_conv_split_ok(dt, N, H, W, CoutP, CinP, KH, KW, dil, x_split):
         ga = torch.empty((N, H, W, x_split), dtype=dy.dtype, device=dy.device)
         gb = torch.empty((N, H, W, CinP - x_split), dtype=dy.dtype, device=dy.device)
@@ -798,21 +845,26 @@
     return nb, _f32(nb * 2 * CP, dev), _f32((2, CP), dev), _f32((4, CP), dev), torch.empty(tuple(y.shape), dtype=y.dtype, device=dev)
 
 
-def _bn_backward(family, lead, geo, y, coef, act, training, nb=None):
+def _bn_backward(family, lead, geo, y, coef, act, training, nb=None, part=None):
     L, st = lib(), stream()
     y, ldy = _nhwc(y)
     CP, npix = y.shape[3], _npix(y)
-    nb, part, sums, cf4, dy = _bn_bwd_buffers(y, nb)
     rows, train = _rows(coef), 1 if training else 0
-    L.call(family + "_bwd_reduce", *lead, ptr(y), ldy, *rows, act, ptr(part), *geo, st)
+    if part is not None:
+        part, nb = part
+        _, _, sums, cf4, dy = _bn_bwd_buffers(y, 1)
+    else:
+        nb, part, sums, cf4, dy = _bn_bwd_buffers(y, nb)
+        L.call(family + "_bwd_reduce", *lead, ptr(y), ldy, *rows, act, ptr(part), *geo, st)
     L.call("egm_bn_bwd_coefs", ptr(part), nb, npix, *rows, train, ptr(sums), ptr(cf4), CP, st)
     L.call(family + "_bwd_apply", *lead, ptr(y), ldy, *rows, act, train, ptr(sums), ptr(dy), CP, *geo, st)
     return dy, sums
 
 
-def _conv_bn_grads(need, x, ldx, dy, weight, wd, sums, dil, groups, has_bias, Cin, Cout, training, x_split=0, c1=True, conv_grads=None):
+def _conv_bn_grads(need, x, ldx, dy, weight, wd, sums, dil, groups, has_bias, Cin, Cout, training, x_split=0, c1=True, conv_grads=None,
+                   below=None):
     if conv_grads is None:
-        conv_grads = _conv_grads(x, ldx, dy, weight, wd, dil, groups, Cin, Cout, need[0], need[1], x_split, c1)
+        conv_grads = _conv_grads(x, ldx, dy, weight, wd, dil, groups, Cin, Cout, need[0], need[1], x_split, c1, below)
     gx, gw = conv_grads
     gb = _bn_conv_bias_grad(Cout, dy, training, dy.device) if (has_bias and need[2]) else None
     return gx, gw, gb, sums[1, :Cout] if need[3] else None, sums[0, :Cout] if need[4] else None
@@ -822,6 +874,7 @@
 
     @staticmethod
     def forward(ctx, x, weight, bias, gamma, beta, running_mean, running_var, eps, momentum, act, training, dil, groups, x_split=0):
+        ctx.below = _bn_below(x, _BWDSTATS_CONV)
         x, ldx = _nhwc(x)
         ctx.x_split = int(x_split) if (x_split and 0 < x_split < x.shape[3] and x_split % 8 == 0) else 0
         Cout, Cin_g = weight.shape[0], weight.shape[1]
@@ -842,6 +895,7 @@
         x, weight, wd, y, coef = ctx.saved_tensors
         dil, groups, has_bias, Cin, Cout, act, training = ctx.meta
         pend = _take_dz(gz)
+        part = _take_bwd_part(gz) if pend is None else None
         gz, ldg = _nhwc(gz)
         x, ldx = _nhwc(x)
         CoutP, npix, dt = y.shape[3], _npix(y), dtype_code(x.dtype)
@@ -853,9 +907,9 @@
         else:
             _, dxo, ldd, gates, mcoef, ns, geo = pend[1]
             family = ("egm_bn_mca", (dt, ptr(dxo), ldd, ptr(gates), ptr(mcoef), ns), geo + (CoutP,))
-        dy, sums = _bn_backward(*family, y, coef, act, training)
+        dy, sums = _bn_backward(*family, y, coef, act, training, part=part)
         return _conv_bn_grads(ctx.needs_input_grad, x, ldx, dy, weight, wd, sums, dil, groups, has_bias, Cin, Cout, training,
-                              ctx.x_split) + (None,) * 9
+                              ctx.x_split, below=ctx.below) + (None,) * 9
 
 
 fuse_mca_bwd = _Switch("EGM_FUSE_MCA_BWD", "1",
@@ -876,6 +930,7 @@
 
     @staticmethod
     def forward(ctx, x, weight, bias, gamma, beta, running_mean, running_var, eps, momentum, act, training, dil, groups, out_slot):
+        ctx.below = _bn_below(x, _BWDSTATS_CONV)
         x, ldx = _nhwc(x)
         Cout, Cin_g = weight.shape[0], weight.shape[1]
         y, stats, wd = _conv_forward(x, ldx, weight, bias, dil, groups, training)
@@ -916,7 +971,7 @@
             family, nb = ("egm_bn_act", (dt, ptr(gz), ldg), (_npix(y), CoutP)), None
         dy, sums = _bn_backward(*family, y, coef, act, training, nb)
         return _conv_bn_grads(ctx.needs_input_grad, x, ldx, dy, weight, wd, sums, dil, groups, has_bias, Cin, Cout, training,
-                              c1=False) + (None,) * 9
+                              c1=False, below=ctx.below) + (None,) * 9
 
 
 def conv_bn_lazy(x, conv, bn, act, dil=1, groups=1):
@@ -1338,7 +1393,7 @@
                         None if out is None else [out])
 
 
-def conv_bn_act(x, conv, bn, act, dil=1, groups=1, out=None, lazy=False):
+def conv_bn_act(x, conv, bn, act, dil=1, groups=1, out=None, lazy=False, sole=False):
     if _fold_packs() is not None:
         z = _fold_conv(x, conv, act, dil, out)
         return Lazy(z, _fold_identity(z.shape[3]), ACT_NONE) if out is None and lazy == "force" else z
@@ -1349,7 +1404,7 @@
     z = Lazy(y, coef, act)
     if out is None and lazy == "force":
         return z
-    return z.materialize(out)
+    return z.materialize(out, sole=sole)
 
 
 _fold_state = threading.local()
@@ -1684,6 +1739,7 @@
 
     @staticmethod
     def forward(ctx, x, n):
+        ctx.below = _bn_below(x, _BWDSTATS_STREAM)
         return (_hp(x),) + tuple(x.view_as(x) for _ in range(n))
 
     @staticmethod
@@ -1699,8 +1755,18 @@
         N, H, W, C = a.shape
         ts = [_nhwc(t) for t in gs] + [(None, 0)] * (3 - len(gs))
         out = torch.empty(a.shape, dtype=a.dtype, device=a.device)
-        lib().call("egm_sum4_hp", dtype_code(a.dtype), ptr(a), lda, ptr(ts[0][0]), ts[0][1], ptr(ts[1][0]), ts[1][1], ptr(ts[2][0]), ts[2][1],
-                   ptr(out), C, N, H, W, C, stream())
+        L, dt, below = lib(), dtype_code(a.dtype), ctx.below
+        if (below is not None and below.uses == 1 and tuple(below.y.shape) == tuple(a.shape)
+                and L.cdll.egm_sum4_hp_bwdstats_ok(dt, N * H * W, C)):
+            yb, ldyb = _nhwc(below.y)
+            nb = L.query("egm_channel_partials_blocks", N * H * W, C)
+            part = _f32(nb * 2 * C, a.device)
+            L.call("egm_sum4_hp_bwdstats", dt, ptr(a), lda, ptr(ts[0][0]), ts[0][1], ptr(ts[1][0]), ts[1][1], ptr(ts[2][0]), ts[2][1],
+                   ptr(out), C, N, H, W, C, ptr(yb), ldyb, *_rows(below.coef), below.act, ptr(part), stream())
+            _note_bwd_part(out, part, nb)
+            return out, None
+        L.call("egm_sum4_hp", dt, ptr(a), lda, ptr(ts[0][0]), ts[0][1], ptr(ts[1][0]), ts[1][1], ptr(ts[2][0]), ts[2][1],
+               ptr(out), C, N, H, W, C, stream())
         return out, None
 
 
diff --git a/egm_unet_amd/unet.py b/egm_unet_amd/unet.py
--- a/egm_unet_amd/unet.py
+++ b/egm_unet_amd/unet.py
@@ -22,7 +22,7 @@
         )
 
     def forward(self, x, out=None, lazy=False, pool=False):
-        x = ops.conv_bn_act(x, self[0], self[1], ACT_RELU)
+        x = ops.conv_bn_act(x, self[0], self[1], ACT_RELU, sole=True)
         if pool:
             if ops.pool_fusable(x):
                 return ops.conv_bn_act_pool(x, self[3], self[4], ACT_RELU, out=out)
diff --git a/include/egm_hip.h b/include/egm_hip.h
--- a/include/egm_hip.h
+++ b/include/egm_hip.h
@@ -31,6 +31,10 @@
 int egm_conv_split_ok(int dtype, int N, int H, int W, int Cin, int Cout, int KH, int KW, int dil, int csplit);
 int egm_conv_fwd_split(int dtype, const void* x, int ldx, const void* wf, void* y, int ldy, void* y2, int ldy2, int csplit, int N,
                        int H, int W, int Cin, int Cout, int KH, int KW, int dil, egm_stream_t s);
+int egm_conv_bwdstats_ok(int dtype, int N, int H, int W, int Cin, int Cout, int KH, int KW, int dil);
+int egm_conv_fwd_bwdstats(int dtype, const void* x, int ldx, const void* wf, void* y, int ldy, float* part, const void* yb, int ldyb,
+                          const float* scale, const float* shift, const float* mean, const float* rstd, int act, int N, int H, int W,
+                          int Cin, int Cout, int KH, int KW, int dil, egm_stream_t s);
 int egm_conv_kernel_name(int dtype, int N, int H, int W, int Cin, int Cout, int KH, int KW, int dil, char* buf, int buflen);
 int egm_conv_fwd(int dtype, const void* x, int ldx, const void* wf, const void* bias_f32, int bias_n, void* y, int ldy,
                  float* stats, int N, int H, int W, int Cin, int Cout, int KH, int KW, int dil, egm_stream_t s);
@@ -191,6 +195,10 @@
              int ldo, long long npix, int C, egm_stream_t s);
 int egm_sum4_hp(int dtype, const void* a, int lda, const void* b, int ldb, const void* c, int ldc, const void* d, int ldd, void* out,
                 int ldo, int N, int H, int W, int C, egm_stream_t s);
+int egm_sum4_hp_bwdstats_ok(int dtype, long long npix, int C);
+int egm_sum4_hp_bwdstats(int dtype, const void* a, int lda, const void* b, int ldb, const void* c, int ldc, const void* d, int ldd,
+                         void* out, int ldo, int N, int H, int W, int C, const void* yb, int ldyb, const float* scale,
+                         const float* shift, const float* mean, const float* rstd, int act, float* part, egm_stream_t s);
 int egm_vec_add_f32(float* y, const float* x, long long n, egm_stream_t s);
 int egm_fill_f32(float* y, float v, long long n, egm_stream_t s);
 int egm_copy_cols_f32(const float* src, int ld_src, int col0_src, float* dst, int ld_dst, int col0_dst, int rows, int ncols,
```

New measurement: 680.0 images/s, median of 6. Within noise of the previous version (+0.4%).
